# JamesYang007/adelie

Measured on AMD Instinct MI355X. Metric: lambda-paths/sec (100-lambda grpnet); HBM GB/s vs peak, higher is better.
Workload: dtype f64

## Files before the change

### adelie_amd/csrc/kernels.hpp

```cpp
#pragma once
#include <hip/hip_runtime.h>
#include <cstdint>

namespace ahip {

template <class T>
struct DenseView {
    const T* X;
    int64_t n, p, ld;
};
struct SnpView {
    const uint8_t* bits;
    int64_t n, p, ldb;
};

template <class T>
struct CscView {
    const int64_t* cptr;
    const int32_t* cidx;
    const T* cval;
    const int64_t* rptr;
    const int32_t* rcol;
    const T* rval;
    int64_t n, p, nnz;
    const int64_t* bptr;
    int nb;
    int64_t rb;
    const T* center;
    const T* inv_scale;
    const int64_t* tptr;
    const uint16_t* trow;
    const T* tval;
    int nt;
    int64_t th;
};

template <class T> void launch_vmul(const T* a, const T* b, T* out, int64_t n, hipStream_t s);
template <class T> void launch_fill(T* out, T value, int64_t n, hipStream_t s);

template <class T>
void launch_sweep(const DenseView<T>& X, const T* v, T* out, int64_t c0, int64_t ncols, const int32_t* cols,
                  const T* sub_scale, const T* sub_vec, bool square, T* work, hipStream_t s);
template <class T>
void launch_sweep_snp(const SnpView& X, const T* impute, const T* v, T* out, int64_t c0, int64_t ncols,
                      const int32_t* cols, const T* sub_scale, const T* sub_vec, bool square, T* work, hipStream_t s);
int64_t sweep_work_elems(int64_t n, int64_t ncols);
int64_t sweep_work_elems_csc(int nb, int64_t ncols);
template <class T>
void launch_sweep_csc(const CscView<T>& X, const T* v, T* out, int64_t c0, int64_t ncols, const int32_t* cols,
                      const T* sub_scale, const T* sub_vec, bool square, T* work, hipStream_t s);
constexpr int kVecSumScratch = 8 + 256;
template <class T> void launch_vec_sum(const T* v, int64_t n, T* out, hipStream_t s);
template <class T>
void launch_std_sweep_epilogue(const T* center, const T* inv_scale, const T* raw, const T* raw_plain, const T* vsum, bool square,
                               T* out, int64_t c0, int64_t ncols, const int32_t* cols, const T* sub_scale, const T* sub_vec,
                               hipStream_t s);
template <class T>
void launch_std_gram_fix(const T* center, const T* inv_scale, T* C, int64_t ldc, int32_t M, int32_t pos0, int32_t N,
                         const int32_t* vcol, const T* m, const T* wsum, const T* xm, bool centered, hipStream_t s);
template <class T>
void launch_std_scale_coef(const T* center, const T* inv_scale, const int32_t* cols, const T* coef, const int32_t* count_dev,
                           int32_t count, T* coef2, T* kappa, hipStream_t s);
template <class T> void launch_vec_shift(T* out, int64_t n, const T* kappa, T sign, const int32_t* count_dev, hipStream_t s);
template <class T>
void launch_std_fix_gblk(T* gblk, const int32_t* cols, int nb, const T* center, const T* inv_scale, const T* rsum_dev,
                         const T* xm_view_or_null, hipStream_t s);
struct SyrkBatch;
template <class T>
void launch_std_block_fix(T* D0, const SyrkBatch& sb, const int32_t* cols_base, int ldb, const T* center, const T* inv_scale,
                          const T* xm_view, const T* wsum_dev, bool centered, hipStream_t s);
template <class T>
void launch_csc_tile_scatter(const int64_t* colptr, const int32_t* cidx, const T* cval, int64_t p, int nt, int64_t th,
                             const int64_t* tptr, uint16_t* trow, T* tval, hipStream_t s);
constexpr int64_t kCscTileBytes = 128 * 1024;
void csc_block_layout(int64_t n, size_t value_size, int* nb, int64_t* rb);
void launch_csc_block_ptr(const int64_t* cptr, const int32_t* cidx, int64_t p, int nb, int64_t rb, int64_t* bptr, hipStream_t s);
int64_t gram_work_elems_csc(int64_t n, int64_t M, int64_t N, int nb);
template <class T>
void launch_gram_csc(const CscView<T>& X, const T* w, const int32_t* mcols, int32_t M, int32_t m_pos0, const int32_t* ncols,
                     int32_t N, int32_t n_pos0, const T* xm_by_col, bool center, T* C, int64_t ldc, T* work, hipStream_t s);
template <class T>
void launch_axpy_cols_csc(const CscView<T>& X, const int32_t* cols, const T* coef, const int32_t* count_dev, int32_t count,
                          T sign, T* out, T* delta_zeroed, hipStream_t s);
int64_t sp_tmul_work_elems_csc(int64_t p);
template <class T>
void launch_sp_tmul_csc(const CscView<T>& X, int64_t L, const int64_t* indptr, const int64_t* indices, const T* values, T* out,
                        T* work, hipStream_t s);

template <class T>
void launch_axpy_cols(const DenseView<T>& X, const int32_t* cols, const T* coef, const int32_t* count_dev,
                      int32_t count, T sign, T* out, hipStream_t s);
template <class T>
void launch_axpy_cols_snp(const SnpView& X, const T* impute, const int32_t* cols, const T* coef,
                          const int32_t* count_dev, int32_t count, T sign, T* out, hipStream_t s);
template <class T>
void launch_sp_tmul(const DenseView<T>& X, int64_t L, const int64_t* indptr, const int64_t* indices, const T* values,
                    T* out, hipStream_t s);
template <class T>
void launch_sp_tmul_snp(const SnpView& X, const T* impute, int64_t L, const int64_t* indptr, const int64_t* indices,
                        const T* values, T* out, hipStream_t s);

template <class T>
void launch_gram(const DenseView<T>& X, const T* w, const int32_t* mcols, int32_t M, int32_t m_pos0,
                 const int32_t* ncols, int32_t N, int32_t n_pos0, const T* xm_by_col, bool center, T* C, int64_t ldc,
                 T* work, hipStream_t s);
template <class T>
void launch_gram_snp(const SnpView& X, const T* impute, const T* w, const int32_t* mcols, int32_t M, int32_t m_pos0,
                     const int32_t* ncols, int32_t N, int32_t n_pos0, const T* xm_by_col, bool center, T* C,
                     int64_t ldc, T* work, hipStream_t s);
int64_t gram_work_elems(int64_t n, int64_t M, int64_t N);
struct SyrkBatch {
    static constexpr int MAX = 16;
    int32_t off[MAX];
    int32_t nb[MAX];
    int64_t dst[MAX];
    int32_t count;
};
int64_t syrk_batch_work_elems(int64_t n, int count);
template <class T>
void launch_panel_step_csc(const CscView<T>& X, const T* w, T* r, const int32_t* dcol, const T* dlt, const int32_t* nz_dev,
                           const int32_t* cols, int nb, const T* rsum_dev, const T* xm_by_col, T* gblk, hipStream_t s);
template <class T>
void launch_block_gram_csc(const CscView<T>& X, const T* w, const int32_t* cols_base, const SyrkBatch& sb, const T* xm_by_col,
                           bool center, T* D0, int ldb, hipStream_t s);
struct GramBatch {
// ... 180 lines not shown
    const T* C;
    int64_t ldc;
    const T* vars;
    const T* xmean;
    T* beta;
    T* g;
    int8_t* is_active;
    int32_t* active_set;
    T l1, l2, newton_tol, dbeta_tol;
    int32_t newton_max_iters, max_active_size, mark;
    const T* V;
    const int64_t* voff;
    const T* spen;
    const int32_t* sbegin;
    const int32_t* ssize;
    const int32_t* blk_g0;
    const int32_t* list;
    int32_t nblk;
    T* Dbuf;
    T* dlt;
    int32_t* didx;
    CdBlkState<T>* st;
    const T* gblk;
    const T* Dptr;
    const int32_t* vcol;
    int32_t* dcol;
    CdBlkState<T>* host_st;
    int32_t* host_seq;
    int32_t report_j, report_seq;
    int64_t* dbg;
    const T* Cprev;
    const T* pdlt;
    const int32_t* ppos;
    const int32_t* pnz;
    int32_t* dpos;
    int32_t* nz_out;
    T* rsum_out;
    int32_t rot;
    const int32_t* desc;
    const T* pdd;
    T* dd;
    const T* part;
    int32_t part_n;
    const T* part_rsum;
    int32_t* tail_counter;
    T* tail_g;
    const T* tail_rsum;
    const T* tail_xm;
    const T* clo;
    const T* chi;
    T* cmu;
    const T* Cnext;
    T* corr_out;
    const T* corr_in;
};
constexpr int GDESC_VMAP = 0;
constexpr int GDESC_VGRP = 128;
constexpr int GDESC_VSS = 256;
constexpr int GDESC_GOFF = 384;
constexpr int GDESC_GQ = 520;
constexpr int GDESC_GSS = 648;
constexpr int GDESC_NG = 776, GDESC_NVAL = 777;
constexpr int GDESC_VOFF = 784;
constexpr int GDESC_VPOS = 912;
constexpr int GDESC_VQ = 1040;
constexpr int GDESC_STRIDE = 1168;
template <class T> void launch_grp_layout(const CdGrpBlkParams<T>& p, int nblk, int32_t* desc, hipStream_t s);
struct GrpRotArgs {
    int32_t ng;
    int32_t goff[129];
    int64_t voff[128];
};
template <class T> void launch_grp_block_rotate(T* Dptr, const T* Dsrc, const T* V, const GrpRotArgs& a, T* scratch, hipStream_t s);
template <class T> void launch_cd_group_block_pass(const CdGrpBlkParams<T>& p, hipStream_t s);
template <class T> void launch_cd_group_block_range(const CdGrpBlkParams<T>& p, int j0, int j1, hipStream_t s);
template <class T> void launch_cd_group_block_update(const CdGrpBlkParams<T>& p, int j, hipStream_t s);
template <class T> void launch_cd_group_panel_solve(const CdGrpBlkParams<T>& p, int j, hipStream_t s);
int cd_block_size();
template <class T> void launch_cd_block_pass(const CdBlkParams<T>& p, hipStream_t s);
template <class T>
int launch_panel_step(const DenseView<T>& X, const T* w, T* r, const int32_t* dcol, const T* dlt, const int32_t* nz_dev,
                      const int32_t* cols, int nb, T* part, hipStream_t s);
template <class T>
struct StepTail {
    int32_t* counter;
    int32_t base;
    T* g;
    const T* rsum;
    const T* xm;
};
template <class T>
int launch_panel_step_snp(const SnpView& X, const T* impute, const T* w, T* r, const int32_t* dcol, const T* dlt,
                          const int32_t* nz_dev, const int32_t* cols, int nb, T* part, hipStream_t s,
                          const StepTail<T>* tail = nullptr, bool* tailed = nullptr);
int64_t panel_part_elems(int64_t n);
template <class T>
void launch_la_open_from_grad(const T* grad, const int32_t* cols, int nb, T* g, const T* rsum_src, T* rsum_out, hipStream_t s);
template <class T>
void launch_panel_reduce(const T* part, int nslices, int nb, const int32_t* cols, const T* rsum_dev, const T* xm_by_col,
                         T* gblk, hipStream_t s);
template <class T>
void launch_panel_reduce_ld(const T* part, int64_t part_ld, int nslices, int nb, const int32_t* cols, const T* rsum_dev,
                            const T* xm_by_col, T* gblk, hipStream_t s);
template <class T>
int launch_panel_fused(const CdBlkParams<T>& sp, int j, const DenseView<T>& X, const T* w, T* r, const int32_t* dcol,
                       const T* dlt, const int32_t* nz_dev, const int32_t* cols, int nb, T* part, bool tr, hipStream_t s);
template <class T>
int launch_panel_fused_snp(const CdBlkParams<T>& sp, int j, const SnpView& X, const T* impute, const T* w, T* r,
                           const int32_t* dcol, const T* dlt, const int32_t* nz_dev, const int32_t* cols, int nb, T* part,
                           bool tr, hipStream_t s);
template <class T>
int launch_panel_fused_grp(const CdGrpBlkParams<T>& sp, int j, const DenseView<T>& X, const T* w, T* r, const int32_t* dcol,
                           const T* dlt, const int32_t* nz_dev, const int32_t* cols, int nb, T* part, bool tr, hipStream_t s);
template <class T>
int launch_panel_fused_grp_snp(const CdGrpBlkParams<T>& sp, int j, const SnpView& X, const T* impute, const T* w, T* r,
                               const int32_t* dcol, const T* dlt, const int32_t* nz_dev, const int32_t* cols, int nb,
                               T* part, bool tr, hipStream_t s);
template <class T> void launch_cd_panel_solve(const CdBlkParams<T>& p, int j, hipStream_t s);
template <class T> void launch_center_vars(T* vars, const T* xm, int cnt, bool center, hipStream_t s);
void launch_gather_i32(const int32_t* src, const int32_t* idx, int cnt, int32_t* out, hipStream_t s);
template <class T>
void launch_cd_compact(const T* beta, const T* beta0, const int32_t* vcol, int nv, int32_t* dcols, T* dvals,
                       int32_t* n_delta, hipStream_t s);

template <class T>
struct MultiView {
    const T* X;
    int64_t nb, pb, ld;
    const T* ones;
    int32_t K, icpt;
    const uint8_t* bits = nullptr;
    int64_t ldb = 0;
    const T* impute = nullptr;
};
template <class T> void launch_multi_sweep(const MultiView<T>& X, const T* v, T* out, T* work, hipStream_t s);
template <class T> int64_t multi_sweep_work_elems(const MultiView<T>& X);
template <class T>
void launch_multi_sweep_snp(const SnpView& X, const T* impute, int K, const T* v, T* out, T* work, hipStream_t s);
template <class T>
int launch_multi_panel_step(const MultiView<T>& X, const T* w, T* r, const int32_t* dcol, const T* dlt,
                            const int32_t* nz_dev, const int32_t* cols, int nb_cols, T* part, hipStream_t s);
int64_t multi_panel_part_elems(int64_t nb);
template <class T>
void launch_multi_axpy_cols(const MultiView<T>& X, const int32_t* cols, const T* coef, const int32_t* cnt_dev, T sign,
                            T* out, hipStream_t s);
template <class T>
void launch_syrk_multi(const MultiView<T>& X, const T* w, const int32_t* ucols, int32_t M, T* C, int64_t ldc, T* work,
                       hipStream_t s);
template <class T>
void launch_multi_expand(const T* C, int64_t ldc, const int32_t* slot, const int32_t* resp, int nv, int lsel, T* D,
                         int64_t ldd, hipStream_t s);
void launch_multi_block_lists(const int32_t* cols, int nv, int K, int32_t* ulist, int32_t* slot, int32_t* resp,
                              hipStream_t s);
template <class T>
int launch_multi_panel_fused(const CdGrpBlkParams<T>& sp, int j, const MultiView<T>& X, const T* w, T* r,
                             const int32_t* dcol, const T* dlt, const int32_t* nz_dev, const int32_t* cols, int nb_cols,
                             T* part, hipStream_t s);
template <class T>
void launch_gram_multi(const MultiView<T>& X, const T* w, const int32_t* mcols, int32_t M, const int32_t* ncols, int32_t N,
                       T* C, int64_t ldc, T* work, hipStream_t s);
template <class T>
void launch_multi_expand_cross(const T* G, int64_t ldg, const int32_t* slot_r, const int32_t* resp_r, int nr,
                               const int32_t* slot_c, const int32_t* resp_c, int nc, T* C, int64_t ldc, hipStream_t s);
template <class T>
void launch_batch_pick(const T* src, int64_t nfeat, int K, int slot, const T* sub_scale, const T* sub_vec, T* out,
                       hipStream_t s);
template <class T> void launch_multi_to_major(const T* src, int64_t nb, int K, T* dst, hipStream_t s);
template <class T> void launch_multi_from_major(const T* src, int64_t nb, int K, T* dst, hipStream_t s);

template <class T>
struct IrlsScalars {
    T hess_sum, y_mean, y_var, resid_sum, conv, loss;
};

template <class T>
void launch_cov_gather(const T* S, int64_t lda, int tr, const int32_t* vcol, int32_t nv, int32_t pos0, int32_t N, T* C,
                       int64_t ldc, hipStream_t s);
template <class T>
void launch_cov_bmul(const T* S, int64_t lda, int tr, const int64_t* subset, int64_t ns, const int64_t* indices,
                     const T* values, int64_t ni, T* out, hipStream_t s);
// ... 84 lines not shown
```

### adelie_amd/csrc/kernels_cd_panel.hip

```cpp
#include "kernels.hpp"
#include "accessors.hpp"
#include "wavered.hpp"
#include "blk_solve_body.hpp"
#include "grp_solve_body.hpp"

namespace ahip {

namespace {

constexpr int PB = 128;
constexpr int PT = 256;

template <class T, int VEC>
struct RawDense { Pack<T, VEC> v; };
struct RawSnp { unsigned byte; };

template <class T, int VEC>
__device__ __forceinline__ RawDense<T, VEC> praw(const DenseAcc<T>& X, int64_t j, int64_t i, int64_t n, bool full) {
    RawDense<T, VEC> r;
    const T* col = X.colptr(j);
    if constexpr (VEC == 1) {
        const T x = col[(full || i < n) ? i : 0];
        r.v.v[0] = (full || i < n) ? x : T(0);
    } else {
        using V = typename VecOf<T>::type;
        static_assert(VEC == VecOf<T>::N, "dense vector width");
        const int64_t ii = (full || i < n) ? i : 0;
        const V x = __builtin_nontemporal_load(reinterpret_cast<const V*>(col + ii));
#pragma unroll
        for (int e = 0; e < VEC; ++e) r.v.v[e] = (full || i + e < n) ? x[e] : T(0);
    }
    return r;
}
template <class T, int VEC>
__device__ __forceinline__ RawSnp praw(const SnpAcc<T>& X, int64_t j, int64_t i, int64_t n, bool full) {
    static_assert(VEC == 4 || VEC == 16, "one byte (4 calls) or one 32-bit word (16 calls) per lane");
    RawSnp r;
    if constexpr (VEC == 4) {
        const unsigned b = unsigned(X.colptr(j)[((full || i < n) ? i : 0) >> 2]);
        r.byte = (full || i < n) ? b : 0u;
    } else {
        const unsigned b = reinterpret_cast<const unsigned*>(X.colptr(j))[((full || i < n) ? i : 0) >> 4];
        r.byte = (full || i < n) ? b : 0u;
    }
    return r;
}
template <class T, int VEC>
__device__ __forceinline__ Pack<T, VEC> pdecode(const DenseAcc<T>&, const RawDense<T, VEC>& r, int64_t, int64_t, int64_t) {
    return r.v;
}
template <class T, int VEC>
__device__ __forceinline__ Pack<T, VEC> pdecode(const SnpAcc<T>& X, const RawSnp& r, int64_t j, int64_t i, int64_t n) {
    Pack<T, VEC> o;
    const T imp = X.impute[j];
#pragma unroll
    for (int e = 0; e < VEC; ++e) {
        const unsigned c = (r.byte >> (2 * e)) & 3u;
        o.v[e] = (i + e < n) ? (c == 3u ? imp : T(c)) : T(0);
    }
    return o;
}
template <class T, class Acc, int VEC> struct RawOf;
template <class T, int VEC> struct RawOf<T, DenseAcc<T>, VEC> { using type = RawDense<T, VEC>; };
template <class T, int VEC> struct RawOf<T, SnpAcc<T>, VEC> { using type = RawSnp; };

template <class T, class Acc, int VEC, bool FULL, bool WGRED = false>
__device__ __forceinline__ void panel_step_body(const Acc& X, int64_t n, const T* __restrict__ w, T* __restrict__ r,
                                                const int32_t* __restrict__ dcol, const T* __restrict__ dlt, int nz,
                                                const int32_t* __restrict__ cols, int nb, T* __restrict__ part,
                                                int64_t part_ld, T (*red)[64 * VEC], T* wrs, int tid, int64_t slice) {
    constexpr int U = 16;
    using Raw = typename RawOf<T, Acc, VEC>::type;
    const int lane = tid & 63;
    const int wv = __builtin_amdgcn_readfirstlane(tid >> 6);
    const int64_t i = slice * (64 * VEC) + int64_t(lane) * VEC;
    const bool full = FULL ? true : (i + VEC <= n);

    constexpr int UB = 8;
    Raw xb[UB];
    int jb[UB];
    if (nb > 0) {
#pragma unroll
        for (int u = 0; u < UB; ++u) jb[u] = cols[min(wv + 4 * u, nb - 1)];
#pragma unroll
        for (int u = 0; u < UB; ++u) xb[u] = praw<T, VEC>(X, jb[u], i, n, full);
    }

    if (nz > 0) {
        T acc[VEC];
#pragma unroll
        for (int e = 0; e < VEC; ++e) acc[e] = T(0);
        for (int m0 = wv; m0 < nz; m0 += 4 * U) {
            Raw xa[U];
            int ja[U];
            T cf[U];
#pragma unroll
            for (int u = 0; u < U; ++u) {
                const int m = m0 + 4 * u;
                ja[u] = dcol[min(m, nz - 1)];
                cf[u] = m < nz ? dlt[min(m, nz - 1)] : T(0);
            }
#pragma unroll
            for (int u = 0; u < U; ++u) xa[u] = praw<T, VEC>(X, ja[u], i, n, full);
#pragma unroll
            for (int u = 0; u < U; ++u) {
                const Pack<T, VEC> xx = pdecode<T, VEC>(X, xa[u], ja[u], i, n);
#pragma unroll
                for (int e = 0; e < VEC; ++e) acc[e] = fma(cf[u], xx.v[e], acc[e]);
            }
        }
#pragma unroll
        for (int e = 0; e < VEC; ++e) red[wv][lane * VEC + e] = acc[e];
        __syncthreads();
        if (wv == 0) {
#pragma unroll
            for (int e = 0; e < VEC; ++e) {
                const int q = lane * VEC + e;
                T wr = T(0);
                if (FULL || i + e < n) {
                    const T rr = r[i + e] - ((red[0][q] + red[1][q]) + (red[2][q] + red[3][q]));
                    r[i + e] = rr;
                    wr = w[i + e] * rr;
                }
                wrs[q] = wr;
            }
        }
    } else if (wv == 0) {
#pragma unroll
        for (int e = 0; e < VEC; ++e) wrs[lane * VEC + e] = (FULL || i + e < n) ? w[i + e] * r[i + e] : T(0);
    }
    if (nb <= 0) return;
    __syncthreads();

    T wr[VEC];
#pragma unroll
    for (int e = 0; e < VEC; ++e) wr[e] = wrs[lane * VEC + e];
    for (int c0 = wv; c0 < nb; c0 += 4 * UB) {
        if (c0 != wv) {
#pragma unroll
            for (int u = 0; u < UB; ++u) jb[u] = cols[min(c0 + 4 * u, nb - 1)];
#pragma unroll
            for (int u = 0; u < UB; ++u) xb[u] = praw<T, VEC>(X, jb[u], i, n, full);
        }
        T pu[UB];
#pragma unroll
        for (int u = 0; u < UB; ++u) {
            const Pack<T, VEC> xx = pdecode<T, VEC>(X, xb[u], jb[u], i, n);
            T sacc = T(0);
#pragma unroll
            for (int e = 0; e < VEC; ++e) sacc = fma(xx.v[e], wr[e], sacc);
            pu[u] = sacc;
        }
        static_assert(UB == 8, "reduce8");
        const T tot = reduce8(pu, lane);
        if (lane < UB && c0 + 4 * lane < nb) {
            if constexpr (WGRED) red[0][c0 + 4 * lane] = tot;
            else part[part_ld > 0 ? int64_t(c0 + 4 * lane) * part_ld + slice : slice * PB + (c0 + 4 * lane)] = tot;
        }
    }
}

template <class T, class Acc, int VEC>
__global__ __launch_bounds__(PT, (VEC >= 16 ? 2 : 4)) void panel_step_kernel(Acc X, int64_t n, const T* __restrict__ w, T* __restrict__ r,
                                                        const int32_t* __restrict__ dcol, const T* __restrict__ dlt,
                                                        const int32_t* __restrict__ nz_dev,
                                                        const int32_t* __restrict__ cols, int nb, T* __restrict__ part,
                                                        int64_t part_ld) {
    constexpr int RS = 64 * VEC;
    __shared__ T red[4][RS];
    __shared__ T wrs[RS];
    const int nz = nz_dev[0];
    if ((int64_t(blockIdx.x) + 1) * RS <= n)
        panel_step_body<T, Acc, VEC, true>(X, n, w, r, dcol, dlt, nz, cols, nb, part, part_ld, red, wrs, threadIdx.x, blockIdx.x);
    else
        panel_step_body<T, Acc, VEC, false>(X, n, w, r, dcol, dlt, nz, cols, nb, part, part_ld, red, wrs, threadIdx.x, blockIdx.x);
}

constexpr int S16_RS = 1024;
constexpr int S16_NSUB = 2;

template <class T>
__device__ __forceinline__ T reduce16(const T (&v)[16], int lane) {
    const bool b0 = lane & 1, b1 = lane & 2, b2 = lane & 4, b3 = lane & 8;
    T a[8], c[4], d[2];
#pragma unroll
    for (int m = 0; m < 8; ++m) {
        const T keep = b0 ? v[2 * m + 1] : v[2 * m], send = b0 ? v[2 * m] : v[2 * m + 1];
        a[m] = keep + pdpp<0xB1>(send);
    }
#pragma unroll
    for (int m = 0; m < 4; ++m) {
        const T keep = b1 ? a[2 * m + 1] : a[2 * m], send = b1 ? a[2 * m] : a[2 * m + 1];
        c[m] = keep + pdpp<0x4E>(send);
    }
#pragma unroll
    for (int m = 0; m < 2; ++m) {
        const T keep = b2 ? c[2 * m + 1] : c[2 * m], send = b2 ? c[2 * m] : c[2 * m + 1];
        d[m] = keep + __shfl_xor(send, 4, 64);
    }
    const T keep = b3 ? d[1] : d[0], send = b3 ? d[0] : d[1];
    T t = keep + pdpp<0x128>(send);
    t += __shfl_xor(t, 16, 64);
    t += __shfl_xor(t, 32, 64);
    return t;
}

template <class T, bool FULL>
__device__ __forceinline__ void snp16_decode(unsigned word, T imp, int64_t i, int64_t n, T (&o)[16]) {
#pragma unroll
    for (int e = 0; e < 16; ++e) {
        const unsigned c = (word >> (2 * e)) & 3u;
        const T x = c == 3u ? imp : T(c);
        o[e] = (FULL || i + e < n) ? x : T(0);
    }
}

template <class T, bool FULL>
__device__ __forceinline__ void panel_step_snp16_body(const SnpAcc<T>& X, int64_t n, const T* __restrict__ w, T* __restrict__ r,
                                                      const int32_t* __restrict__ dcol, const T* __restrict__ dlt, int nz,
                                                      const int32_t* __restrict__ cols, int nb, T* __restrict__ part,
                                                      int64_t part_ld, T (*red)[S16_RS], T* wrs, T* psum, const T* ptab, int t,
                                                      int64_t slice) {
    constexpr int U = 16;
    const int lane = t & 63;
    const int wv = __builtin_amdgcn_readfirstlane(t >> 6);
    const int64_t i = slice * S16_RS + int64_t(lane) * 16;
    const bool in = FULL || i < n;
    const int64_t wofs = in ? (i >> 4) : 0;
    auto word = [&](int j) -> unsigned {
        const unsigned x = reinterpret_cast<const unsigned*>(X.colptr(j))[wofs];
        return in ? x : 0u;
    };
    unsigned xa[U], xb[U];
    int ja[U], jb[U];
    if (nz > 0) {
#pragma unroll
        for (int u = 0; u < U; ++u) ja[u] = dcol[min(wv + 4 * u, nz - 1)];
#pragma unroll
        for (int u = 0; u < U; ++u) xa[u] = word(ja[u]);
    }
    unsigned vmask = 0xFFFFFFFFu;
    if (!FULL) {
        const int64_t left = n - i;
        vmask = left >= 16 ? 0xFFFFFFFFu : (left <= 0 ? 0u : ((1u << (2 * int(left))) - 1u));
    }
    if (nb > 0) {
#pragma unroll
        for (int u = 0; u < U; ++u) jb[u] = cols[min(wv + 4 * u, nb - 1)];
#pragma unroll
        for (int u = 0; u < U; ++u) xb[u] = word(jb[u]);
    }
    const int64_t q0 = i + 4 * wv;
    T rq[4], wq[4];
#pragma unroll
    for (int k = 0; k < 4; ++k) {
        const bool ok = FULL || q0 + k < n;
        rq[k] = ok ? r[q0 + k] : T(0);
        wq[k] = ok ? w[q0 + k] : T(0);
// ... 196 lines not shown
            panel_step_body<T, Acc, VEC, true>(X, n, w, r, dcol, dlt, nz, cols, nb, part, part_ld, red, wrs, tid, slice4);
        else
            panel_step_body<T, Acc, VEC, false>(X, n, w, r, dcol, dlt, nz, cols, nb, part, part_ld, red, wrs, tid, slice4);
    }
}

inline int fused_fsa(int64_t ns) {
    if ((ns + 3) / 4 > 250) return 4;
    if (ns <= 250) return 1;
    if ((ns + 1) / 2 <= 250) return 2;
    return 4;
}

template <class T, class Acc, int VEC>
__global__ __launch_bounds__(256 * FS) void panel_fused_kernel(CdBlkParams<T> sp, int j, Acc X, int64_t n,
                                                              const T* __restrict__ w, T* __restrict__ r,
                                                              const int32_t* __restrict__ dcol, const T* __restrict__ dlt,
                                                              const int32_t* __restrict__ nz_dev,
                                                              const int32_t* __restrict__ cols, int nb,
                                                              T* __restrict__ part, int64_t part_ld, int fsa) {
    extern __shared__ __attribute__((aligned(16))) char smem_raw[];
    constexpr int RS = 64 * VEC;
    if (blockIdx.x == 0) {
        if (j < 0) {
            if (threadIdx.x == 0 && sp.part_rsum) {
                const T v = sp.part_rsum[0];
                sp.rsum_out[0] = v;
                sp.rsum_out[1] = v;
            }
            return;
        }
        blk_solve_la_body<T>(sp, j, smem_raw, threadIdx.x);
        return;
    }
    fused_step_part<T, Acc, VEC>(smem_raw, X, n, w, r, dcol, dlt, nz_dev, cols, nb, part, part_ld, fsa);
}

template <class T>
__global__ __launch_bounds__(PT) void panel_reduce_kernel(const T* __restrict__ part, int64_t part_ld, int nslices,
                                                          const int32_t* __restrict__ cols,
                                                          const T* __restrict__ rsum, const T* __restrict__ xm_by_col,
                                                          T* __restrict__ gblk) {
    __shared__ T red[4];
    const int c = blockIdx.x, tid = threadIdx.x, lane = tid & 63, wv = tid >> 6;
    const T* pc = part + int64_t(c) * part_ld;
    T s = T(0);
    for (int k = tid; k < nslices; k += PT) s += pc[k];
    s = wave_sum64(s);
    if (lane == 0) red[wv] = s;
    __syncthreads();
    if (tid == 0) {
        T g = (red[0] + red[1]) + (red[2] + red[3]);
        if (xm_by_col) g -= rsum[0] * xm_by_col[cols[c]];
        gblk[c] = g;
    }
}

template <class T>
__global__ void center_vars_kernel(T* __restrict__ vars, const T* __restrict__ xm, int cnt, int center) {
    const int a = blockIdx.x * blockDim.x + threadIdx.x;
    if (a >= cnt) return;
    T v = vars[a];
    if (center) v -= xm[a] * xm[a];
    vars[a] = v > T(0) ? v : T(0);
}

__global__ void gather_i32_kernel(const int32_t* __restrict__ src, const int32_t* __restrict__ idx, int cnt,
                                  int32_t* __restrict__ out) {
    const int a = blockIdx.x * blockDim.x + threadIdx.x;
    if (a < cnt) out[a] = src[idx[a]];
}

template <class T, class Acc, int VEC>
int step_launch(const Acc& acc, int64_t n, const T* w, T* r, const int32_t* dcol, const T* dlt, const int32_t* nz_dev,
                const int32_t* cols, int nb, T* part, hipStream_t s) {
    constexpr int RS = 64 * VEC;
    const int64_t ns = (n + RS - 1) / RS;
    hipLaunchKernelGGL((panel_step_kernel<T, Acc, VEC>), dim3((unsigned)ns), dim3(PT), 0, s, acc, n, w, r, dcol, dlt,
                       nz_dev, cols, nb, part, ns);
    return int(ns);
}

template <class T, class Acc, int VEC>
__global__ __launch_bounds__(256 * FS) void panel_fused_grp_kernel(CdGrpBlkParams<T> sp, int j, Acc X, int64_t n,
                                                                  const T* __restrict__ w, T* __restrict__ r,
                                                                  const int32_t* __restrict__ dcol,
                                                                  const T* __restrict__ dlt,
                                                                  const int32_t* __restrict__ nz_dev,
                                                                  const int32_t* __restrict__ cols, int nb,
                                                                  T* __restrict__ part, int64_t part_ld, int fsa) {
    extern __shared__ __attribute__((aligned(16))) char smem_raw[];
    constexpr int RS = 64 * VEC;
    if (blockIdx.x == 0) {
        if (j < 0) {
            if (threadIdx.x == 0 && sp.part_rsum) {
                const T v = sp.part_rsum[0];
                sp.rsum_out[0] = v;
                sp.rsum_out[1] = v;
            }
            return;
        }
        grp_solve_body<T, true, true>(sp, j, smem_raw, 256 * FS);
        return;
    }
    fused_step_part<T, Acc, VEC>(smem_raw, X, n, w, r, dcol, dlt, nz_dev, cols, nb, part, part_ld, fsa, sp.tail_counter != nullptr);
    if constexpr (RS >= PB) {
        if (sp.tail_counter == nullptr || nb <= 0) return;
        __shared__ int s_rank;
        __builtin_amdgcn_fence(__ATOMIC_RELEASE, "workgroup");
        __syncthreads();
        if (threadIdx.x == 0) s_rank = __hip_atomic_fetch_add(sp.tail_counter, 1, __ATOMIC_RELAXED, __HIP_MEMORY_SCOPE_AGENT);
        __syncthreads();
        const int nwg = int(gridDim.x) - 1, NT = nwg < 8 ? 1 : 8;
        const int rank = s_rank;
        if (rank < nwg - NT) return;
        const int tidx = rank - (nwg - NT);
        if (threadIdx.x == 0) {
            while (__hip_atomic_load(sp.tail_counter, __ATOMIC_RELAXED, __HIP_MEMORY_SCOPE_AGENT) < nwg) __builtin_amdgcn_s_sleep(1);
        }
        __syncthreads();
        __builtin_amdgcn_fence(__ATOMIC_ACQUIRE, "workgroup");
        T* red = reinterpret_cast<T*>(smem_raw);
        const int cpw = PB / NT;
        const int cl = int(threadIdx.x) % cpw, q = int(threadIdx.x) / cpw;
        const int c = tidx * cpw + cl;
        if (q < 8) {
            T sacc = T(0);
            for (int k0 = q; k0 < nwg; k0 += 8 * 32) {
                T v[32];
#pragma unroll
                for (int u = 0; u < 32; ++u) {
                    const int k = k0 + 8 * u;
                    v[u] = k < nwg ? __hip_atomic_load(part + int64_t(k) * PB + c, __ATOMIC_RELAXED, __HIP_MEMORY_SCOPE_AGENT) : T(0);
                }
#pragma unroll
                for (int u = 0; u < 32; ++u) sacc += v[u];
            }
            red[q * PB + c] = sacc;
        }
        __syncthreads();
        if (int(threadIdx.x) < cpw && c < nb) {
            T g = ((red[c] + red[PB + c]) + (red[2 * PB + c] + red[3 * PB + c])) +
                  ((red[4 * PB + c] + red[5 * PB + c]) + (red[6 * PB + c] + red[7 * PB + c]));
            if (sp.tail_xm) g -= sp.tail_rsum[0] * sp.tail_xm[cols[c]];
            sp.tail_g[c] = g;
        }
        if (threadIdx.x == 0) {
            const int d = __hip_atomic_fetch_add(sp.tail_counter + 1, 1, __ATOMIC_RELAXED, __HIP_MEMORY_SCOPE_AGENT);
            if (d == NT - 1) {
                __hip_atomic_store(sp.tail_counter + 1, 0, __ATOMIC_RELAXED, __HIP_MEMORY_SCOPE_AGENT);
                __hip_atomic_store(sp.tail_counter, 0, __ATOMIC_RELAXED, __HIP_MEMORY_SCOPE_AGENT);
            }
        }
    }
}

template <class T, class Acc, int VEC>
int fused_grp_launch(const CdGrpBlkParams<T>& sp, int j, const Acc& acc, int64_t n, const T* w, T* r, const int32_t* dcol,
                     const T* dlt, const int32_t* nz_dev, const int32_t* cols, int nb, T* part, bool tr, hipStream_t s) {
    constexpr int RS = 64 * VEC;
    const int64_t ns = (n + RS - 1) / RS;
    const int fsa = (64 * VEC >= PB) ? fused_fsa(ns) : FS;
    const int64_t nwg = (ns + fsa - 1) / fsa;
    const int64_t part_ld = (64 * VEC >= PB) ? nwg : nwg * FS;
    static bool attr_done = false;
    if (!attr_done) {
        (void)hipFuncSetAttribute(reinterpret_cast<const void*>(panel_fused_grp_kernel<T, Acc, VEC>),
                                  hipFuncAttributeMaxDynamicSharedMemorySize, int(grp_solve_lds_total<T>()));
        attr_done = true;
    }
    hipLaunchKernelGGL((panel_fused_grp_kernel<T, Acc, VEC>), dim3((unsigned)(nwg + 1)), dim3(256 * FS),
                       grp_solve_lds_total<T>(), s, sp, j, acc, n, w, r, dcol, dlt, nz_dev, cols, nb, part,
                       tr ? int64_t(0) : part_ld, fsa);
    return int(part_ld);
}

template <class T, class Acc, int VEC>
int fused_launch(const CdBlkParams<T>& sp, int j, const Acc& acc, int64_t n, const T* w, T* r, const int32_t* dcol,
                 const T* dlt, const int32_t* nz_dev, const int32_t* cols, int nb, T* part, bool tr, hipStream_t s) {
    constexpr int RS = 64 * VEC;
    const int64_t ns = (n + RS - 1) / RS;
    const int fsa = (64 * VEC >= PB) ? fused_fsa(ns) : FS;
    const int64_t nwg = (ns + fsa - 1) / fsa;
    const int64_t part_ld = (64 * VEC >= PB) ? nwg : nwg * FS;
    static bool attr_done = false;
    if (!attr_done) {
        (void)hipFuncSetAttribute(reinterpret_cast<const void*>(panel_fused_kernel<T, Acc, VEC>),
                                  hipFuncAttributeMaxDynamicSharedMemorySize, int(fused_lds<T>()));
        attr_done = true;
    }
    hipLaunchKernelGGL((panel_fused_kernel<T, Acc, VEC>), dim3((unsigned)(nwg + 1)), dim3(256 * FS),
                       fused_lds<T>(), s, sp, j, acc, n, w, r, dcol, dlt, nz_dev, cols, nb, part,
                       tr ? int64_t(0) : part_ld, fsa);
    return int(part_ld);
}

}

template <class T>
int launch_panel_fused(const CdBlkParams<T>& sp, int j, const DenseView<T>& X, const T* w, T* r, const int32_t* dcol,
                       const T* dlt, const int32_t* nz_dev, const int32_t* cols, int nb, T* part, bool tr, hipStream_t s) {
    DenseAcc<T> acc{X.X, X.ld};
    constexpr int V = VecOf<T>::N;
    const bool vecok = (X.ld % V == 0) && ((reinterpret_cast<uintptr_t>(X.X) % 16) == 0);
    if (vecok) return fused_launch<T, DenseAcc<T>, V>(sp, j, acc, X.n, w, r, dcol, dlt, nz_dev, cols, nb, part, tr, s);
    return fused_launch<T, DenseAcc<T>, 1>(sp, j, acc, X.n, w, r, dcol, dlt, nz_dev, cols, nb, part, tr, s);
}
template <class T>
int launch_panel_fused_snp(const CdBlkParams<T>& sp, int j, const SnpView& X, const T* impute, const T* w, T* r,
                           const int32_t* dcol, const T* dlt, const int32_t* nz_dev, const int32_t* cols, int nb, T* part,
                           bool tr, hipStream_t s) {
    SnpAcc<T> acc{X.bits, X.ldb, impute};
    return fused_launch<T, SnpAcc<T>, 4>(sp, j, acc, X.n, w, r, dcol, dlt, nz_dev, cols, nb, part, tr, s);
}

template <class T>
int launch_panel_fused_grp(const CdGrpBlkParams<T>& sp, int j, const DenseView<T>& X, const T* w, T* r, const int32_t* dcol,
                           const T* dlt, const int32_t* nz_dev, const int32_t* cols, int nb, T* part, bool tr, hipStream_t s) {
    DenseAcc<T> acc{X.X, X.ld};
    constexpr int V = VecOf<T>::N;
    const bool vecok = (X.ld % V == 0) && ((reinterpret_cast<uintptr_t>(X.X) % 16) == 0);
    if (vecok) return fused_grp_launch<T, DenseAcc<T>, V>(sp, j, acc, X.n, w, r, dcol, dlt, nz_dev, cols, nb, part, tr, s);
    return fused_grp_launch<T, DenseAcc<T>, 1>(sp, j, acc, X.n, w, r, dcol, dlt, nz_dev, cols, nb, part, tr, s);
}
template <class T>
int launch_panel_fused_grp_snp(const CdGrpBlkParams<T>& sp, int j, const SnpView& X, const T* impute, const T* w, T* r,
                               const int32_t* dcol, const T* dlt, const int32_t* nz_dev, const int32_t* cols, int nb,
                               T* part, bool tr, hipStream_t s) {
    SnpAcc<T> acc{X.bits, X.ldb, impute};
    return fused_grp_launch<T, SnpAcc<T>, 4>(sp, j, acc, X.n, w, r, dcol, dlt, nz_dev, cols, nb, part, tr, s);
}

namespace {
template <class T>
__global__ void la_open_kernel(const T* __restrict__ grad, const int32_t* __restrict__ cols, int nb, T* __restrict__ g,
                               const T* __restrict__ rsum_src, T* __restrict__ rsum_out) {
    const int c = threadIdx.x;
    if (c < nb) g[c] = grad[cols[c]];
    if (c == 0 && rsum_src) {
        const T v = rsum_src[0];
        rsum_out[0] = v;
        rsum_out[1] = v;
    }
}
}
template <class T>
void launch_la_open_from_grad(const T* grad, const int32_t* cols, int nb, T* g, const T* rsum_src, T* rsum_out, hipStream_t s) {
    hipLaunchKernelGGL((la_open_kernel<T>), dim3(1), dim3(PB), 0, s, grad, cols, nb, g, rsum_src, rsum_out);
}
template void launch_la_open_from_grad<double>(const double*, const int32_t*, int, double*, const double*, double*, hipStream_t);
template void launch_la_open_from_grad<float>(const float*, const int32_t*, int, float*, const float*, float*, hipStream_t);

int64_t panel_part_elems(int64_t n) { return int64_t(PB) * ((n + 63) / 64) + 16; }

template <class T>
int launch_panel_step(const DenseView<T>& X, const T* w, T* r, const int32_t* dcol, const T* dlt, const int32_t* nz_dev,
                      const int32_t* cols, int nb, T* part, hipStream_t s) {
    DenseAcc<T> acc{X.X, X.ld};
    constexpr int V = VecOf<T>::N;
    const bool vecok = (X.ld % V == 0) && ((reinterpret_cast<uintptr_t>(X.X) % 16) == 0);
    if (vecok) return step_launch<T, DenseAcc<T>, V>(acc, X.n, w, r, dcol, dlt, nz_dev, cols, nb, part, s);
    return step_launch<T, DenseAcc<T>, 1>(acc, X.n, w, r, dcol, dlt, nz_dev, cols, nb, part, s);
}

template <class T>
int launch_panel_step_snp(const SnpView& X, const T* impute, const T* w, T* r, const int32_t* dcol, const T* dlt,
                          const int32_t* nz_dev, const int32_t* cols, int nb, T* part, hipStream_t s, const StepTail<T>* tail,
                          bool* tailed) {
    SnpAcc<T> acc{X.bits, X.ldb, impute};
    if (tailed) *tailed = false;
    if (X.n >= 16384 && X.ldb % 4 == 0 && (reinterpret_cast<uintptr_t>(X.bits) % 4) == 0) {
        if (nb > PB) return step_launch<T, SnpAcc<T>, 16>(acc, X.n, w, r, dcol, dlt, nz_dev, cols, nb, part, s);
        constexpr int64_t RW = int64_t(S16_RS) * S16_NSUB;
        const int64_t nwg = (X.n + RW - 1) / RW;
        StepTail<T> tl{};
        if (tail && nb > 0) {
            tl = *tail;
            if (tailed) *tailed = true;
        }
        hipLaunchKernelGGL((panel_step_snp16_kernel<T>), dim3((unsigned)nwg), dim3(256 * S16_NSUB), 0, s, acc, X.n, w, r, dcol, dlt,
                           nz_dev, cols, nb, part, nwg, tl);
        return int(nwg);
    }
    return step_launch<T, SnpAcc<T>, 4>(acc, X.n, w, r, dcol, dlt, nz_dev, cols, nb, part, s);
}
template <class T>
void launch_panel_reduce(const T* part, int nslices, int nb, const int32_t* cols, const T* rsum_dev, const T* xm_by_col,
                         T* gblk, hipStream_t s) {
    if (nb <= 0) return;
    hipLaunchKernelGGL((panel_reduce_kernel<T>), dim3((unsigned)nb), dim3(PT), 0, s, part, int64_t(nslices), nslices, cols,
                       rsum_dev, xm_by_col, gblk);
}
template <class T>
void launch_panel_reduce_ld(const T* part, int64_t part_ld, int nslices, int nb, const int32_t* cols, const T* rsum_dev,
                            const T* xm_by_col, T* gblk, hipStream_t s) {
    if (nb <= 0) return;
    hipLaunchKernelGGL((panel_reduce_kernel<T>), dim3((unsigned)nb), dim3(PT), 0, s, part, part_ld, nslices, cols, rsum_dev,
                       xm_by_col, gblk);
}
template <class T>
void launch_center_vars(T* vars, const T* xm, int cnt, bool center, hipStream_t s) {
    if (cnt <= 0) return;
    hipLaunchKernelGGL((center_vars_kernel<T>), dim3((unsigned)((cnt + 255) / 256)), dim3(256), 0, s, vars, xm, cnt,
                       center ? 1 : 0);
}
void launch_gather_i32(const int32_t* src, const int32_t* idx, int cnt, int32_t* out, hipStream_t s) {
    if (cnt <= 0) return;
    hipLaunchKernelGGL(gather_i32_kernel, dim3((unsigned)((cnt + 255) / 256)), dim3(256), 0, s, src, idx, cnt, out);
}

#define INST(T)                                                                                                        \
    template int launch_panel_step<T>(const DenseView<T>&, const T*, T*, const int32_t*, const T*, const int32_t*,     \
                                      const int32_t*, int, T*, hipStream_t);                                           \
    template int launch_panel_step_snp<T>(const SnpView&, const T*, const T*, T*, const int32_t*, const T*,            \
                                          const int32_t*, const int32_t*, int, T*, hipStream_t, const StepTail<T>*,    \
                                          bool*);                                                                      \
    template void launch_panel_reduce<T>(const T*, int, int, const int32_t*, const T*, const T*, T*, hipStream_t);     \
    template void launch_panel_reduce_ld<T>(const T*, int64_t, int, int, const int32_t*, const T*, const T*, T*,       \
                                            hipStream_t);                                                              \
    template int launch_panel_fused<T>(const CdBlkParams<T>&, int, const DenseView<T>&, const T*, T*, const int32_t*,  \
                                       const T*, const int32_t*, const int32_t*, int, T*, bool, hipStream_t);          \
    template int launch_panel_fused_grp<T>(const CdGrpBlkParams<T>&, int, const DenseView<T>&, const T*, T*,           \
                                           const int32_t*, const T*, const int32_t*, const int32_t*, int, T*, bool,    \
                                           hipStream_t);                                                               \
    template int launch_panel_fused_grp_snp<T>(const CdGrpBlkParams<T>&, int, const SnpView&, const T*, const T*, T*,  \
                                               const int32_t*, const T*, const int32_t*, const int32_t*, int, T*, bool,\
                                               hipStream_t);                                                           \
    template int launch_panel_fused_snp<T>(const CdBlkParams<T>&, int, const SnpView&, const T*, const T*, T*,         \
                                           const int32_t*, const T*, const int32_t*, const int32_t*, int, T*, bool,    \
                                           hipStream_t);                                                               \
    template void launch_center_vars<T>(T*, const T*, int, bool, hipStream_t);
INST(double)
INST(float)
#undef INST

}
```

### adelie_amd/csrc/kernels_sweep.hip

```cpp
#include "kernels.hpp"
#include "accessors.hpp"
#include <cstdlib>

namespace ahip {

namespace {

constexpr int kThreads = 256;

template <class T>
__device__ __forceinline__ T wave_sum(T x) {
#pragma unroll
    for (int off = 32; off > 0; off >>= 1) x += __shfl_down(x, off, 64);
    return x;
}

template <class T, int VEC>
__device__ __forceinline__ Pack<T, VEC> load_vec(const T* p) {
    Pack<T, VEC> r;
    if constexpr (VEC == 1) r.v[0] = p[0];
    else {
        using V = typename VecOf<T>::type;
        V x = *reinterpret_cast<const V*>(p);
#pragma unroll
        for (int e = 0; e < VEC; ++e) r.v[e] = x[e];
    }
    return r;
}

template <class T, class Acc, int CB, int VEC, bool SQ>
__global__ __launch_bounds__(kThreads) void sweep_kernel(Acc X, const T* __restrict__ v, T* __restrict__ out,
                                                         int64_t n, int64_t c0, int64_t ncols,
                                                         const int32_t* __restrict__ cols, int64_t rows_per_split,
                                                         int nsplit, const T* __restrict__ sub_scale,
                                                         const T* __restrict__ sub_vec) {
    const int tid = threadIdx.x;
    const int64_t cb = blockIdx.x;
    const int split = blockIdx.y;
    const int64_t r0 = int64_t(split) * rows_per_split;
    const int64_t r1 = min(n, r0 + rows_per_split);

    int64_t cj[CB];
    decltype(X.colptr(0)) cp[CB];
#pragma unroll
    for (int k = 0; k < CB; ++k) {
        int64_t c = cb * CB + k;
        if (c >= ncols) c = ncols - 1;
        cj[k] = cols ? int64_t(cols[c]) : c0 + c;
        cp[k] = X.colptr(cj[k]);
    }
    T acc[CB];
#pragma unroll
    for (int k = 0; k < CB; ++k) acc[k] = T(0);

    const int64_t body_end = r0 + ((r1 - r0) / VEC) * VEC;
#pragma unroll 2
    for (int64_t i = r0 + int64_t(tid) * VEC; i < body_end; i += int64_t(kThreads) * VEC) {
        const Pack<T, VEC> vv = load_vec<T, VEC>(v + i);
        Pack<T, VEC> xx[CB];
#pragma unroll
        for (int k = 0; k < CB; ++k) xx[k] = X.template load<VEC>(cp[k], i, cj[k]);
#pragma unroll
        for (int k = 0; k < CB; ++k)
#pragma unroll
            for (int e = 0; e < VEC; ++e) {
                const T x = SQ ? xx[k].v[e] * xx[k].v[e] : xx[k].v[e];
                acc[k] = fma(x, vv.v[e], acc[k]);
            }
    }
    for (int64_t i = body_end + tid; i < r1; i += kThreads) {
        const T vi = v[i];
#pragma unroll
        for (int k = 0; k < CB; ++k) {
            const T x0 = X.template load<1>(cp[k], i, cj[k]).v[0];
            const T x = SQ ? x0 * x0 : x0;
            acc[k] = fma(x, vi, acc[k]);
        }
    }

    __shared__ T red[kThreads / 64][CB];
    const int lane = tid & 63, wv = tid >> 6;
#pragma unroll
    for (int k = 0; k < CB; ++k) {
        const T s = wave_sum(acc[k]);
        if (lane == 0) red[wv][k] = s;
    }
    __syncthreads();
    if (tid < CB) {
        const int64_t c = cb * CB + tid;
        if (c < ncols) {
            T s = T(0);
#pragma unroll
            for (int w = 0; w < kThreads / 64; ++w) s += red[w][tid];
            if (nsplit == 1) {
                if (sub_vec) s -= sub_scale[0] * sub_vec[cols ? int64_t(cols[c]) : c0 + c];
                out[c] = s;
            } else {
                out[int64_t(split) * ncols + c] = s;
            }
        }
    }
}

template <class T>
__global__ void sweep_reduce_kernel(const T* __restrict__ part, T* __restrict__ out, int64_t ncols, int nsplit,
                                    int64_t c0, const int32_t* __restrict__ cols, const T* __restrict__ sub_scale,
                                    const T* __restrict__ sub_vec) {
    const int64_t c = int64_t(blockIdx.x) * blockDim.x + threadIdx.x;
    if (c >= ncols) return;
    T s = T(0);
    for (int r = 0; r < nsplit; ++r) s += part[int64_t(r) * ncols + c];
    if (sub_vec) {
        const int64_t j = cols ? int64_t(cols[c]) : c0 + c;
        s -= sub_scale[0] * sub_vec[j];
    }
    out[c] = s;
}

constexpr int kSweepCB = 4;
inline int sweep_cb() { return kSweepCB; }

inline void sweep_shape(int64_t n, int64_t ncols, int vec, int64_t& blocks_c, int& nsplit, int64_t& rows_per_split) {
    const int cbv = sweep_cb();
    blocks_c = (ncols + cbv - 1) / cbv;
    const int64_t unit = int64_t(kThreads) * vec;
    const int64_t max_split = (n + unit * 4 - 1) / (unit * 4);
    int64_t want = (1024 + blocks_c - 1) / blocks_c;
    int64_t ns = want < 1 ? 1 : want;
    if (ns > max_split) ns = max_split;
    if (ns < 1) ns = 1;
    if (ns > 65535) ns = 65535;
    rows_per_split = (n + ns - 1) / ns;
    rows_per_split = ((rows_per_split + unit - 1) / unit) * unit;
    ns = (n + rows_per_split - 1) / rows_per_split;
    if (ns < 1) ns = 1;
    nsplit = int(ns);
}

template <class T, class Acc, int VEC>
void sweep_dispatch(Acc acc, const T* v, T* out, int64_t n, int64_t c0, int64_t ncols, const int32_t* cols,
                    const T* sub_scale, const T* sub_vec, bool square, T* work, hipStream_t s) {
    if (ncols <= 0) return;
    int64_t blocks_c, rows_per_split;
    int nsplit;
    sweep_shape(n, ncols, VEC, blocks_c, nsplit, rows_per_split);
    dim3 grid((unsigned)blocks_c, (unsigned)nsplit);
    T* dst = nsplit == 1 ? out : work;
    if (square && sweep_cb() == 8)
        hipLaunchKernelGGL((sweep_kernel<T, Acc, 8, VEC, true>), grid, dim3(kThreads), 0, s, acc, v, dst, n, c0,
                           ncols, cols, rows_per_split, nsplit, sub_scale, sub_vec);
    else if (square)
        hipLaunchKernelGGL((sweep_kernel<T, Acc, kSweepCB, VEC, true>), grid, dim3(kThreads), 0, s, acc, v, dst, n, c0,
                           ncols, cols, rows_per_split, nsplit, sub_scale, sub_vec);
    else if (sweep_cb() == 8)
        hipLaunchKernelGGL((sweep_kernel<T, Acc, 8, VEC, false>), grid, dim3(kThreads), 0, s, acc, v, dst, n, c0,
                           ncols, cols, rows_per_split, nsplit, sub_scale, sub_vec);
    else
        hipLaunchKernelGGL((sweep_kernel<T, Acc, kSweepCB, VEC, false>), grid, dim3(kThreads), 0, s, acc, v, dst, n, c0,
                           ncols, cols, rows_per_split, nsplit, sub_scale, sub_vec);
    if (nsplit > 1) {
        const int bt = 256;
        hipLaunchKernelGGL((sweep_reduce_kernel<T>), dim3((unsigned)((ncols + bt - 1) / bt)), dim3(bt), 0, s, work, out,
                           ncols, nsplit, c0, cols, sub_scale, sub_vec);
    }
}

template <class T, class Acc, int VEC>
__global__ __launch_bounds__(kThreads) void axpy_cols_kernel(Acc X, int64_t n, const int32_t* __restrict__ cols,
                                                             const T* __restrict__ coef,
                                                             const int32_t* __restrict__ count_dev, int32_t count,
                                                             T sign, T* __restrict__ out) {
    const int K = count_dev ? count_dev[0] : count;
    if (K <= 0) return;
    const int64_t i = (int64_t(blockIdx.x) * kThreads + threadIdx.x) * VEC;
    if (i >= n) return;
    if (i + VEC <= n) {
        T acc[VEC];
#pragma unroll
        for (int e = 0; e < VEC; ++e) acc[e] = T(0);
        int k = 0;
        for (; k + 4 <= K; k += 4) {
            Pack<T, VEC> xx[4];
            T cf[4];
#pragma unroll
            for (int u = 0; u < 4; ++u) {
                const int64_t j = cols[k + u];
                cf[u] = coef[k + u];
                xx[u] = X.template load<VEC>(X.colptr(j), i, j);
            }
#pragma unroll
            for (int u = 0; u < 4; ++u)
#pragma unroll
                for (int e = 0; e < VEC; ++e) acc[e] = fma(cf[u], xx[u].v[e], acc[e]);
        }
        for (; k < K; ++k) {
            const int64_t j = cols[k];
            const T cf = coef[k];
            const Pack<T, VEC> xx = X.template load<VEC>(X.colptr(j), i, j);
#pragma unroll
            for (int e = 0; e < VEC; ++e) acc[e] = fma(cf, xx.v[e], acc[e]);
        }
#pragma unroll
        for (int e = 0; e < VEC; ++e) out[i + e] += sign * acc[e];
    } else {
        for (int64_t r = i; r < n; ++r) {
            T acc = T(0);
            for (int k = 0; k < K; ++k) {
                const int64_t j = cols[k];
                acc = fma(coef[k], X.template load<1>(X.colptr(j), r, j).v[0], acc);
            }
            out[r] += sign * acc;
        }
    }
}

template <class T, class Acc, int VEC>
__global__ __launch_bounds__(kThreads) void sp_tmul_kernel(Acc X, int64_t n, const int64_t* __restrict__ indptr,
                                                           const int64_t* __restrict__ indices,
                                                           const T* __restrict__ values, T* __restrict__ out) {
    const int64_t l = blockIdx.y;
    const int64_t e0 = indptr[l], e1 = indptr[l + 1];
    const int64_t i = (int64_t(blockIdx.x) * kThreads + threadIdx.x) * VEC;
    if (i >= n) return;
    T* o = out + l * n;
    if (i + VEC <= n) {
        T acc[VEC];
#pragma unroll
        for (int e = 0; e < VEC; ++e) acc[e] = T(0);
        int64_t k = e0;
        for (; k + 4 <= e1; k += 4) {
            Pack<T, VEC> xx[4];
            T cf[4];
#pragma unroll
            for (int u = 0; u < 4; ++u) {
                const int64_t j = indices[k + u];
                cf[u] = values[k + u];
                xx[u] = X.template load<VEC>(X.colptr(j), i, j);
            }
#pragma unroll
            for (int u = 0; u < 4; ++u)
#pragma unroll
                for (int e = 0; e < VEC; ++e) acc[e] = fma(cf[u], xx[u].v[e], acc[e]);
        }
        for (; k < e1; ++k) {
            const int64_t j = indices[k];
            const T cf = values[k];
            const Pack<T, VEC> xx = X.template load<VEC>(X.colptr(j), i, j);
// ... 160 lines not shown
}

template <class T>
__global__ __launch_bounds__(256) void snp_impute_kernel(const uint8_t* __restrict__ bits, int64_t n, int64_t ldb,
                                                         T* __restrict__ impute) {
    __shared__ unsigned long long red[3][4];
    const int64_t j = blockIdx.x;
    const int tid = threadIdx.x, lane = tid & 63, wv = tid >> 6;
    const int64_t nb = (n + 3) / 4;
    unsigned long long c1 = 0, c2 = 0, c3 = 0;
    for (int64_t b = tid; b < nb; b += 256) {
        const unsigned byte = bits[j * ldb + b];
#pragma unroll
        for (int k = 0; k < 4; ++k) {
            const unsigned c = (byte >> (2 * k)) & 3u;
            c1 += c == 1u; c2 += c == 2u; c3 += c == 3u;
        }
    }
#pragma unroll
    for (int off = 32; off > 0; off >>= 1) {
        c1 += __shfl_xor(c1, off, 64); c2 += __shfl_xor(c2, off, 64); c3 += __shfl_xor(c3, off, 64);
    }
    if (lane == 0) { red[0][wv] = c1; red[1][wv] = c2; red[2][wv] = c3; }
    __syncthreads();
    if (tid == 0) {
        const unsigned long long s1 = red[0][0] + red[0][1] + red[0][2] + red[0][3];
        const unsigned long long s2 = red[1][0] + red[1][1] + red[1][2] + red[1][3];
        const unsigned long long s3 = red[2][0] + red[2][1] + red[2][2] + red[2][3];
        const unsigned long long valid = (unsigned long long)n - s3;
        impute[j] = T(double(s1 + 2 * s2) / double(valid > 0 ? valid : 1));
    }
}

inline unsigned grid1d(int64_t n, int bt, int64_t cap = 4096) {
    int64_t g = (n + bt - 1) / bt;
    if (g > cap) g = cap;
    if (g < 1) g = 1;
    return unsigned(g);
}

}

constexpr int kLutTile = 256;
inline void lut_shape(int64_t n, int64_t ncols, int64_t& blocks_c, int64_t& ns, int64_t& rps) {
    blocks_c = (ncols + kThreads - 1) / kThreads;
    ns = std::max<int64_t>(1, (8192 + blocks_c - 1) / blocks_c);
    ns = std::min<int64_t>(std::min(ns, std::max<int64_t>(1, n / (int64_t(kLutTile) * 8))), 65535);
    rps = (n + ns - 1) / ns;
    rps = ((rps + 2 * kLutTile - 1) / (2 * kLutTile)) * (2 * kLutTile);
    ns = (n + rps - 1) / rps;
}
int64_t sweep_work_elems(int64_t n, int64_t ncols) {
    if (ncols <= 0) return 0;
    int64_t blocks_c, rps;
    int ns;
    sweep_shape(n, ncols, 1, blocks_c, ns, rps);
    int64_t a = int64_t(ns) * ncols;
    sweep_shape(n, ncols, 4, blocks_c, ns, rps);
    int64_t b = int64_t(ns) * ncols;
    int64_t lns;
    lut_shape(n, ncols, blocks_c, lns, rps);
    return std::max(std::max(a, b), lns * ncols) + 16;
}

template <class T>
void launch_vmul(const T* a, const T* b, T* out, int64_t n, hipStream_t s) {
    if (n <= 0) return;
    hipLaunchKernelGGL((vmul_kernel<T>), dim3(grid1d(n, 256)), dim3(256), 0, s, a, b, out, n);
}
template <class T>
void launch_fill(T* out, T value, int64_t n, hipStream_t s) {
    if (n <= 0) return;
    hipLaunchKernelGGL((fill_kernel<T>), dim3(grid1d(n, 256)), dim3(256), 0, s, out, value, n);
}

template <class T>
static inline bool dense_vec_ok(const DenseView<T>& X) {
    constexpr int V = VecOf<T>::N;
    return (X.ld % V == 0) && ((reinterpret_cast<uintptr_t>(X.X) % 16) == 0);
}

template <class T>
void launch_sweep(const DenseView<T>& X, const T* v, T* out, int64_t c0, int64_t ncols, const int32_t* cols,
                  const T* sub_scale, const T* sub_vec, bool square, T* work, hipStream_t s) {
    DenseAcc<T> acc{X.X, X.ld};
    if (dense_vec_ok(X) && (reinterpret_cast<uintptr_t>(v) % 16) == 0)
        sweep_dispatch<T, DenseAcc<T>, VecOf<T>::N>(acc, v, out, X.n, c0, ncols, cols, sub_scale, sub_vec, square, work, s);
    else
        sweep_dispatch<T, DenseAcc<T>, 1>(acc, v, out, X.n, c0, ncols, cols, sub_scale, sub_vec, square, work, s);
}
constexpr int LUT_TR = 256;
static_assert(LUT_TR == 256, "lut_shape's tile");
template <class T, bool SQ>
__global__ __launch_bounds__(kThreads) void sweep_snp_lut_kernel(const uint8_t* __restrict__ bits, int64_t ldb,
                                                                 const T* __restrict__ impute, const T* __restrict__ v,
                                                                 T* __restrict__ out, int64_t n, int64_t c0, int64_t ncols,
                                                                 const int32_t* __restrict__ cols, int64_t rows_per_split,
                                                                 int nsplit, const T* __restrict__ sub_scale,
                                                                 const T* __restrict__ sub_vec) {
    static_assert(kThreads == 256, "256 columns per workgroup, 8 lanes per line");
    constexpr int NP = LUT_TR / 2;
    typedef unsigned u4_t __attribute__((ext_vector_type(4)));
    constexpr int NQ = LUT_TR / 4;
    __shared__ T t012[NP][16];
    __shared__ T t3q[NQ][16];
    __shared__ u4_t stage[kThreads * 8];
    __shared__ int64_t cofs[kThreads];
    const int tid = threadIdx.x;
    const int split = blockIdx.y;
    const int64_t r0 = int64_t(split) * rows_per_split;
    const int64_t r1 = min(n, r0 + rows_per_split);
    int64_t c = int64_t(blockIdx.x) * kThreads + tid;
    const bool live = c < ncols;
    if (!live) c = ncols - 1;
    const int64_t cj = cols ? int64_t(cols[c]) : c0 + c;
    cofs[tid] = cj * ldb;
    __syncthreads();
    const int fp = tid & 7, fc = tid >> 3;
    const uint8_t* fptr[8];
#pragma unroll
    for (int u = 0; u < 8; ++u) fptr[u] = bits + cofs[fc + 32 * u] + fp * 16;
    const int tp = tid >> 1, te0 = (tid & 1) * 8;
    const int tq = tid >> 2, tqe0 = (tid & 3) * 4;
    T a = T(0), b = T(0);
    u4_t w[8];
#pragma unroll
    for (int u = 0; u < 8; ++u) w[u] = __builtin_nontemporal_load(reinterpret_cast<const u4_t*>(fptr[u] + r0 / 4));
    for (int64_t base = r0; base < r1; base += 2 * LUT_TR) {
        __syncthreads();
#pragma unroll
        for (int u = 0; u < 8; ++u) {
            const int col = fc + 32 * u;
            stage[col * 8 + ((fp + col) & 7)] = w[u];
        }
        const int64_t nbase = base + 2 * LUT_TR;
        if (nbase < r1) {
#pragma unroll
            for (int u = 0; u < 8; ++u) w[u] = __builtin_nontemporal_load(reinterpret_cast<const u4_t*>(fptr[u] + nbase / 4));
        }
        T vv[4], vq[8];
#pragma unroll
        for (int h = 0; h < 2; ++h) {
            const int64_t i0 = base + h * LUT_TR + 2 * tp;
            vv[2 * h] = i0 < r1 ? v[i0] : T(0);
            vv[2 * h + 1] = i0 + 1 < r1 ? v[i0 + 1] : T(0);
            const int64_t j0 = base + h * LUT_TR + 4 * tq;
#pragma unroll
            for (int k = 0; k < 4; ++k) vq[4 * h + k] = j0 + k < r1 ? v[j0 + k] : T(0);
        }
#pragma unroll
        for (int h = 0; h < 2; ++h) {
            const T v0 = vv[2 * h], v1 = vv[2 * h + 1];
            if (h == 1) __syncthreads();
#pragma unroll
            for (int e = 0; e < 8; ++e) {
                const int idx = te0 + e, k0 = idx & 3, k1 = idx >> 2;
                t012[tp][idx] = (k0 < 3 ? T(SQ ? k0 * k0 : k0) : T(0)) * v0 + (k1 < 3 ? T(SQ ? k1 * k1 : k1) : T(0)) * v1;
            }
#pragma unroll
            for (int e = 0; e < 4; ++e) {
                const int idx = tqe0 + e;
                t3q[tq][idx] = (((idx & 1) ? vq[4 * h] : T(0)) + ((idx & 2) ? vq[4 * h + 1] : T(0))) +
                               (((idx & 4) ? vq[4 * h + 2] : T(0)) + ((idx & 8) ? vq[4 * h + 3] : T(0)));
            }
            __syncthreads();
            u4_t wd[4];
#pragma unroll
            for (int u = 0; u < 4; ++u) wd[u] = stage[tid * 8 + ((4 * h + u + tid) & 7)];
#pragma unroll
            for (int u = 0; u < 4; ++u) {
#pragma unroll
                for (int hh = 0; hh < 4; ++hh) {
                    const unsigned wq = wd[u][hh];
                    unsigned ms = wq & (wq >> 1) & 0x55555555u;
                    ms = (ms | (ms >> 1)) & 0x33333333u;
                    ms = (ms | (ms >> 2)) & 0x0F0F0F0Fu;
#pragma unroll
                    for (int k = 0; k < 8; ++k) {
                        const int pr = (u * 4 + hh) * 8 + k;
                        a += t012[pr][(wq >> (4 * k)) & 15u];
                    }
#pragma unroll
                    for (int k = 0; k < 4; ++k) {
                        const int qr = (u * 4 + hh) * 4 + k;
                        b += t3q[qr][(ms >> (8 * k)) & 15u];
                    }
                }
            }
        }
    }
    if (!live) return;
    const T imp = impute[cj];
    T sres = fma(SQ ? imp * imp : imp, b, a);
    if (nsplit == 1) {
        if (sub_vec) sres -= sub_scale[0] * sub_vec[cj];
        out[c] = sres;
    } else {
        out[int64_t(split) * ncols + c] = sres;
    }
}

template <class T>
void launch_sweep_snp(const SnpView& X, const T* impute, const T* v, T* out, int64_t c0, int64_t ncols,
                      const int32_t* cols, const T* sub_scale, const T* sub_vec, bool square, T* work, hipStream_t s) {
    if (ncols >= 512 && X.n >= 4096 && X.ldb % 128 == 0 && (reinterpret_cast<uintptr_t>(X.bits) % 128) == 0) {
        int64_t blocks_c, ns, rps;
        lut_shape(X.n, ncols, blocks_c, ns, rps);
        T* dst = ns == 1 ? out : work;
        if (square)
            hipLaunchKernelGGL((sweep_snp_lut_kernel<T, true>), dim3((unsigned)blocks_c, (unsigned)ns), dim3(kThreads), 0, s,
                               X.bits, X.ldb, impute, v, dst, X.n, c0, ncols, cols, rps, int(ns), sub_scale, sub_vec);
        else
            hipLaunchKernelGGL((sweep_snp_lut_kernel<T, false>), dim3((unsigned)blocks_c, (unsigned)ns), dim3(kThreads), 0, s,
                               X.bits, X.ldb, impute, v, dst, X.n, c0, ncols, cols, rps, int(ns), sub_scale, sub_vec);
        if (ns > 1) {
            const int bt = 256;
            hipLaunchKernelGGL((sweep_reduce_kernel<T>), dim3((unsigned)((ncols + bt - 1) / bt)), dim3(bt), 0, s, work, out,
                               ncols, int(ns), c0, cols, sub_scale, sub_vec);
        }
        return;
    }
    SnpAcc<T> acc{X.bits, X.ldb, impute};
    sweep_dispatch<T, SnpAcc<T>, VecOf<T>::N>(acc, v, out, X.n, c0, ncols, cols, sub_scale, sub_vec, square, work, s);
}

template <class T>
void launch_axpy_cols(const DenseView<T>& X, const int32_t* cols, const T* coef, const int32_t* count_dev,
                      int32_t count, T sign, T* out, hipStream_t s) {
    if (X.n <= 0 || (!count_dev && count <= 0)) return;
    DenseAcc<T> acc{X.X, X.ld};
    constexpr int V = VecOf<T>::N;
    if (dense_vec_ok(X)) {
        const unsigned g = unsigned((X.n + int64_t(kThreads) * V - 1) / (int64_t(kThreads) * V));
        hipLaunchKernelGGL((axpy_cols_kernel<T, DenseAcc<T>, V>), dim3(g), dim3(kThreads), 0, s, acc, X.n, cols, coef,
                           count_dev, count, sign, out);
    } else {
        const unsigned g = unsigned((X.n + kThreads - 1) / kThreads);
        hipLaunchKernelGGL((axpy_cols_kernel<T, DenseAcc<T>, 1>), dim3(g), dim3(kThreads), 0, s, acc, X.n, cols, coef,
                           count_dev, count, sign, out);
    }
}
template <class T>
void launch_axpy_cols_snp(const SnpView& X, const T* impute, const int32_t* cols, const T* coef,
                          const int32_t* count_dev, int32_t count, T sign, T* out, hipStream_t s) {
    if (X.n <= 0 || (!count_dev && count <= 0)) return;
    SnpAcc<T> acc{X.bits, X.ldb, impute};
    constexpr int V = VecOf<T>::N;
    const unsigned g = unsigned((X.n + int64_t(kThreads) * V - 1) / (int64_t(kThreads) * V));
    hipLaunchKernelGGL((axpy_cols_kernel<T, SnpAcc<T>, V>), dim3(g), dim3(kThreads), 0, s, acc, X.n, cols, coef,
                       count_dev, count, sign, out);
}

template <class T>
void launch_sp_tmul(const DenseView<T>& X, int64_t L, const int64_t* indptr, const int64_t* indices, const T* values,
                    T* out, hipStream_t s) {
    if (L <= 0 || X.n <= 0) return;
    DenseAcc<T> acc{X.X, X.ld};
    constexpr int V = VecOf<T>::N;
    const bool vec = dense_vec_ok(X) && (X.n % V == 0);
    for (int64_t l0 = 0; l0 < L; l0 += 65535) {
        const unsigned ly = unsigned(L - l0 < 65535 ? L - l0 : 65535);
        if (vec) {
            const unsigned g = unsigned((X.n + int64_t(kThreads) * V - 1) / (int64_t(kThreads) * V));
            hipLaunchKernelGGL((sp_tmul_kernel<T, DenseAcc<T>, V>), dim3(g, ly), dim3(kThreads), 0, s, acc, X.n,
                               indptr + l0, indices, values, out + l0 * X.n);
        } else {
            const unsigned g = unsigned((X.n + kThreads - 1) / kThreads);
            hipLaunchKernelGGL((sp_tmul_kernel<T, DenseAcc<T>, 1>), dim3(g, ly), dim3(kThreads), 0, s, acc, X.n,
                               indptr + l0, indices, values, out + l0 * X.n);
        }
    }
}
template <class T>
void launch_sp_tmul_snp(const SnpView& X, const T* impute, int64_t L, const int64_t* indptr, const int64_t* indices,
                        const T* values, T* out, hipStream_t s) {
    if (L <= 0 || X.n <= 0) return;
    SnpAcc<T> acc{X.bits, X.ldb, impute};
    constexpr int V = VecOf<T>::N;
    const bool vec = (X.n % V == 0);
    for (int64_t l0 = 0; l0 < L; l0 += 65535) {
        const unsigned ly = unsigned(L - l0 < 65535 ? L - l0 : 65535);
        if (vec) {
            const unsigned g = unsigned((X.n + int64_t(kThreads) * V - 1) / (int64_t(kThreads) * V));
            hipLaunchKernelGGL((sp_tmul_kernel<T, SnpAcc<T>, V>), dim3(g, ly), dim3(kThreads), 0, s, acc, X.n,
                               indptr + l0, indices, values, out + l0 * X.n);
        } else {
            const unsigned g = unsigned((X.n + kThreads - 1) / kThreads);
            hipLaunchKernelGGL((sp_tmul_kernel<T, SnpAcc<T>, 1>), dim3(g, ly), dim3(kThreads), 0, s, acc, X.n,
                               indptr + l0, indices, values, out + l0 * X.n);
        }
    }
}

template <class T>
void launch_abs_grad(const T* grad, const int64_t* groups, const int64_t* group_sizes, int64_t G, const int32_t* slot,
                     const T* screen_beta, const T* penalty, T oma_lmda, T* abs_grad, hipStream_t s) {
    if (G <= 0) return;
    hipLaunchKernelGGL((abs_grad_kernel<T>), dim3(unsigned((G + 255) / 256)), dim3(256), 0, s, grad, groups,
                       group_sizes, G, slot, screen_beta, penalty, oma_lmda, abs_grad);
}

// ... 91 lines not shown
    }
    dst[c * ldb_dst + bo] = uint8_t(out);
}
void launch_snp_subset(const SnpView& X, int64_t nout, int64_t pout, const int64_t* rows, const int64_t* cols, uint8_t* dst,
                       int64_t ldb_dst, hipStream_t s) {
    for (int64_t c0 = 0; c0 < pout; c0 += 65535) {
        const int64_t pc = std::min<int64_t>(65535, pout - c0);
        hipLaunchKernelGGL(snp_subset_kernel, dim3((unsigned)((ldb_dst + 255) / 256), (unsigned)pc), dim3(256), 0, s,
                           X.bits + (cols ? 0 : c0 * X.ldb), X.ldb, nout, pc, rows, cols ? cols + c0 : nullptr, dst + c0 * ldb_dst,
                           ldb_dst);
    }
}
template <class T>
__global__ void gather_cols_kernel(const T* __restrict__ src, const int64_t* __restrict__ cols, int64_t pout, T* __restrict__ out) {
    const int64_t c = int64_t(blockIdx.x) * blockDim.x + threadIdx.x;
    if (c < pout) out[c] = src[cols ? cols[c] : c];
}
template <class T>
void launch_gather_cols(const T* src, const int64_t* cols, int64_t pout, T* out, hipStream_t s) {
    hipLaunchKernelGGL((gather_cols_kernel<T>), dim3((unsigned)((pout + 255) / 256)), dim3(256), 0, s, src, cols, pout, out);
}

template <class T>
__global__ void csc_scatter_kernel(const int64_t* __restrict__ indptr, const int32_t* __restrict__ indices,
                                   const T* __restrict__ values, int64_t n, T* __restrict__ dst, int64_t ld) {
    const int64_t c = blockIdx.x;
    const int64_t b = indptr[c], e = indptr[c + 1];
    T* col = dst + c * ld;
    for (int64_t k = b + threadIdx.x; k < e; k += blockDim.x) {
        const int64_t i = indices[k];
        if (i >= 0 && i < n) atomicAdd(col + i, values[k]);
    }
}
template <class T>
void launch_csc_scatter(const int64_t* indptr, const int32_t* indices, const T* values, int64_t n, int64_t p, T* dst,
                        int64_t ld, hipStream_t s) {
    for (int64_t c0 = 0; c0 < p; c0 += 1 << 30) {
        const int64_t pc = std::min<int64_t>(int64_t(1) << 30, p - c0);
        hipLaunchKernelGGL((csc_scatter_kernel<T>), dim3((unsigned)pc), dim3(256), 0, s, indptr + c0, indices, values, n,
                           dst + c0 * ld, ld);
    }
}

template <class T>
void launch_transpose(const T* src, int64_t n, int64_t p, T* dst, int64_t ld, hipStream_t s) {
    if (n <= 0 || p <= 0) return;
    const int64_t gy_total = (n + 31) / 32;
    for (int64_t y0 = 0; y0 < gy_total; y0 += 65535) {
        const unsigned gy = unsigned(gy_total - y0 < 65535 ? gy_total - y0 : 65535);
        hipLaunchKernelGGL((transpose_kernel<T>), dim3(unsigned((p + 31) / 32), gy), dim3(32, 8), 0, s,
                           src + y0 * 32 * p, n - y0 * 32, p, dst + y0 * 32, ld);
    }
}
void launch_pack_snp(const int8_t* calldata, int64_t n, int64_t p, uint8_t* bits, int64_t ldb, hipStream_t s) {
    if (n <= 0 || p <= 0) return;
    for (int64_t j0 = 0; j0 < p; j0 += 65535) {
        const unsigned cy = unsigned(p - j0 < 65535 ? p - j0 : 65535);
        hipLaunchKernelGGL(pack_snp_kernel, dim3(grid1d(ldb, 256, 256), cy), dim3(256), 0, s, calldata + j0 * n, n, p,
                           bits + j0 * ldb, ldb);
    }
}

void launch_bed_transcode(const uint8_t* bed, int64_t n, int64_t p, int64_t stride_in, uint8_t* bits, int64_t ldb,
                          hipStream_t s) {
    if (n <= 0 || p <= 0) return;
    for (int64_t j0 = 0; j0 < p; j0 += 65535) {
        const unsigned cy = unsigned(p - j0 < 65535 ? p - j0 : 65535);
        hipLaunchKernelGGL(bed_transcode_kernel, dim3(grid1d(ldb, 256, 256), cy), dim3(256), 0, s, bed + j0 * stride_in, n,
                           stride_in, bits + j0 * ldb, ldb);
    }
}
template <class T>
void launch_snp_impute(const uint8_t* bits, int64_t n, int64_t p, int64_t ldb, T* impute, hipStream_t s) {
    if (p <= 0) return;
    hipLaunchKernelGGL((snp_impute_kernel<T>), dim3((unsigned)p), dim3(256), 0, s, bits, n, ldb, impute);
}
template void launch_snp_impute<double>(const uint8_t*, int64_t, int64_t, int64_t, double*, hipStream_t);
template void launch_snp_impute<float>(const uint8_t*, int64_t, int64_t, int64_t, float*, hipStream_t);

#define INST(T)                                                                                                        \
    template void launch_vmul<T>(const T*, const T*, T*, int64_t, hipStream_t);                                        \
    template void launch_fill<T>(T*, T, int64_t, hipStream_t);                                                         \
    template void launch_sweep<T>(const DenseView<T>&, const T*, T*, int64_t, int64_t, const int32_t*, const T*,       \
                                  const T*, bool, T*, hipStream_t);                                                    \
    template void launch_sweep_snp<T>(const SnpView&, const T*, const T*, T*, int64_t, int64_t, const int32_t*,        \
                                      const T*, const T*, bool, T*, hipStream_t);                                      \
    template void launch_axpy_cols<T>(const DenseView<T>&, const int32_t*, const T*, const int32_t*, int32_t, T, T*,   \
                                      hipStream_t);                                                                    \
    template void launch_axpy_cols_snp<T>(const SnpView&, const T*, const int32_t*, const T*, const int32_t*, int32_t, \
                                          T, T*, hipStream_t);                                                         \
    template void launch_sp_tmul<T>(const DenseView<T>&, int64_t, const int64_t*, const int64_t*, const T*, T*,        \
                                    hipStream_t);                                                                      \
    template void launch_sp_tmul_snp<T>(const SnpView&, const T*, int64_t, const int64_t*, const int64_t*, const T*,   \
                                        T*, hipStream_t);                                                              \
    template void launch_abs_grad<T>(const T*, const int64_t*, const int64_t*, int64_t, const int32_t*, const T*,      \
                                     const T*, T, T*, hipStream_t);                                                    \
    template void launch_abs_grad_cons<T>(const T*, const int64_t*, const int64_t*, int64_t, const int32_t*, const T*, \
                                          const T*, T, const T*, const T*, const T*, T*, T*, hipStream_t);             \
    template void launch_copy2d<T>(const T*, int64_t, T*, int64_t, int64_t, int64_t, hipStream_t);                     \
    template void launch_diag_vars<T>(const T*, int64_t, int32_t, int32_t, T*, hipStream_t);                           \
    template void launch_block_diag_vars<T>(const T*, const SyrkBatch&, int, int32_t, const int32_t*, T*, hipStream_t); \
    template void launch_csc_scatter<T>(const int64_t*, const int32_t*, const T*, int64_t, int64_t, T*, int64_t, hipStream_t);\
    template void launch_transpose<T>(const T*, int64_t, int64_t, T*, int64_t, hipStream_t);                            \
    template void launch_derive_dense<T>(const DenseView<T>&, int64_t, int64_t, const int64_t*, const int64_t*, const T*, \
                                         const T*, T*, int64_t, hipStream_t);                                          \
    template void launch_derive_dense_snp<T>(const SnpView&, const T*, int64_t, int64_t, const int64_t*, const int64_t*, \
                                             const T*, const T*, T*, int64_t, hipStream_t);                              \
    template void launch_gather_cols<T>(const T*, const int64_t*, int64_t, T*, hipStream_t);
INST(double)
INST(float)
#undef INST

}
```

### adelie_amd/csrc/solver_fit.hpp

```cpp
    FitOut<T> pin_solve(T lm, T pin_tol, T rsq_in, T& rsum_io, T y_mean_pin, T* r_dev) {
        poll_mid();
        const idx ns = idx(screen_set.size());
        FitOut<T> o;
        bool resume = false;
        if (spec_active) {
            resume = lm == spec_lm && r_dev == d_r.p && !is_glm() && nv >= spec_nv && panel_mode() &&
                     active_set_size == spec_asz;
            if (!resume) spec_rollback();
        }
        if (!resume) {
            AHIP_CHECK(hipMemcpyAsync(d_beta0.p, d_beta.p, size_t(nv) * sizeof(T), hipMemcpyDeviceToDevice, st));
        } else if (nv > spec_nv) {
            AHIP_CHECK(hipMemcpyAsync(d_beta0.p + spec_nv, d_beta.p + spec_nv, size_t(nv - spec_nv) * sizeof(T),
                                      hipMemcpyDeviceToDevice, st));
        }
        CdScalars<T> sc{};
        sc.rsq = rsq_in;
        sc.resid_sum = rsum_io;
        sc.active_size = int32_t(active_set_size);
        d_sc.upload(&sc, 1, st);
        CdParams<T> cp{};
        cp.nv = int32_t(nv);
        cp.ns = int32_t(ns);
        cp.sbegin = d_sbegin.p;
        cp.ssize = d_ssize.p;
        cp.spen = d_spen.p;
        cp.spen2 = has_pen2 ? d_spen2.p : nullptr;
        cp.C = d_C.p;
        cp.ldc = ldc;
        cp.vars = d_vars.p;
        cp.xmean = d_sxm.p;
        cp.V = d_V.p;
        cp.voff = d_voff.p;
        cp.beta = d_beta.p;
        cp.g = d_g.p;
        cp.is_active = d_isact.p;
        cp.active_set = d_actset.p;
        cp.lmda = lm;
        cp.alpha = alpha;
        cp.tol = pin_tol;
        cp.newton_tol = newton_tol;
        cp.dbeta_tol = T(g_dbeta_tol);
        cp.newton_max_iters = int32_t(std::min<size_t>(newton_max_iters, size_t(1) << 30));
        cp.max_active_size = int32_t(std::min<size_t>(max_active_size, size_t(1) << 30));
        cp.intercept = intercept;
        cp.all_scalar = all_scalar ? 1 : 0;
        cp.max_iters = int64_t(max_iters);
        cp.sc = d_sc.p;
        cp.beta0 = d_beta0.p;
        cp.vcol = d_vcol.p;
        cp.dcols = d_dcols.p;
        cp.dvals = d_dvals.p;
        cp.max_group_size = int32_t(max_gs);
        Stopwatch sw;
        sw.start();
        bool small_fit = false;
        open_from_grad = grad_fresh && open_from_grad_opt && !is_glm() && !cov_mode && r_dev == d_r.p && !resume && !std_generic();
        grad_fresh = false;
        if (!(nv > 0 && panel_mode() && !all_scalar)) join_uv();
        if (nv > 0 && panel_mode()) {
            spec_mode = resume ? 2 : 0;
            spec_active = false;
            struct ModeGuard { int& m; ~ModeGuard() { m = 0; } } mode_guard{spec_mode};
            if (all_scalar) run_panel_passes(cp, sc, r_dev);
            else run_group_panel_passes(cp, sc, r_dev);
            if (!is_glm() && sc.status == CD_OK && r_dev == d_r.p && prelaunch_sweep && inv_wanted) {
                launch_vmul<T>(d_w.p, d_r.p, d_v.p, n, st);
                t_sweep.begin(st);
                sweep(d_v.p, d_grad.p, nullptr, p, &d_blk.p->resid_sum, intercept ? d_xm.p : nullptr);
                t_sweep.end(st);
                device_abs_grad(lm, int(sc.active_size));
                grad_fresh = true;
                inv_prelaunched = true;
                inv_prelaunched_lm = lm;
            }
        } else if (nv > 0 && all_scalar && nv >= cd_block_min_nv) {
            run_block_passes(cp, sc, (is_glm() && gram_stale) ? r_dev : nullptr);
        } else if (nv > 0 && !all_scalar && max_gs <= cd_block_size() && nv >= cd_block_min_nv) {
            run_group_block_passes(cp, sc);
        } else {
            if (nv > 0) {
                t_cd.begin(st);
                launch_cd<T>(cp, st);
                t_cd.end(st);
            }
            d_sc.download(&sc, 1, st);
            sync();
            small_fit = true;
        }
        const double t_cd = sw.elapsed();
        open_from_grad = false;
        if (nv == 0) {
            if (!(T(0) < pin_tol)) throw max_cds_error(0);
            sc.status = CD_OK;
            sc.iters = 2;
        }
        cnt.n_cd_visits_screen += sc.n_visits_screen;
        cnt.n_cd_visits_active += sc.n_visits_active;
        cnt.n_updates += sc.n_updates;
        cnt.n_update_cols += all_scalar ? sc.n_updates : int64_t(double(sc.n_updates) * double(nv) / double(std::max<idx>(ns, 1)) + 0.5);
        cnt.n_cd_passes_screen += sc.n_passes_screen;
        cnt.n_cd_passes_active += sc.n_passes_active;
        for (int i = 0; i < 8; ++i) cd_dbg[i] += sc.dbg[i];
        if (sc.status != CD_OK) {
            AHIP_CHECK(hipMemcpyAsync(d_beta.p, d_beta0.p, size_t(nv) * sizeof(T), hipMemcpyDeviceToDevice, st));
            d_isact.upload(screen_is_active.data(), screen_is_active.size(), st);
            actcols_key = -1;
            ptab_act.count = -1;
            sync();
            if (sc.status == CD_MAX_CDS) throw max_cds_error(0);
            if (sc.status == CD_MAX_ACTIVE) throw make_solver_error("Maximum number of active groups reached.");
            if (sc.status == CD_CONS_PN) throw make_solver_error("ConstraintBase: proximal newton max iterations reached!");
            if (sc.status == CD_CONS_QP_BOX) throw make_solver_error("StatePinballFull: max iterations reached!");
            if (sc.status == CD_CONS_QP_NNQP) throw make_solver_error("StateNNQPFull: max iterations reached!");
            if (sc.status == CD_CONS_UNEXPECTED)
                throw make_core_error("Possibly an unexpected error! Previous iterate should have been properly initialized. ");
            throw make_solver_error("Newton-ABS max iterations reached! Try increasing newton_max_iters.");
        }
        if (sc.n_delta > 0 && !cov_mode) {
            t_axpy.begin(st);
            axpy_cols(d_dcols.p, d_dvals.p, &d_sc.p->n_delta, 0, T(-1), r_dev);
            t_axpy.end(st);
            cnt.n_resid_col_reads += sc.n_delta;
        }
        if (small_fit && !is_glm() && !cov_mode && prelaunch_sweep && inv_wanted && sc.status == CD_OK && r_dev == d_r.p &&
            !multi()) {
            launch_vmul<T>(d_w.p, d_r.p, d_v.p, n, st);
            t_sweep.begin(st);
            sweep(d_v.p, d_grad.p, nullptr, p, &d_sc.p->resid_sum, intercept ? d_xm.p : nullptr);
            t_sweep.end(st);
            device_abs_grad(lm, int(sc.active_size));
            grad_fresh = true;
            inv_prelaunched = true;
            inv_prelaunched_lm = lm;
        }
        grad_valid = false;
        const size_t old_active = active_set_size;
        active_set_size = size_t(sc.active_size);
        rsum_io = sc.resid_sum;
        o.rsq = sc.rsq;
        if (!defer_fit_output) d_beta.download(screen_beta.data(), size_t(nv), st);
        std::vector<int32_t> act(active_set_size > old_active ? active_set_size - old_active : 0);
        if (!act.empty()) d_actset.download(act.data(), act.size(), st, old_active);
        bool waited = false;
        if (spec_enabled && spec_next_lm > T(0) && inv_prelaunched && inv_prelaunched_lm == lm && !cons_on && nv > 0 &&
            panel_mode() && r_dev == d_r.p) {
            if (!spec_ev) AHIP_CHECK(hipEventCreateWithFlags(&spec_ev, hipEventDisableTiming));
            AHIP_CHECK(hipEventRecord(spec_ev, st));
            const size_t stage_mark = stage.mark();
            if (!all_scalar) {
                AHIP_CHECK(hipEventSynchronize(spec_ev));
                stage.flush();
                for (size_t i = 0; i < act.size(); ++i) {
                    active_set[old_active + i] = act[i];
                    screen_is_active[act[i]] = 1;
                }
                act.clear();
            }
            d_r_snap.reserve(size_t(n));
            AHIP_CHECK(hipMemcpyAsync(d_beta0.p, d_beta.p, size_t(nv) * sizeof(T), hipMemcpyDeviceToDevice, st));
            AHIP_CHECK(hipMemcpyAsync(d_r_snap.p, d_r.p, size_t(n) * sizeof(T), hipMemcpyDeviceToDevice, st));
            CdParams<T> cp2 = cp;
            cp2.lmda = spec_next_lm;
            CdScalars<T> sc2{};
            sc2.rsq = sc.rsq;
            sc2.resid_sum = sc.resid_sum;
            sc2.active_size = sc.active_size;
            spec_mode = 1;
            open_from_grad = grad_fresh && open_from_grad_opt;
            spec_used_grad = grad_fresh;
            grad_fresh = false;
            {
                struct ModeGuard { int& m; ~ModeGuard() { m = 0; } } mode_guard{spec_mode};
                if (all_scalar) run_panel_passes(cp2, sc2, r_dev);
                else run_group_panel_passes(cp2, sc2, r_dev);
            }
            if (spec_enqueued) {
                spec_active = true;
                spec_lm = spec_next_lm;
                spec_nv = nv;
                spec_asz = active_set_size;
                ++n_spec;
            }
            AHIP_CHECK(hipEventSynchronize(spec_ev));
            stage.flush();
            stage.release(stage_mark);
            waited = true;
        }
        if (!waited) sync();
        for (size_t i = 0; i < act.size(); ++i) {
            active_set[old_active + i] = act[i];
            screen_is_active[act[i]] = 1;
        }
        o.intercept = T(intercept) * (y_mean_pin + rsum_io);
        const double va = double(sc.n_visits_active), vs = double(sc.n_visits_screen);
        o.t_active = (va + vs) > 0 ? t_cd * va / (va + vs) : 0;
        o.t_screen = t_cd - o.t_active;
        if (!defer_fit_output) assemble_fit_output(o, true);
        return o;
    }

    bool defer_fit_output = false;
    void assemble_fit_output(FitOut<T>& o, bool have_beta) {
        if (!have_beta && nv > 0) {
            d_beta.download(screen_beta.data(), size_t(nv), st);
            sync();
        }
        {
            auto by_col = [&](idx i, idx j) { return groups[screen_set[active_set[i]]] < groups[screen_set[active_set[j]]]; };
            if (active_order.size() > active_set_size) active_order.clear();
            const size_t have = active_order.size();
            if (have < active_set_size) {
                std::vector<idx> fresh(active_set_size - have);
                std::iota(fresh.begin(), fresh.end(), idx(have));
                std::sort(fresh.begin(), fresh.end(), by_col);
                std::vector<idx> merged(active_set_size);
                std::merge(active_order.begin(), active_order.end(), fresh.begin(), fresh.end(), merged.begin(), by_col);
                active_order.swap(merged);
            }
        }
        const std::vector<idx>& order = active_order;
        o.beta_idx.reserve(size_t(nv));
        o.beta_val.reserve(size_t(nv));
        for (size_t i = 0; i < order.size(); ++i) {
            const idx ss = active_set[order[i]], g = screen_set[ss];
            for (idx t = 0; t < group_sizes[g]; ++t) {
                o.beta_idx.push_back(groups[g] + t);
                o.beta_val.push_back(screen_beta[screen_begins[ss] + t]);
            }
        }
    }

    void load_screen_gradient(const T* w_dev, const T* r_dev, const T* rsum_dev) {
        if (nv == 0) return;
        if (grad_valid) {
            launch_gather<T>(d_grad.p, d_vcol.p, nv, d_g.p, st);
        } else {
            launch_vmul<T>(w_dev, r_dev, d_v.p, n, st);
            sweep(d_v.p, d_g.p, d_vcol.p, nv, rsum_dev, intercept ? d_sxm_by_value() : nullptr);
        }
    }
    const T* d_sxm_by_value() const { return d_xm.p; }

    FitOut<T> cov_fit(T lm) {
        if (nv > 0) launch_gather<T>(d_grad.p, d_vcol.p, nv, d_g.p, st);
        T rsum = 0;
        FitOut<T> o = pin_solve(lm, tol, rsq, rsum, T(0), nullptr);
        rsq = o.rsq;
        return o;
    }

    FitOut<T> gaussian_fit(T lm) {
        CdScalars<T> sc{};
        sc.resid_sum = resid_sum;
        d_sc.upload(&sc, 1, st);
        cur_w = d_w.p;
// ... 303 lines not shown
```

### adelie_amd/csrc/solver_panel.hpp

```cpp
    void run_block_passes(const CdParams<T>& cp, CdScalars<T>& sc, T* r_stale = nullptr) {
        const int B = cd_block_size();
        if (r_stale) {
            d_beta_ref.reserve(size_t(cp.nv) + 8);
            AHIP_CHECK(hipMemcpyAsync(d_beta_ref.p, cp.beta, size_t(cp.nv) * sizeof(T), hipMemcpyDeviceToDevice, st));
        }
        int64_t n_pass = 0;
        d_blk.reserve(1);
        d_Dbuf.reserve(size_t(2) * B * B);
        d_dlt.reserve(B);
        d_didx.reserve(B);
        CdBlkState<T> bs{};
        bs.rsq = sc.rsq;
        bs.resid_sum = sc.resid_sum;
        bs.cm = 0;
        bs.n_updates = 0;
        bs.active_size = sc.active_size;
        bs.status = CD_OK;
        d_blk.upload(&bs, 1, st);
        CdBlkParams<T> bp{};
        bp.nv = cp.nv; bp.C = cp.C; bp.ldc = cp.ldc; bp.vars = cp.vars; bp.xmean = cp.xmean; bp.spen = cp.spen; bp.spen2 = cp.spen2;
        bp.beta = cp.beta; bp.g = cp.g; bp.is_active = cp.is_active; bp.active_set = cp.active_set;
        bp.l1 = cp.lmda * cp.alpha; bp.l2 = cp.lmda * (T(1) - cp.alpha);
        bp.max_active_size = cp.max_active_size;
        bp.Dbuf = d_Dbuf.p; bp.dlt = d_dlt.p; bp.didx = d_didx.p; bp.st = d_blk.p;
// ... 30 lines not shown
                const T cm = pass(cp.active_set, asz, false);
                if (status != CD_OK) break;
                if (cm < cp.tol) break;
                if (iters >= cp.max_iters) { status = CD_MAX_CDS; break; }
            }
            if (status != CD_OK) break;
            ++iters;
            ++sc.n_passes_screen;
            sc.n_visits_screen += cp.nv;
            const T cm = pass(nullptr, cp.nv, true);
            if (status != CD_OK) break;
            if (cm < cp.tol) break;
            if (iters >= cp.max_iters) { status = CD_MAX_CDS; break; }
        }
        sc.rsq = bs.rsq;
        sc.resid_sum = bs.resid_sum;
        sc.iters = iters;
        sc.n_updates = bs.n_updates;
        sc.active_size = asz;
        sc.status = status;
        launch_cd_compact<T>(cp.beta, r_stale ? d_beta_ref.p : cp.beta0, cp.vcol, cp.nv, cp.dcols, cp.dvals, &cp.sc->n_delta, st);
        AHIP_CHECK(hipMemcpyAsync(&sc.n_delta, &cp.sc->n_delta, sizeof(int32_t), hipMemcpyDeviceToHost, st));
        sync();
    }

    CdBlkState<T>* rep_st_dev = nullptr;
    int32_t* rep_seq_dev = nullptr;
    size_t panel_maxblk = 0;
    void panel_setup(size_t maxblk) {
        const int SL = cd_block_size();
        d_blk.reserve(1);
        d_dlt.reserve(SL);
        d_dcolblk.reserve(SL);
        d_gblk.reserve(SL);
        d_actcols.reserve(size_t(p) + SL);
        d_part.reserve(size_t(panel_part_elems(n)));
        if (panel_maxblk != maxblk) {
            d_Dpool.reserve(size_t(2) * maxblk * SL * SL);
            AHIP_CHECK(hipMemsetAsync(d_Dpool.p, 0, size_t(2) * maxblk * SL * SL * sizeof(T), st));
            dscr_nb.assign(maxblk, 0); dact_nb.assign(maxblk, 0);
            dscr_ver.assign(maxblk, 0); dact_ver.assign(maxblk, 0);
            if (strips_apply() && !all_scalar) {
                d_Draw.reserve(size_t(2) * maxblk * SL * SL);
                AHIP_CHECK(hipMemsetAsync(d_Draw.p, 0, size_t(2) * maxblk * SL * SL * sizeof(T), st));
            }
            panel_maxblk = maxblk;
        }
        if (side_grams && !st2) st2 = StreamPool::take();
        for (int k = 0; side_grams && k < std::min(n_side - 1, kMaxExtra); ++k)
            if (!st_x[k]) st_x[k] = StreamPool::take();
        if (use_report && !h_report) {
            void* hp = HostPool::take(sizeof(PassReport), hipHostMallocMapped);
            void* dp = nullptr;
            if (hp && hipHostGetDevicePointer(&dp, hp, 0) == hipSuccess) {
                h_report = static_cast<PassReport*>(hp);
                std::memset(h_report, 0, sizeof(PassReport));
                rep_st_dev = &static_cast<PassReport*>(dp)->st;
                rep_seq_dev = &static_cast<PassReport*>(dp)->seq;
            } else {
                (void)hipGetLastError();
                HostPool::give(hp, sizeof(PassReport), hipHostMallocMapped);
                use_report = false;
            }
        }
    }
    void wait_pass_state(CdBlkState<T>& bs) {
        if (h_report) {
            const auto t_spin = std::chrono::steady_clock::now();
            int spins = 0;
            while (__atomic_load_n(&h_report->seq, __ATOMIC_ACQUIRE) != report_seq) {
                if ((++spins & 0xFFFF) == 0 &&
                    std::chrono::duration<double>(std::chrono::steady_clock::now() - t_spin).count() > 20.0)
                    break;
            }
            if (__atomic_load_n(&h_report->seq, __ATOMIC_ACQUIRE) == report_seq) {
                bs = h_report->st;
                return;
            }
        }
        d_blk.download(&bs, 1, st);
        sync();
    }

    void run_panel_passes(const CdParams<T>& cp, CdScalars<T>& sc, T* r_dev) {
        const int B = panel_bsz > 0 ? panel_bsz : (is_glm() ? 64 : cd_block_size());
        const int SL = cd_block_size();
        const size_t maxblk = size_t((p + B - 1) / B + 1);
        panel_setup(maxblk);
        CdBlkState<T> bs{};
        bs.rsq = sc.rsq;
        bs.resid_sum = sc.resid_sum;
        bs.active_size = sc.active_size;
        bs.status = CD_OK;
        bs.nz = 0;
        const int mode = spec_mode;
        if (mode != 2) d_blk.upload(&bs, 1, st);
        bool first_open = open_from_grad && mode != 2 && !cons_on;
        open_from_grad = false;
        CdBlkParams<T> bp{};
        bp.nv = cp.nv; bp.vars = cp.vars; bp.xmean = cp.xmean; bp.spen = cp.spen; bp.spen2 = cp.spen2;
        bp.beta = cp.beta; bp.is_active = cp.is_active; bp.active_set = cp.active_set;
        bp.l1 = cp.lmda * cp.alpha; bp.l2 = cp.lmda * (T(1) - cp.alpha);
        bp.max_active_size = cp.max_active_size;
        bp.dlt = d_dlt.p; bp.st = d_blk.p;
        bp.gblk = d_gblk.p; bp.vcol = cp.vcol; bp.dcol = d_dcolblk.p;
        if (cons_on) { bp.clo = d_clo.p; bp.chi = d_chi.p; bp.cmu = d_cmu.p; }
        bp.bsz = B;
        bp.host_st = rep_st_dev; bp.host_seq = rep_seq_dev; bp.report_j = -1; bp.report_seq = 0;
        const T* xm_c = intercept ? cur_xm : nullptr;
        const bool trace = hooks.trace >= 1;
        int64_t iters = 0;
        int status = CD_OK;
        int asz = sc.active_size;
        for (hipEvent_t e : pre_ev)
            if (e) AHIP_CHECK(hipStreamWaitEvent(st, e, 0));
        pre_ev.clear();
        pre_used = 0;
        const bool prebuild_screen = is_glm() && prebuild_enabled;
        bool screen_prebuilt = false;
        const bool la = lookahead && !is_glm() && B == SL && !std_generic() && !sparse();
        if (la) {
            if (xscr_key.size() != maxblk) {
                d_Xpool.reserve(size_t(2) * maxblk * SL * SL);
                xscr_key.assign(maxblk, XKey{});
                xact_key.assign(maxblk, XKey{});
            }
            d_la_dlt.reserve(size_t(2) * SL); d_la_g.reserve(size_t(2) * SL); d_la_rsum.reserve(2); d_la_dd.reserve(size_t(2) * SL);
            d_la_dcol.reserve(size_t(2) * SL); d_la_dpos.reserve(size_t(2) * SL); d_la_nz.reserve(2);
            if (!d_zero_i32.p) {
                d_zero_i32.reserve(1);
                AHIP_CHECK(hipMemsetAsync(d_zero_i32.p, 0, sizeof(int32_t), st));
            }
            d_part.reserve(size_t(2 * panel_part_elems(n) + 2048));
            part2_half = size_t(panel_part_elems(n));
            d_part2.reserve(2 * part2_half);
            if (mode != 2) pending_slot = -1;
        }
        bool no_wait = false;
        auto pass_la = [&](bool screen_pass) -> T {
            const bool first_pass = first_open;
            first_open = false;
            const int count = screen_pass ? cp.nv : asz;
            if (count <= 0) return T(0);
            const int32_t* cols_all = d_vcol.p;
            if (!screen_pass) {
                if (actcols_key != count) launch_gather_i32(d_vcol.p, cp.active_set, count, d_actcols.p, st);
                actcols_key = count;
                cols_all = d_actcols.p;
            }
            auto& tab_nb = screen_pass ? dscr_nb : dact_nb;
            auto& tab_ver = screen_pass ? dscr_ver : dact_ver;
            T* pool = d_Dpool.p + (screen_pass ? size_t(0) : maxblk * SL * SL);
            T* xpool = d_Xpool.p + (screen_pass ? size_t(0) : maxblk * SL * SL);
            bp.list = screen_pass ? nullptr : cp.active_set;
            bp.count = count;
            bp.mark = screen_pass ? 1 : 0;
            const int nblk = (count + B - 1) / B;
            auto nb_of = [&](int j) { return std::min(B, count - j * B); };
            auto cols_of = [&](int j) { return cols_all + size_t(j) * B; };
            Stopwatch sw_enq;
            sw_enq.start();
            record_pass_e0();
            t_cd.begin(st);
            const bool fr_open = fuse_reduce && la_fused_open;
            int prev_ld = 0;
            const bool from_grad = fr_open && first_pass && pending_slot < 0;
            if (from_grad) {
                launch_la_open_from_grad<T>(d_grad.p, cols_all, nb_of(0), d_la_g.p, xm_c ? &d_blk.p->resid_sum : nullptr,
                                            d_la_rsum.p, st);
            } else if (fr_open) {
                const int ps = pending_slot;
                CdBlkParams<T> op = bp;
                op.report_j = -1;
                op.rsum_out = d_la_rsum.p;
                op.part_rsum = xm_c ? &d_blk.p->resid_sum : nullptr;
                const int32_t* dc = ps < 0 ? d_dcolblk.p : d_la_dcol.p + size_t(ps) * SL;
                const T* dl = ps < 0 ? d_dlt.p : d_la_dlt.p + size_t(ps) * SL;
                const int32_t* nzp = ps < 0 ? &d_blk.p->nz : d_la_nz.p + ps;
                T* part_out = d_part2.p + part2_half;
                if (time_panel) t_step.begin(st);
                if (dense())
                    prev_ld = launch_panel_fused<T>(op, -1, D->dense<T>(), cur_w, r_dev, dc, dl, nzp, cols_all, nb_of(0), part_out, true, st);
                else
                    prev_ld = launch_panel_fused_snp<T>(op, -1, D->snp(), static_cast<const T*>(D->impute), cur_w, r_dev, dc, dl, nzp,
                                                        cols_all, nb_of(0), part_out, true, st);
                if (time_panel) t_step.end(st);
                cnt.n_panel_cols += nb_of(0);
            } else {
                const int nb01 = nb_of(0) + (nblk > 1 ? nb_of(1) : 0);
                const int ps = pending_slot;
                if (time_panel) t_step.begin(st);
                const int nsl = panel_step(cur_w, r_dev, ps < 0 ? d_dcolblk.p : d_la_dcol.p + size_t(ps) * SL,
                                           ps < 0 ? d_dlt.p : d_la_dlt.p + size_t(ps) * SL,
                                           ps < 0 ? &d_blk.p->nz : d_la_nz.p + ps, cols_all, nb01);
                if (time_panel) t_step.end(st);
                launch_panel_reduce<T>(d_part.p, nsl, nb01, cols_all, &d_blk.p->resid_sum, xm_c, d_la_g.p, st);
                cnt.n_panel_cols += nb01;
            }
            build_stale_strips(nblk, tab_nb, tab_ver, screen_pass ? &xscr_key : &xact_key, pool, xpool, nb_of, cols_of);
            build_stale_blocks(nblk, tab_nb, tab_ver, pool, nb_of, cols_of);
            build_stale_cross(nblk, screen_pass ? xscr_key : xact_key, xpool, nb_of, cols_of);
            merge_strip_events(true);
            pass_e0_valid = false;
            for (int j = 0; j < nblk; ++j) {
                const int slot = j & 1, pslot = slot ^ 1;
                bp.gblk = d_la_g.p + size_t(slot) * B;
                bp.part = (fuse_reduce && prev_ld > 0) ? d_part2.p + size_t((j - 1) & 1) * part2_half : nullptr;
                bp.part_ld = 0;
                bp.part_n = prev_ld;
                bp.part_rsum = xm_c ? d_la_rsum.p + slot : nullptr;
                prev_ld = 0;
                bp.Dptr = pool + size_t(j) * SL * SL;
                bp.Cprev = j > 0 ? xpool + size_t(j) * SL * SL : nullptr;
                bp.pdlt = d_la_dlt.p + size_t(pslot) * SL;
                bp.ppos = d_la_dpos.p + size_t(pslot) * SL;
                bp.pnz = d_la_nz.p + pslot;
                bp.dlt = d_la_dlt.p + size_t(slot) * SL;
                bp.dcol = d_la_dcol.p + size_t(slot) * SL;
                bp.dpos = d_la_dpos.p + size_t(slot) * SL;
                bp.nz_out = d_la_nz.p + slot;
                bp.rsum_out = d_la_rsum.p + slot;
                bp.pdd = d_la_dd.p + size_t(pslot) * SL;
                bp.dd = d_la_dd.p + size_t(slot) * SL;
                if (h_report && j == nblk - 1) {
                    bp.report_j = j;
                    bp.report_seq = ++report_seq;
                } else {
                    bp.report_j = -1;
                }
                if (blk_ev[size_t(j)]) AHIP_CHECK(hipStreamWaitEvent(st, blk_ev[size_t(j)], 0));
                if (x_ev[size_t(j)]) AHIP_CHECK(hipStreamWaitEvent(st, x_ev[size_t(j)], 0));
                if (j == 0 && !fr_open) {
                    launch_cd_panel_solve<T>(bp, 0, st);
                    continue;
                }
                const int nbn = (j + 1 < nblk) ? nb_of(j + 1) : 0;
                const int32_t* cols_n = cols_all + size_t(j + 1) * B;
                const int32_t* nz_apply = (j == 0) ? d_zero_i32.p : d_la_nz.p + pslot;
                int ld;
                T* part_out = fuse_reduce ? d_part2.p + size_t(j & 1) * part2_half : d_part.p;
                if (time_panel) t_step.begin(st);
                if (dense())
                    ld = launch_panel_fused<T>(bp, j, D->dense<T>(), cur_w, r_dev, d_la_dcol.p + size_t(pslot) * SL,
                                               d_la_dlt.p + size_t(pslot) * SL, nz_apply, cols_n, nbn, part_out, fuse_reduce, st);
                else
                    ld = launch_panel_fused_snp<T>(bp, j, D->snp(), static_cast<const T*>(D->impute), cur_w, r_dev,
                                                   d_la_dcol.p + size_t(pslot) * SL, d_la_dlt.p + size_t(pslot) * SL,
                                                   nz_apply, cols_n, nbn, part_out, fuse_reduce, st);
                if (time_panel) t_step.end(st);
                if (nbn > 0) {
                    if (fuse_reduce) {
                        prev_ld = ld;
// ... 54 lines not shown
            t_cd.begin(st);
            const int nsl0 = step_of(0);
            build_stale_strips(nblk, tab_nb, tab_ver, nullptr, pool, static_cast<T*>(nullptr),
                               [&](int j) { return std::min(B, count - j * B); }, [&](int j) { return cols_all + size_t(j) * B; });
            const bool vfb = vars_from_blocks();
            if (vfb) {
                if (d_vars_act.cap < size_t(p) + 8) {
                    d_vars_act.reserve(size_t(p) + 8);
                    AHIP_CHECK(hipMemsetAsync(d_vars_act.p, 0, (size_t(p) + 8) * sizeof(T), st));
                }
                vb_vars = screen_pass ? d_vars.p : d_vars_act.p;
                vb_cols_all = cols_all;
                vb_list = screen_pass ? nullptr : cp.active_set;
            }
            build_stale_blocks(nblk, tab_nb, tab_ver, pool, [&](int j) { return std::min(B, count - j * B); },
                               [&](int j) { return cols_all + size_t(j) * B; }, false, screen_pass);
            vb_vars = nullptr;
            merge_strip_events(false);
            pass_e0_valid = false;
            if (!screen_pass && prebuild_screen && !screen_prebuilt && side_grams && st2) {
                screen_prebuilt = true;
                const int cnt_s = cp.nv, nblk_s = (cnt_s + B - 1) / B;
                if (vfb) { vb_vars = d_vars.p; vb_cols_all = d_vcol.p; vb_list = nullptr; }
                build_stale_blocks(nblk_s, dscr_nb, dscr_ver, d_Dpool.p, [&](int j) { return std::min(B, cnt_s - j * B); },
                                   [&](int j) { return d_vcol.p + size_t(j) * B; }, true);
                vb_vars = nullptr;
            }
            bp.gblk = d_gblk.p; bp.dlt = d_dlt.p; bp.dcol = d_dcolblk.p;
            bp.vars = vfb ? (screen_pass ? d_vars.p : d_vars_act.p) : cp.vars;
            bp.Cprev = nullptr; bp.dpos = nullptr; bp.nz_out = nullptr; bp.rsum_out = nullptr;
            bp.part = nullptr; bp.pdd = nullptr; bp.dd = nullptr;
            for (int j = 0; j < nblk; ++j) {
                const int nb = std::min(B, count - j * B);
                const int32_t* cols = cols_all + size_t(j) * B;
                T* Dptr = pool + size_t(j) * SL * SL;
                const int nsl = (j == 0) ? nsl0 : step_of(j);
                pending_slot = -1;
                cnt.n_panel_cols += nb;
                if (!step_tailed_of[j & 1]) panel_reduce(nsl, nb, cols, xm_c, d_gblk.p);
                bp.Dptr = Dptr;
                if (h_report && j == nblk - 1) {
                    bp.report_j = j;
                    bp.report_seq = ++report_seq;
                } else {
                    bp.report_j = -1;
                }
                if (blk_ev[size_t(j)]) AHIP_CHECK(hipStreamWaitEvent(st, blk_ev[size_t(j)], 0));
                launch_cd_panel_solve<T>(bp, j, st);
            }
            t_cd.end(st);
            AHIP_CHECK(hipGetLastError());
            cnt.n_panel_blocks += nblk;
            t_enq += sw_enq.elapsed();
            if (no_wait) { spec_blocks = nblk; return T(0); }
            sw_enq.start();
            wait_pass_state(bs);
            t_wait += sw_enq.elapsed();
            status = bs.status;
            asz = bs.active_size;
            if (trace) std::fprintf(stderr, "[panel] %s count=%d nblk=%d cm=%g tol=%g status=%d asz=%d nz=%d rsq=%g rsum=%g nupd=%lld\n",
                                    screen_pass ? "screen" : "active", count, nblk, double(bs.cm), double(cp.tol), status, asz,
                                    bs.nz, double(bs.rsq), double(bs.resid_sum), (long long)bs.n_updates);
            return bs.cm;
        };
        bool resume_first = mode == 2;
        auto pass = [&](bool screen_pass) -> T {
            if (resume_first) {
                resume_first = false;
                Stopwatch sw_w;
                sw_w.start();
                wait_pass_state(bs);
                t_wait += sw_w.elapsed();
                status = bs.status;
                if (bs.active_size != int32_t(spec_asz))
                    throw make_core_error("speculative pass changed the active set (internal error).");
                asz = bs.active_size;
                return bs.cm;
            }
            const int count = screen_pass ? cp.nv : asz;
            return (la && (count + B - 1) / B >= la_min_blocks) ? pass_la(screen_pass) : pass_plain(screen_pass);
        };
        if (mode == 1) {
            spec_enqueued = false;
            if (asz > 0 && !is_glm()) {
                const int64_t cols0 = cnt.n_panel_cols;
                no_wait = true;
                if (la && (asz + B - 1) / B >= la_min_blocks) pass_la(false);
                else pass_plain(false);
                spec_cols = cnt.n_panel_cols - cols0;
                spec_enqueued = true;
            }
            return;
        }
        while (status == CD_OK) {
            while (status == CD_OK) {
                ++iters;
                ++sc.n_passes_active;
                sc.n_visits_active += asz;
                const T cm = pass(false);
                if (status != CD_OK) break;
                if (cm < cp.tol) break;
                if (iters >= cp.max_iters) { status = CD_MAX_CDS; break; }
            }
            if (status != CD_OK) break;
            ++iters;
            ++sc.n_passes_screen;
            sc.n_visits_screen += cp.nv;
            const T cm = pass(true);
            if (status != CD_OK) break;
            if (cm < cp.tol) break;
            if (iters >= cp.max_iters) { status = CD_MAX_CDS; break; }
        }
        t_cd.begin(st);
        if (la && pending_slot >= 0) {
            panel_step(cur_w, r_dev, d_la_dcol.p + size_t(pending_slot) * SL, d_la_dlt.p + size_t(pending_slot) * SL,
                       d_la_nz.p + pending_slot, d_vcol.p, 0);
            pending_slot = -1;
        } else {
            panel_step(cur_w, r_dev, d_dcolblk.p, d_dlt.p, &d_blk.p->nz, d_vcol.p, 0);
        }
        t_cd.end(st);
        sc.rsq = bs.rsq;
        sc.resid_sum = bs.resid_sum;
        sc.iters = iters;
        sc.n_updates = bs.n_updates;
        sc.active_size = asz;
        sc.status = status;
        sc.n_delta = 0;
        if (status != CD_OK) {
            launch_cd_compact<T>(cp.beta, cp.beta0, cp.vcol, cp.nv, cp.dcols, cp.dvals, &cp.sc->n_delta, st);
            axpy_cols(cp.dcols, cp.dvals, &cp.sc->n_delta, 0, T(1), r_dev);
            sync();
        }
    }

    DevBuf<int32_t> d_blk_g0;
    int64_t actcols_key = -1;
    struct PassTables { int64_t count = -1; int nblk = 0; };
    PassTables ptab_scr, ptab_act;
    DevBuf<int32_t> d_blk_g0_act, d_gdesc_act;
    DevBuf<T> d_la_corr;
    bool pass_tables_cached = true;
    std::vector<int32_t> part_host;
    int build_partition(const idx* list, idx count) {
        const int B = cd_block_size();
        part_host.clear();
        part_host.push_back(0);
        idx acc = 0;
        for (idx pos = 0; pos < count; ++pos) {
            const idx ss = list ? list[pos] : pos;
            const idx q = group_sizes[screen_set[ss]];
            const bool alone = host_cons(screen_set[ss]);
            if (acc > 0 && (acc + q > B || alone)) {
                part_host.push_back(int32_t(pos));
                acc = 0;
            }
            acc += q;
            if (alone) acc = B;
        }
        if (count > 0) part_host.push_back(int32_t(count));
        return int(part_host.size()) - 1;
    }
    void run_group_block_passes(const CdParams<T>& cp, CdScalars<T>& sc) {
        const int B = cd_block_size();
        d_blk.reserve(1);
        d_Dbuf.reserve(size_t(2) * B * B);
        d_dlt.reserve(B);
        d_didx.reserve(B);
        CdBlkState<T> bs{};
        bs.rsq = sc.rsq;
        bs.resid_sum = sc.resid_sum;
        bs.active_size = sc.active_size;
        bs.status = CD_OK;
        d_blk.upload(&bs, 1, st);
        CdGrpBlkParams<T> bp{};
        bp.nv = cp.nv; bp.C = cp.C; bp.ldc = cp.ldc; bp.vars = cp.vars; bp.xmean = cp.xmean; bp.beta = cp.beta; bp.g = cp.g;
        bp.is_active = cp.is_active; bp.active_set = cp.active_set;
        bp.l1 = cp.lmda * cp.alpha; bp.l2 = cp.lmda * (T(1) - cp.alpha);
        bp.newton_tol = cp.newton_tol; bp.dbeta_tol = cp.dbeta_tol; bp.newton_max_iters = cp.newton_max_iters;
        bp.max_active_size = cp.max_active_size;
        bp.V = cp.V; bp.voff = cp.voff; bp.spen = cp.spen; bp.sbegin = cp.sbegin; bp.ssize = cp.ssize;
        bp.Dbuf = d_Dbuf.p; bp.dlt = d_dlt.p; bp.didx = d_didx.p; bp.st = d_blk.p;
        if (cons_on) { bp.clo = d_clo.p; bp.chi = d_chi.p; bp.cmu = d_cmu.p; }
        int64_t iters = 0;
        int status = CD_OK;
        int asz = sc.active_size;
        std::vector<idx> act_host(active_set.begin(), active_set.begin() + asz);
        auto pass = [&](bool screen_pass) -> T {
            const idx count = screen_pass ? idx(cp.ns) : idx(asz);
            if (count <= 0) return T(0);
            const int nblk = build_partition(screen_pass ? nullptr : act_host.data(), count);
            d_blk_g0.reserve(part_host.size());
            d_blk_g0.upload(part_host.data(), part_host.size(), st);
            ptab_scr.count = -1;
            bp.blk_g0 = d_blk_g0.p;
            bp.list = screen_pass ? nullptr : cp.active_set;
            bp.nblk = nblk;
            bp.mark = screen_pass ? 1 : 0;
            t_cd.begin(st);
            if (!cons_host) {
                launch_cd_group_block_pass<T>(bp, st);
            } else {
// ... 172 lines not shown
        for (size_t ss = 0; ss < screen_set.size() && ss < screen_begins.size(); ++ss) begin_of[size_t(screen_set[ss])] = screen_begins[ss];
        for (idx g = 0; g < G; ++g) {
            if (!host_cons(g) || on_device(g)) continue;
            const idx q = group_sizes[g], k = groups[g];
            v.assign(size_t(q), 0);
            if (begin_of[size_t(g)] >= 0) {
                const idx b = begin_of[size_t(g)];
                const double regul = double((1 - alpha) * lm) * double(penalty[g]);
                for (idx t = 0; t < q; ++t) v[size_t(t)] = double(screen_beta[size_t(b + t)]);
                out.assign(size_t(q), 0);
                if (cons_cb->gradient(cons_cb->user, g, q, v.data(), out.data()))
                    throw make_solver_error("constraint.gradient() raised.");
                double acc = 0;
                for (idx t = 0; t < q; ++t) {
                    const double e = double(grad[size_t(k + t)]) - regul * v[size_t(t)] - out[size_t(t)];
                    acc += e * e;
                }
                abs_grad[size_t(g)] = T(std::sqrt(acc));
            } else {
                for (idx t = 0; t < q; ++t) v[size_t(t)] = double(grad[size_t(k + t)]);
                double nrm = 0;
                if (cons_cb->solve_zero(cons_cb->user, g, q, v.data(), &nrm))
                    throw make_solver_error("constraint.solve_zero() raised.");
                abs_grad[size_t(g)] = T(nrm);
            }
        }
    }

    void dev_cons_abs_grad_host(T lm) {
        if (!cons_dev) return;
        const double M = 1e100;
        std::vector<idx> begin_of(static_cast<size_t>(G), idx(-1));
        for (size_t ss = 0; ss < screen_set.size() && ss < screen_begins.size(); ++ss) begin_of[size_t(screen_set[ss])] = screen_begins[ss];
        std::vector<T> va(static_cast<size_t>(p), T(0)), vb(static_cast<size_t>(p), T(0));
        d_cons_va.download(va.data(), size_t(p), st);
        d_cons_vb.download(vb.data(), size_t(p), st);
        sync();
        for (int32_t g : devcons_list) {
            const idx q = group_sizes[g], k = groups[g];
            const bool box = cons_native[g] == ADELIE_HIP_NATIVE_BOX;
            double acc = 0;
            if (begin_of[size_t(g)] >= 0) {
                const idx b = begin_of[size_t(g)];
                const double regul = double((1 - alpha) * lm) * double(penalty[g]);
                for (idx t = 0; t < q; ++t) {
                    const double cg = box ? double(cons_vmu[size_t(k + t)]) : double(va[size_t(k + t)]) * double(cons_vmu[size_t(k + t)]);
                    const double e = double(grad[size_t(k + t)]) - regul * double(screen_beta[size_t(b + t)]) - cg;
                    acc += e * e;
                }
            } else {
                for (idx t = 0; t < q; ++t) {
                    const double v = double(grad[size_t(k + t)]);
                    double m, e;
                    if (box) {
                        const double lo = -std::max(double(va[size_t(k + t)]), -M), up = std::min(double(vb[size_t(k + t)]), M);
                        m = std::min(std::max(v, (lo <= 0) ? -M : 0.0), (up <= 0) ? M : 0.0);
                        e = v - m;
                    } else {
                        const double sg = double(va[size_t(k + t)]), bb = std::min(double(vb[size_t(k + t)]), M);
                        m = std::min(std::max(sg * v, 0.0), (bb <= 0) ? M : 0.0);
                        e = v - sg * m;
                    }
                    cons_vmu[size_t(k + t)] = T(m);
                    acc += e * e;
                }
            }
            abs_grad[size_t(g)] = T(std::sqrt(acc));
        }
        d_cons_mu.upload(cons_vmu.data(), size_t(p), st);
        sync();
    }

    void run_group_panel_passes(const CdParams<T>& cp, CdScalars<T>& sc, T* r_dev) {
        const int SL = cd_block_size();
        panel_setup(group_maxblk());
        const size_t maxblk = panel_maxblk;
        CdBlkState<T> bs{};
        bs.rsq = sc.rsq;
        bs.resid_sum = sc.resid_sum;
        bs.active_size = sc.active_size;
        bs.status = CD_OK;
        bs.nz = 0;
        const int mode = spec_mode;
        if (mode != 2) d_blk.upload(&bs, 1, st);
        bool first_open = open_from_grad && mode != 2 && !cons_on && !multi();
        open_from_grad = false;
        CdGrpBlkParams<T> bp{};
        bp.nv = cp.nv; bp.vars = cp.vars; bp.xmean = cp.xmean; bp.beta = cp.beta;
        bp.is_active = cp.is_active; bp.active_set = cp.active_set;
        bp.l1 = cp.lmda * cp.alpha; bp.l2 = cp.lmda * (T(1) - cp.alpha);
        bp.newton_tol = cp.newton_tol; bp.dbeta_tol = cp.dbeta_tol; bp.newton_max_iters = cp.newton_max_iters;
        bp.max_active_size = cp.max_active_size;
        bp.V = cp.V; bp.voff = cp.voff; bp.spen = cp.spen; bp.sbegin = cp.sbegin; bp.ssize = cp.ssize;
        bp.dlt = d_dlt.p; bp.st = d_blk.p;
        bp.gblk = d_gblk.p; bp.vcol = cp.vcol; bp.dcol = d_dcolblk.p;
        bp.host_st = rep_st_dev; bp.host_seq = rep_seq_dev; bp.report_j = -1; bp.report_seq = 0;
        bp.rot = group_rot ? 1 : 0;
        if (cons_on) { bp.clo = d_clo.p; bp.chi = d_chi.p; bp.cmu = d_cmu.p; }
        struct RotGuard {
            Solver* s;
            ~RotGuard() { s->rot_on = false; s->rot_list = nullptr; }
        } rot_guard{this};
#ifdef AHIP_GRP_PROFILE
        if (!d_grp_dbg.p) { d_grp_dbg.reserve(8); AHIP_CHECK(hipMemsetAsync(d_grp_dbg.p, 0, 8 * sizeof(int64_t), st)); }
        bp.dbg = d_grp_dbg.p;
#endif
        const T* xm_c = intercept ? cur_xm : nullptr;
        int64_t iters = 0;
        int status = CD_OK;
        int asz = sc.active_size;
        std::vector<idx> act_host(active_set.begin(), active_set.begin() + asz);
        std::vector<int32_t>& acols = h_actcols;
        const bool la = lookahead && !is_glm() && (!multi() || multi_w_uniform) && !std_generic() && !sparse();
        if (la) {
            if (xscr_key.size() != maxblk) {
                d_Xpool.reserve(size_t(2) * maxblk * SL * SL);
                xscr_key.assign(maxblk, XKey{});
                xact_key.assign(maxblk, XKey{});
            }
            d_la_dlt.reserve(size_t(2) * SL); d_la_g.reserve(size_t(2) * SL); d_la_rsum.reserve(2); d_la_dd.reserve(size_t(2) * SL);
            d_la_dcol.reserve(size_t(2) * SL); d_la_dpos.reserve(size_t(2) * SL); d_la_nz.reserve(2);
            d_la_dd.reserve(size_t(2) * SL);
            d_part.reserve(size_t(2 * panel_part_elems(n) + 2048));
            part2_half = size_t(panel_part_elems(n));
            d_part2.reserve(2 * part2_half);
            if (mode != 2) pending_slot = -1;
        }
        bool tail_ok = false;
        if (!multi()) {
            if (dense()) {
                constexpr int V = int(16 / sizeof(T));
                tail_ok = (64 * V >= 128) && (D->ld % V == 0) && ((reinterpret_cast<uintptr_t>(D->X) % 16) == 0);
            } else {
                tail_ok = true;
            }
        }
        if (tail_ok && !d_tail_counter.p) {
            d_tail_counter.reserve(2);
            AHIP_CHECK(hipMemsetAsync(d_tail_counter.p, 0, 2 * sizeof(int32_t), st));
        }
        if (!d_zero_i32.p) {
            d_zero_i32.reserve(1);
            AHIP_CHECK(hipMemsetAsync(d_zero_i32.p, 0, sizeof(int32_t), st));
        }
        if (tail_ok) d_part2.reserve(2 * size_t(panel_part_elems(n)));
        bool no_wait = false;
        d_gdesc.reserve(maxblk * size_t(GDESC_STRIDE));
        auto pass_la = [&](bool screen_pass) -> T {
            const bool first_pass = first_open;
            first_open = false;
            const idx count = screen_pass ? idx(cp.ns) : idx(asz);
            if (count <= 0) return T(0);
            const int nblk = build_partition_values(screen_pass ? nullptr : act_host.data(), count);
            PassTables& ptab = screen_pass ? ptab_scr : ptab_act;
            DevBuf<int32_t>& g0buf = screen_pass ? d_blk_g0 : d_blk_g0_act;
            DevBuf<int32_t>& descbuf = screen_pass ? d_gdesc : d_gdesc_act;
            const bool tables_hit = pass_tables_cached && ptab.count == int64_t(count) && ptab.nblk == nblk && g0buf.p && descbuf.p;
            if (!tables_hit) {
                g0buf.reserve(std::max<size_t>(part_host.size(), maxblk + 2));
                g0buf.upload(part_host.data(), part_host.size(), st);
            }
            const int32_t* cols_all = d_vcol.p;
            if (!screen_pass) {
                if (!tables_hit) {
                    acols.clear();
                    for (idx pos = 0; pos < count; ++pos) {
// ... 241 lines not shown
                        if (on_device(screen_set[ss0])) {
                            dev_group_visit(cp, ss0, screen_pass, j == 0, false, j == nblk - 1);
                            last_on_host = false;
                            continue;
                        }
                        host_bs = host_group_visit(cp, ss0, screen_pass, j == 0);
                        last_on_host = (j == nblk - 1);
                        continue;
                    }
                    last_on_host = false;
                }
                bp.Dptr = Dptr;
                if (h_report && j == nblk - 1) {
                    bp.report_j = j;
                    bp.report_seq = ++report_seq;
                } else {
                    bp.report_j = -1;
                }
                if (blk_ev[size_t(j)]) AHIP_CHECK(hipStreamWaitEvent(st, blk_ev[size_t(j)], 0));
                launch_cd_group_panel_solve<T>(bp, j, st);
            }
            t_cd.end(st);
            AHIP_CHECK(hipGetLastError());
            cnt.n_panel_blocks += nblk;
            if (no_wait) { spec_blocks = nblk; return T(0); }
            if (last_on_host) bs = host_bs;
            else wait_pass_state(bs);
            status = bs.status;
            if (bs.active_size > asz) {
                std::vector<int32_t> fresh(size_t(bs.active_size - asz));
                d_actset.download(fresh.data(), fresh.size(), st, asz);
                sync();
                for (int32_t v : fresh) act_host.push_back(v);
            }
            asz = bs.active_size;
            return bs.cm;
        };
        bool resume_first = mode == 2;
        auto pass = [&](bool screen_pass) -> T {
            if (resume_first) {
                resume_first = false;
                wait_pass_state(bs);
                status = bs.status;
                asz = bs.active_size;
                return bs.cm;
            }
            if (!la) return pass_plain(screen_pass);
            const idx count = screen_pass ? idx(cp.ns) : idx(asz);
            const int nblk = count > 0 ? build_partition(screen_pass ? nullptr : act_host.data(), count) : 0;
            return nblk >= la_min_blocks ? pass_la(screen_pass) : pass_plain(screen_pass);
        };
        if (mode == 1) {
            spec_enqueued = false;
            if (asz > 0 && !is_glm()) {
                const int64_t cols0 = cnt.n_panel_cols;
                no_wait = true;
                pass(false);
                spec_cols = cnt.n_panel_cols - cols0;
                spec_enqueued = true;
            }
            return;
        }
        while (status == CD_OK) {
            while (status == CD_OK) {
                ++iters;
                ++sc.n_passes_active;
                sc.n_visits_active += asz;
                const T cm = pass(false);
                if (status != CD_OK) break;
                if (cm < cp.tol) break;
                if (iters >= cp.max_iters) { status = CD_MAX_CDS; break; }
            }
            if (status != CD_OK) break;
            ++iters;
            ++sc.n_passes_screen;
            sc.n_visits_screen += cp.ns;
            const T cm = pass(true);
            if (status != CD_OK) break;
            if (cm < cp.tol) break;
            if (iters >= cp.max_iters) { status = CD_MAX_CDS; break; }
        }
        t_cd.begin(st);
        if (la && pending_slot >= 0) {
            panel_step(cur_w, r_dev, d_la_dcol.p + size_t(pending_slot) * SL, d_la_dlt.p + size_t(pending_slot) * SL,
                       d_la_nz.p + pending_slot, d_vcol.p, 0);
            pending_slot = -1;
        } else {
            panel_step(cur_w, r_dev, d_dcolblk.p, d_dlt.p, &d_blk.p->nz, d_vcol.p, 0);
        }
        t_cd.end(st);
        sc.rsq = bs.rsq;
        sc.resid_sum = bs.resid_sum;
        sc.iters = iters;
        sc.n_updates = bs.n_updates;
        sc.active_size = asz;
        sc.status = status;
        sc.n_delta = 0;
        if (status != CD_OK) {
            launch_cd_compact<T>(cp.beta, cp.beta0, cp.vcol, cp.nv, cp.dcols, cp.dvals, &cp.sc->n_delta, st);
            axpy_cols(cp.dcols, cp.dvals, &cp.sc->n_delta, 0, T(1), r_dev);
            sync();
        }
    }
```

### adelie_amd/csrc/solver_screen.hpp

```cpp
    void sweep(const T* v, T* out, const int32_t* cols, idx ncols, const T* sub_scale, const T* sub_vec,
               bool square = false) {
        if (multi()) {
            if (cols || ncols != p || sub_vec || square) throw make_core_error("unsupported sweep on a multi-response view.");
            const MultiView<T> mv = D->multi<T>();
            launch_multi_sweep<T>(mv, v, out, d_work_sweep.reserve(size_t(multi_sweep_work_elems<T>(mv))), st);
            return;
        }
        if (std_generic()) {
            const T* ce = static_cast<const T*>(D->std_center);
            const T* is = static_cast<const T*>(D->std_iscale);
            T* tmp = d_std_tmp.reserve(size_t(2 * ncols + kVecSumScratch));
            T *raw = tmp, *raw_plain = tmp + ncols, *vsum = tmp + 2 * ncols;
            T* work = d_work_sweep.reserve(size_t(sweep_work_elems(n, ncols)));
            auto base = [&](T* dst, bool sq) {
                if (dense()) launch_sweep<T>(D->dense<T>(), v, dst, 0, ncols, cols, nullptr, nullptr, sq, work, st);
                else launch_sweep_snp<T>(D->snp(), static_cast<const T*>(D->impute), v, dst, 0, ncols, cols, nullptr, nullptr, sq, work, st);
            };
            base(raw, square);
            if (square) base(raw_plain, false);
            launch_vec_sum<T>(v, n, vsum, st);
            launch_std_sweep_epilogue<T>(ce, is, raw, raw_plain, vsum, square, out, 0, ncols, cols, sub_scale, sub_vec, st);
            return;
        }
        if (batcher && dense() && !cols && ncols == p && !square &&
            batcher->template sweep<T>(D->dense<T>(), v, out, sub_scale, sub_vec, st)) {
            ++cnt.n_sweeps_shared;
            return;
        }
        if (dense() && D->factor() && !cols && ncols == p && !square && factor_sweep_on(hooks.factor_sweep)) {
            launch_sweep_factor<T>(D->factor_view<T>(), v, out, sub_scale, sub_vec,
                                   d_work_sweep.reserve(size_t(factor_sweep_work_elems(n, p, D->f_nchunk))), st);
            ++cnt.n_sweeps_factor;
            return;
        }
        if (sparse()) {
            launch_sweep_csc<T>(D->csc<T>(), v, out, 0, ncols, cols, sub_scale, sub_vec, square,
                                d_work_sweep.reserve(size_t(sweep_work_elems_csc(D->sp_parts(), ncols))), st);
            return;
        }
        T* work = d_work_sweep.reserve(size_t(sweep_work_elems(n, ncols)));
        if (dense()) launch_sweep<T>(D->dense<T>(), v, out, 0, ncols, cols, sub_scale, sub_vec, square, work, st);
        else launch_sweep_snp<T>(D->snp(), static_cast<const T*>(D->impute), v, out, 0, ncols, cols, sub_scale, sub_vec, square, work, st);
    }
    DevBuf<int32_t> d_tail_ctr;
    int32_t tail_base = 0;
    bool step_tailed = false;
    int panel_step(const T* w, T* r, const int32_t* dcol, const T* dlt, const int32_t* nz_dev, const int32_t* cols, int nb,
                   bool want_tail = false, const T* tail_xm = nullptr) {
        step_tailed = false;
        if (multi()) return launch_multi_panel_step<T>(D->multi<T>(), w, r, dcol, dlt, nz_dev, cols, nb, d_part.p, st);
        const T* kappa = nullptr;
        const bool stdv = D->std_center != nullptr;
        if (stdv) {
            T* c2 = d_std_coef.reserve(size_t(cd_block_size()) + 16);
            T* kp = c2 + cd_block_size();
            launch_std_scale_coef<T>(static_cast<const T*>(D->std_center), static_cast<const T*>(D->std_iscale), dcol, dlt, nz_dev, 0, c2,
                                     kp, st);
            dlt = c2;
            kappa = kp;
            launch_vec_shift<T>(r, n, kappa, T(-1), nz_dev, st);
        }
        if (sparse()) {
            launch_panel_step_csc<T>(D->csc<T>(), w, r, dcol, dlt, nz_dev, cols, nb, &d_blk.p->resid_sum,
                                     (intercept && !stdv) ? cur_xm : nullptr, d_gblk.p, st);
            if (stdv && nb > 0)
                launch_std_fix_gblk<T>(d_gblk.p, cols, nb, static_cast<const T*>(D->std_center), static_cast<const T*>(D->std_iscale),
                                       &d_blk.p->resid_sum, intercept ? cur_xm : nullptr, st);
            return 0;
        }
        if (dense()) return launch_panel_step<T>(D->dense<T>(), w, r, dcol, dlt, nz_dev, cols, nb, d_part.p, st);
        StepTail<T> tl{};
        const bool tail_ok = want_tail && !stdv && nb > 0;
        if (tail_ok) {
            if (!d_tail_ctr.p) {
                d_tail_ctr.reserve(4);
                AHIP_CHECK(hipMemsetAsync(d_tail_ctr.p, 0, 4 * sizeof(int32_t), st));
                tail_base = 0;
            }
            tl.counter = d_tail_ctr.p; tl.base = tail_base; tl.g = d_gblk.p; tl.rsum = &d_blk.p->resid_sum; tl.xm = tail_xm;
        }
        const int nsl = launch_panel_step_snp<T>(D->snp(), static_cast<const T*>(D->impute), w, r, dcol, dlt, nz_dev, cols, nb,
                                                 d_part.p, st, tail_ok ? &tl : nullptr, &step_tailed);
        if (step_tailed) {
            tail_base += nsl;
            if (tail_base > (int32_t(1) << 30)) {
                AHIP_CHECK(hipMemsetAsync(d_tail_ctr.p, 0, 4 * sizeof(int32_t), st));
                tail_base = 0;
            }
        }
        (void)kappa;
        return nsl;
    }
    void panel_reduce(int nsl, int nb, const int32_t* cols, const T* xm_c, T* gblk) {
        if (nsl <= 0) return;
        if (!std_generic()) {
            launch_panel_reduce<T>(d_part.p, nsl, nb, cols, &d_blk.p->resid_sum, xm_c, gblk, st);
            return;
        }
        launch_panel_reduce<T>(d_part.p, nsl, nb, cols, &d_blk.p->resid_sum, static_cast<const T*>(nullptr), gblk, st);
        launch_std_fix_gblk<T>(gblk, cols, nb, static_cast<const T*>(D->std_center), static_cast<const T*>(D->std_iscale),
                               &d_blk.p->resid_sum, xm_c, st);
    }
    DevBuf<T> d_std_ws[2 + kMaxExtra + 1];
    void std_block_fix(const T* w, const int32_t* cols_base, const SyrkBatch& sb, const T* xm_view, T* D0, int side, hipStream_t gs) {
        T* ws = d_std_ws[side].reserve(size_t(kVecSumScratch) + 8);
        launch_vec_sum<T>(w, n, ws, gs);
        launch_std_block_fix<T>(D0, sb, cols_base, cd_block_size(), static_cast<const T*>(D->std_center),
                                static_cast<const T*>(D->std_iscale), xm_view, ws, intercept, gs);
    }
    void gram_block_batch(const T* w, const int32_t* cols_base, const SyrkBatch& sb, const T* xm, T* D0, int side) {
        const int B = cd_block_size();
        hipStream_t gs = side == 0 ? st : (side >= 2 ? st_x[side - 2] : st2);
        if (sparse()) {
            t_gram.begin(gs);
            const bool stdv = D->std_center != nullptr;
            launch_block_gram_csc<T>(D->csc<T>(), w, cols_base, sb, xm, intercept && !stdv, D0, B, gs);
            if (stdv) std_block_fix(w, cols_base, sb, xm, D0, side, gs);
            t_gram.end(gs);
            for (int y = 0; y < sb.count; ++y) cnt.n_gram_col_reads += 2 * sb.nb[y];
            return;
        }
        T* work = (side == 0 ? d_work_gram : (side >= 2 ? d_work_x[side - 2] : d_work_gram2))
                      .reserve(size_t(std::max(syrk_batch_work_elems(n, sb.count), syrk_work_elems(n, 128))));
        t_gram.begin(gs);
        const bool stdv = std_generic();
        if (dense()) launch_syrk_batch<T>(D->dense<T>(), w, cols_base, sb, xm, intercept && !stdv, D0, B, work, gs);
        else launch_syrk_batch_snp<T>(D->snp(), static_cast<const T*>(D->impute), w, cols_base, sb, xm, intercept && !stdv, D0, B, work, gs);
        if (stdv) std_block_fix(w, cols_base, sb, xm, D0, side, gs);
        t_gram.end(gs);
        for (int y = 0; y < sb.count; ++y) {
            const int nb = sb.nb[y];
            cnt.gram_flops += 2.0 * double(n) * 256.0 * (nb <= 32 ? 3.0 : (nb <= 64 ? 10.0 : 36.0));
            cnt.n_gram_col_reads += 2 * nb;
        }
    }
    void gram_block(const T* w, const int32_t* cols, int nb, const T* xm, T* Dptr, int side = 0) {
        const int B = cd_block_size();
        hipStream_t gs = side == 0 ? st : (side >= 2 ? st_x[side - 2] : st2);
        t_gram.begin(gs);
        if (sparse()) {
            SyrkBatch sb{};
            sb.count = 1; sb.off[0] = 0; sb.nb[0] = nb; sb.dst[0] = 0;
            const bool stdv = D->std_center != nullptr;
            launch_block_gram_csc<T>(D->csc<T>(), w, cols, sb, xm, intercept && !stdv, Dptr, B, gs);
            if (stdv) std_block_fix(w, cols, sb, xm, Dptr, side, gs);
            t_gram.end(gs);
            cnt.n_gram_col_reads += 2 * nb;
            return;
        }
        if (multi()) {
            const MultiView<T> mv = D->multi<T>();
            const int32_t* hc = host_cols(cols);
            multi_seen.clear();
            for (int a = 0; a < nb; ++a) {
                const int32_t u = hc[a] / mv.K;
                if (std::find(multi_seen.begin(), multi_seen.end(), u) == multi_seen.end()) multi_seen.push_back(u);
            }
            const int nu = int(multi_seen.size());
            DevBuf<int32_t>& ml = side ? d_mlist2 : d_mlist;
            DevBuf<T>& mc = side ? d_mC2 : d_mC;
            ml.reserve(size_t(6 * B));
            mc.reserve(size_t(B) * B);
            launch_multi_block_lists(cols, nb, mv.K, ml.p, ml.p + B, ml.p + 2 * B, gs);
            T* work = (side ? d_work_gram2 : d_work_gram).reserve(size_t(syrk_work_elems(mv.nb, 128)));
            const int reps = multi_w_uniform ? 1 : mv.K;
            for (int l = 0; l < reps; ++l) {
                launch_syrk_multi<T>(mv, w + size_t(l) * size_t(mv.nb), ml.p, nu, mc.p, B, work, gs);
                launch_multi_expand<T>(mc.p, B, ml.p + B, ml.p + 2 * B, nb, multi_w_uniform ? -1 : l, Dptr, B, gs);
                cnt.gram_flops += 2.0 * double(mv.nb) * 256.0 * (nu <= 32 ? 3.0 : (nu <= 64 ? 10.0 : 36.0));
            }
            cnt.n_gram_col_reads += 2 * nu * reps;
            t_gram.end(gs);
            return;
        }
// ... 44 lines not shown
    void gram(const T* w, idx M, idx pos0, idx N, const T* xm, bool center) {
        T* work = d_work_gram.reserve(size_t(sparse() ? gram_work_elems_csc(n, M, N, D->sp_parts()) : gram_work_elems(n, M, N)));
        t_gram.begin(st);
        if (std_generic()) {
            const T* ce = static_cast<const T*>(D->std_center);
            const T* is = static_cast<const T*>(D->std_iscale);
            if (dense())
                launch_gram<T>(D->dense<T>(), w, d_vcol.p, int32_t(M), 0, d_vcol.p + pos0, int32_t(N), int32_t(pos0), xm, false, d_C.p,
                               ldc, work, st);
            else
                launch_gram_snp<T>(D->snp(), static_cast<const T*>(D->impute), w, d_vcol.p, int32_t(M), 0, d_vcol.p + pos0, int32_t(N),
                                   int32_t(pos0), xm, false, d_C.p, ldc, work, st);
            T* tmp = d_std_tmp.reserve(size_t(M + kVecSumScratch));
            T *mv = tmp, *wsum = tmp + M;
            T* swork = d_work_sweep.reserve(size_t(sweep_work_elems(n, M)));
            if (dense()) launch_sweep<T>(D->dense<T>(), w, mv, 0, M, d_vcol.p, nullptr, nullptr, false, swork, st);
            else launch_sweep_snp<T>(D->snp(), static_cast<const T*>(D->impute), w, mv, 0, M, d_vcol.p, nullptr, nullptr, false, swork, st);
            launch_vec_sum<T>(w, n, wsum, st);
            launch_std_gram_fix<T>(ce, is, d_C.p, ldc, int32_t(M), int32_t(pos0), int32_t(N), d_vcol.p, mv, wsum, xm, center, st);
        } else if (sparse())
            launch_gram_csc<T>(D->csc<T>(), w, d_vcol.p, int32_t(M), 0, d_vcol.p + pos0, int32_t(N), int32_t(pos0), xm, center, d_C.p,
                               ldc, work, st);
        else if (dense())
            launch_gram<T>(D->dense<T>(), w, d_vcol.p, int32_t(M), 0, d_vcol.p + pos0, int32_t(N), int32_t(pos0), xm, center,
                           d_C.p, ldc, work, st);
        else
            launch_gram_snp<T>(D->snp(), static_cast<const T*>(D->impute), w, d_vcol.p, int32_t(M), 0, d_vcol.p + pos0,
                               int32_t(N), int32_t(pos0), xm, center, d_C.p, ldc, work, st);
        t_gram.end(st);
        cnt.n_gram_col_reads += M + N;
        cnt.gram_flops += 2.0 * double(n) * double(M) * double(N);
        gram_shapes.emplace_back(M, N);
    }
    Staging stage;
    DeferredFrees deferred;
    double t_sync_total = 0;
    bool uv_side = true;
    hipEvent_t uv_ev = nullptr, uv_in_ev = nullptr;
    bool uv_pending = false;
    void join_uv() {
        if (!uv_pending) return;
        AHIP_CHECK(hipStreamWaitEvent(st, uv_ev, 0));
        uv_pending = false;
    }
    void sync() {
        join_uv();
        const auto t0 = std::chrono::steady_clock::now();
        AHIP_CHECK(hipStreamSynchronize(st));
        t_sync_total += std::chrono::duration<double>(std::chrono::steady_clock::now() - t0).count();
        stage.reset();
    }

    void update_abs_grad_host(T lm) {
        for (size_t ss = 0; ss < screen_set.size(); ++ss) {
            const idx i = screen_set[ss], b = screen_begins[ss], k = groups[i], sz = group_sizes[i];
            const T regul = ((1 - alpha) * lm) * penalty2[i];
            if (cons_on && cons_kind[i] && !host_cons(i)) {
                abs_grad[i] = std::abs(grad[k] - regul * screen_beta[b] - cons_mu[i]);
                continue;
            }
            T acc = 0;
            for (idx t = 0; t < sz; ++t) {
                const T e = grad[k + t] - regul * screen_beta[b + t];
                acc += e * e;
            }
            abs_grad[i] = std::sqrt(acc);
        }
        for (idx i = 0; i < G; ++i) {
            if (is_screen(i)) continue;
            const idx k = groups[i];
            if (cons_on && cons_kind[i] && !host_cons(i)) {
                const T M = T(1e100), v = grad[k];
                cons_mu[i] = std::min(std::max(v, cons_lo[i] >= 0 ? -M : T(0)), cons_hi[i] <= 0 ? M : T(0));
                abs_grad[i] = std::abs(v - cons_mu[i]);
                continue;
            }
            T acc = 0;
            for (idx t = 0; t < group_sizes[i]; ++t) acc += grad[k + t] * grad[k + t];
            abs_grad[i] = std::sqrt(acc);
        }
    }

    T lmda_of_sweep = 0;
    void device_abs_grad(T lm, int active_now) {
        lmda_of_sweep = lm;
        if (cons_on) {
            launch_abs_grad_cons<T>(d_grad.p, d_groups.p, d_gsizes.p, G, d_slot.p, d_beta.p, d_penalty.p, (1 - alpha) * lm, d_clo_g.p,
                                    d_chi_g.p, d_cmu.p, d_absgrad.p, d_mu_g.p, st);
            d_mu_g.download(cons_mu.data(), size_t(G), st);
            if (cons_dev)
                launch_cons_abs_grad<T>(d_devcons_list.p, int(devcons_list.size()), d_cons_native.p, d_groups.p, d_gsizes.p, d_slot.p,
                                        d_grad.p, d_beta.p, d_penalty.p, (1 - alpha) * lm, d_cons_va.p, d_cons_vb.p, d_cons_mu.p, d_absgrad.p, st);
        } else {
            launch_abs_grad<T>(d_grad.p, d_groups.p, d_gsizes.p, G, d_slot.p, d_beta.p, has_pen2 ? d_penalty2.p : d_penalty.p,
                               (1 - alpha) * lm, d_absgrad.p, st);
        }
        d_absgrad.download(abs_grad.data(), size_t(G), st);
    }

    int64_t n_host_screens = 0;

    void update_screen_derived_base() {
        const auto old = screen_begins.size();
        if (in_screen.size() != size_t(G)) in_screen.assign(G, 0);
        for (size_t i = old; i < screen_set.size(); ++i) in_screen[screen_set[i]] = 1;
        size_t vs = (old == 0) ? 0 : (screen_begins.back() + group_sizes[screen_set[old - 1]]);
        for (size_t i = old; i < screen_set.size(); ++i) {
            screen_begins.push_back(vs);
            vs += group_sizes[screen_set[i]];
        }
        screen_beta.resize(vs, 0);
        screen_is_active.resize(screen_set.size(), 0);
    }

    void device_append_screen() {
        const idx ns = idx(screen_set.size());
        if (ns_dev == ns) return;
        std::vector<int32_t> vcol, sbegin, ssize, slot_idx;
        std::vector<T> spen, beta_new;
        std::vector<int8_t> isact;
        const size_t fallbacks0 = stage.n_fallback;
        const idx nv_old = nv;
        idx nv_new = nv_old;
        for (idx ss = ns_dev; ss < ns; ++ss) {
            const idx g = screen_set[ss];
            sbegin.push_back(int32_t(screen_begins[ss]));
            ssize.push_back(int32_t(group_sizes[g]));
            spen.push_back(penalty[g]);
            isact.push_back(screen_is_active[ss]);
            for (idx t = 0; t < group_sizes[g]; ++t) {
                vcol.push_back(int32_t(groups[g] + t));
                beta_new.push_back(screen_beta[screen_begins[ss] + t]);
            }
            nv_new += group_sizes[g];
        }
        h_vcol.resize(size_t(nv_old));
        h_vcol.insert(h_vcol.end(), vcol.begin(), vcol.end());
        const int Ng = int(ns - ns_dev), Nv = int(nv_new - nv_old);
        const AppendImage<T> L(Ng, Nv, cons_on);
        app_img.assign(L.total, 0);
        auto put = [&](size_t off, const void* src, size_t bytes) { if (bytes) std::memcpy(app_img.data() + off, src, bytes); };
        put(L.pen, spen.data(), sizeof(T) * spen.size());
        if (has_pen2) {
            h_spen2.reserve(size_t(G));
            h_spen2.resize(size_t(ns_dev));
            for (idx ss = ns_dev; ss < ns; ++ss) h_spen2.push_back(penalty2[screen_set[ss]]);
            d_spen2.upload(h_spen2.data() + ns_dev, size_t(ns - ns_dev), st, size_t(ns_dev));
        }
        put(L.beta, beta_new.data(), sizeof(T) * beta_new.size());
        if (cons_on) {
            std::vector<T> clo_new, chi_new, cmu_new;
            for (idx ss = ns_dev; ss < ns; ++ss) {
                const idx g = screen_set[ss];
                for (idx t = 0; t < group_sizes[g]; ++t) {
                    clo_new.push_back(cons_lo[g]);
                    chi_new.push_back(cons_hi[g]);
                    cmu_new.push_back(cons_mu[g]);
                }
            }
            put(L.lo, clo_new.data(), sizeof(T) * clo_new.size());
            put(L.hi, chi_new.data(), sizeof(T) * chi_new.size());
            put(L.mu, cmu_new.data(), sizeof(T) * cmu_new.size());
        }
        std::vector<int32_t> isact32(isact.begin(), isact.end()), grp32;
        for (idx ss = ns_dev; ss < ns; ++ss) grp32.push_back(int32_t(screen_set[ss]));
        put(L.begin, sbegin.data(), 4 * sbegin.size());
        put(L.size, ssize.data(), 4 * ssize.size());
        put(L.isact, isact32.data(), 4 * isact32.size());
        put(L.group, grp32.data(), 4 * grp32.size());
// ... 60 lines not shown
        for (idx ss = idx(g_begin); ss < ns; ++ss) {
            const idx q = group_sizes[screen_set[ss]];
            if (q > 1) any_group = true;
            max_q = std::max(max_q, q);
        }
        if (any_group && device_eig && max_q <= idx(kEigMaxQ)) {
            eig_desc.clear();
            size_t v_new = 0;
            if (h_voff.size() < size_t(ns)) h_voff.resize(size_t(ns), 0);
            for (idx ss = idx(g_begin); ss < ns; ++ss) {
                const idx q = group_sizes[screen_set[ss]], b = screen_begins[ss];
                if (q == 1) continue;
                EigDesc e{};
                e.src = b + b * ldc;
                e.ld = int32_t(ldc);
                e.q = int32_t(q);
                e.vars_pos = b;
                e.v_off = int64_t(v_used + v_new);
                voff[ss - g_begin] = idx(v_used + v_new);
                h_voff[size_t(ss)] = voff[ss - g_begin];
                v_new += size_t(q) * q;
                eig_desc.push_back(e);
            }
            if (v_new) d_V.grow(v_used + v_new, v_used, st);
            v_used += v_new;
            d_eig_desc.reserve(eig_desc.size());
            d_eig_desc.upload(eig_desc.data(), eig_desc.size(), st);
            launch_grp_eig<T>(d_C.p, d_eig_desc.p, int(eig_desc.size()), int(max_q), d_vars.p, d_V.p, st);
            d_voff.upload(voff.data(), voff.size(), st, g_begin);
            host_mirrors_stale = true;
            if (Staging::current() != &stage || !stage.base) sync();
            return;
        }
        std::vector<T> vars_host(N);
        d_vars.download(vars_host.data(), N, st, pos0);
        sync();
        if (any_group) {
            for (idx ss = idx(g_begin); ss < ns; ++ss) {
                const idx q = group_sizes[screen_set[ss]], b = screen_begins[ss];
                if (q == 1) {
                    screen_transforms[ss] = std::vector<T>{T(1)};
                    continue;
                }
                std::vector<T> blk(size_t(q) * q);
                AHIP_CHECK(hipMemcpy2DAsync(blk.data(), q * sizeof(T), d_C.p + b + b * ldc, ldc * sizeof(T), q * sizeof(T), q,
                                            hipMemcpyDeviceToHost, st));
                sync();
                std::vector<double> A(blk.begin(), blk.end()), V, Dv;
                jacobi_eigh(int(q), A, V, Dv);
                std::vector<T> Vt(V.begin(), V.end());
                for (idx t = 0; t < q; ++t) vars_host[b + t - pos0] = T(Dv[t] >= 0 ? Dv[t] : 0.0);
                d_V.grow(v_used + size_t(q) * q, v_used, st);
                d_V.upload(Vt.data(), Vt.size(), st, v_used);
                voff[ss - g_begin] = idx(v_used);
                if (h_voff.size() < size_t(ns)) h_voff.resize(size_t(ns), 0);
                h_voff[size_t(ss)] = idx(v_used);
                v_used += size_t(q) * q;
                screen_transforms[ss] = std::move(Vt);
                sync();
            }
            d_vars.upload(vars_host.data(), N, st, pos0);
            d_voff.upload(voff.data(), voff.size(), st, g_begin);
            sync();
        } else {
            for (idx ss = idx(g_begin); ss < ns; ++ss) screen_transforms[ss] = std::vector<T>{T(1)};
        }
        for (idx t = 0; t < N; ++t) screen_vars[pos0 + t] = vars_host[t];
    }

    void update_vars_panel(const T* w_dev, const T* xm_dev, const std::vector<T>& xm_host, size_t g_begin) {
        const idx ns = idx(screen_set.size());
        const idx pos0 = (g_begin < size_t(ns)) ? screen_begins[g_begin] : nv;
        const idx N = nv - pos0;
        screen_X_means.resize(nv);
        screen_vars.resize(nv, 0);
        screen_transforms.resize(ns);
        if (N <= 0) return;
        cnt.n_new_screen_cols += N;
        if (!all_scalar) {
            update_vars_panel_groups(w_dev, xm_dev, xm_host, g_begin, pos0, N);
            return;
        }
        const bool vfb = vars_from_blocks();
        if (!vfb) sweep(w_dev, d_vars.p + pos0, d_vcol.p + pos0, N, nullptr, nullptr, true);
        for (idx ss = idx(g_begin); ss < ns; ++ss) {
            const idx g = screen_set[ss], b = screen_begins[ss];
            screen_X_means[b] = xm_host[groups[g]];
            if (screen_transforms[ss].size() != 1) screen_transforms[ss].assign(1, T(1));
        }
        launch_gather<T>(xm_dev, d_vcol.p + pos0, N, d_sxm.p + pos0, st);
        if (!vfb) launch_center_vars<T>(d_vars.p + pos0, d_sxm.p + pos0, int(N), intercept, st);
    }

    std::vector<int32_t> gp_vbeg;
    size_t n_host_cons = 0;
    size_t group_maxblk() const { return size_t(2 * p / cd_block_size() + 2) + 2 * n_host_cons; }
    int build_partition_values(const idx* list, idx count) {
        const int nblk = build_partition(list, count);
        gp_vbeg.assign(size_t(nblk) + 1, 0);
        int32_t acc = 0;
        for (int j = 0; j < nblk; ++j) {
            for (int32_t pos = part_host[j]; pos < part_host[j + 1]; ++pos)
                acc += int32_t(group_sizes[screen_set[list ? list[pos] : pos]]);
            gp_vbeg[size_t(j) + 1] = acc;
        }
        return nblk;
    }
    void update_vars_panel_groups(const T* w_dev, const T* xm_dev, const std::vector<T>& xm_host, size_t g_begin, idx pos0,
                                  idx N) {
        const idx ns = idx(screen_set.size());
        const int SL = cd_block_size();
        panel_setup(group_maxblk());
        const int nblk = build_partition_values(nullptr, ns);
        for (idx ss = idx(g_begin); ss < ns; ++ss) {
            const idx g = screen_set[ss], b = screen_begins[ss];
            for (idx t = 0; t < group_sizes[g]; ++t) screen_X_means[b + t] = xm_host[groups[g] + t];
        }
        launch_gather<T>(xm_dev, d_vcol.p + pos0, N, d_sxm.p + pos0, st);
        int j0 = 0;
        while (j0 + 1 < nblk && size_t(part_host[j0 + 1]) <= g_begin) ++j0;
        idx max_q = 1;
        for (idx ss = idx(g_begin); ss < ns; ++ss) max_q = std::max(max_q, group_sizes[screen_set[ss]]);
        const bool dev_eig = device_eig && max_q <= idx(kEigMaxQ);
        std::vector<T> hD(dev_eig ? size_t(0) : size_t(nblk - j0) * SL * SL);
        std::vector<int> rebuilt_blocks;
        if (!is_glm()) { cur_w = w_dev; cur_xm = xm_dev; }
        const bool use_strips = strips_apply();
        const bool raw_split = use_strips && group_rot;
        T* const rawbase = raw_split ? d_Draw.p : d_Dpool.p;
        const bool on_side = use_strips && dev_eig && uv_side && side_grams && st2 != nullptr;
        if (use_strips) {
            const bool with_x = lookahead && xscr_key.size() == panel_maxblk && d_Xpool.p != nullptr;
            build_stale_strips(nblk, dscr_nb, dscr_ver, with_x ? &xscr_key : nullptr, rawbase, with_x ? d_Xpool.p : static_cast<T*>(nullptr),
                               [&](int j) { return int(gp_vbeg[size_t(j) + 1] - gp_vbeg[j]); },
                               [&](int j) { return d_vcol.p + gp_vbeg[j]; }, nullptr, nullptr, !on_side);
            rebuilt_blocks = strip_built;
        }
        for (int j = j0; j < nblk; ++j) {
            const int nval = gp_vbeg[size_t(j) + 1] - gp_vbeg[j];
            T* Dptr = rawbase + size_t(j) * SL * SL;
            if (dscr_nb[j] != nval || dscr_ver[j] != w_version) {
                gram_block(w_dev, d_vcol.p + gp_vbeg[j], nval, xm_dev, Dptr);
                dscr_nb[j] = nval;
                dscr_ver[j] = w_version;
                ++cnt.n_panel_grams;
                rebuilt_blocks.push_back(j);
            }
            if (!dev_eig)
                AHIP_CHECK(hipMemcpyAsync(hD.data() + size_t(j - j0) * SL * SL, Dptr, size_t(SL) * SL * sizeof(T),
                                          hipMemcpyDeviceToHost, st));
        }
        std::vector<idx> voff(size_t(ns) - g_begin, 0);
        h_voff.resize(size_t(ns), 0);
        if (dev_eig) {
            eig_desc.clear();
            size_t v_new = 0;
            int j = j0;
            for (idx ss = idx(g_begin); ss < ns; ++ss) {
                while (j + 1 < nblk && part_host[j + 1] <= int32_t(ss)) ++j;
                const idx q = group_sizes[screen_set[ss]], b = screen_begins[ss];
                const idx o = b - gp_vbeg[j];
                EigDesc e{};
                e.src = int64_t(j) * SL * SL + o + o * SL;
                e.ld = SL;
                e.q = int32_t(q);
                e.vars_pos = b;
                e.v_off = 0;
                if (q > 1) {
                    voff[ss - g_begin] = idx(v_used + v_new);
                    h_voff[size_t(ss)] = voff[ss - g_begin];
                    e.v_off = int64_t(v_used + v_new);
                    v_new += size_t(q) * q;
                }
                eig_desc.push_back(e);
            }
// ... 280 lines not shown
```

Before: 3.970.

## Fuse abs-grad into sweep, vars into one launch, panel close, speculative open

Several kernel launches are merged. The sweep kernel now computes abs_grad in its epilogue for scalar groups. Screen variances, centering and the mean gather run in a single split-reduce kernel that uses an atomic counter. The closing panel step writes w*r and a residual snapshot directly, and the beta0 copy and column gather are folded into the speculative-open kernel. The aim is to cut launch overhead and extra passes over HBM. The cost is added code paths with device counters and internal state flags that must stay consistent.

```diff
diff --git a/adelie_amd/csrc/kernels.hpp b/adelie_amd/csrc/kernels.hpp
--- a/adelie_amd/csrc/kernels.hpp
+++ b/adelie_amd/csrc/kernels.hpp
@@ -39,8 +39,21 @@
 template <class T> void launch_fill(T* out, T value, int64_t n, hipStream_t s);
 
 template <class T>
+struct SweepAbsGrad {
+    const int32_t* slot;
+    const T* screen_beta;
+    const T* penalty;
+    T oma_lmda;
+    T* abs_grad;
+};
+template <class T>
 void launch_sweep(const DenseView<T>& X, const T* v, T* out, int64_t c0, int64_t ncols, const int32_t* cols,
-                  const T* sub_scale, const T* sub_vec, bool square, T* work, hipStream_t s);
+                  const T* sub_scale, const T* sub_vec, bool square, T* work, hipStream_t s,
+                  const SweepAbsGrad<T>* abs_grad = nullptr);
+template <class T>
+void launch_sweep_vars(const DenseView<T>& X, const T* v, int64_t ncols, const int32_t* cols, const T* xm_by_col, bool center,
+                       T* vars, T* xm_out, T* work, int32_t* counter, hipStream_t s);
+int64_t sweep_vars_counters(int64_t ncols);
 template <class T>
 void launch_sweep_snp(const SnpView& X, const T* impute, const T* v, T* out, int64_t c0, int64_t ncols,
                       const int32_t* cols, const T* sub_scale, const T* sub_vec, bool square, T* work, hipStream_t s);
@@ -387,6 +400,9 @@
 int launch_panel_step(const DenseView<T>& X, const T* w, T* r, const int32_t* dcol, const T* dlt, const int32_t* nz_dev,
                       const int32_t* cols, int nb, T* part, hipStream_t s);
 template <class T>
+int launch_panel_close(const DenseView<T>& X, const T* w, T* r, const int32_t* dcol, const T* dlt, const int32_t* nz_dev,
+                       T* v_out, T* snap_out, hipStream_t s);
+template <class T>
 struct StepTail {
     int32_t* counter;
     int32_t base;
@@ -401,6 +417,9 @@
 int64_t panel_part_elems(int64_t n);
 template <class T>
 void launch_la_open_from_grad(const T* grad, const int32_t* cols, int nb, T* g, const T* rsum_src, T* rsum_out, hipStream_t s);
+template <class T>
+void launch_spec_open(const T* beta, T* beta0, int nv, const int32_t* vcol, const int32_t* active_set, int ngather,
+                      int32_t* actcols, const T* grad, int nb, T* g, const T* rsum_src, T* rsum_out, hipStream_t s);
 template <class T>
 void launch_panel_reduce(const T* part, int nslices, int nb, const int32_t* cols, const T* rsum_dev, const T* xm_by_col,
                          T* gblk, hipStream_t s);
diff --git a/adelie_amd/csrc/kernels_cd_panel.hip b/adelie_amd/csrc/kernels_cd_panel.hip
--- a/adelie_amd/csrc/kernels_cd_panel.hip
+++ b/adelie_amd/csrc/kernels_cd_panel.hip
@@ -64,11 +64,12 @@
 template <class T, int VEC> struct RawOf<T, DenseAcc<T>, VEC> { using type = RawDense<T, VEC>; };
 template <class T, int VEC> struct RawOf<T, SnpAcc<T>, VEC> { using type = RawSnp; };
 
-template <class T, class Acc, int VEC, bool FULL, bool WGRED = false>
+template <class T, class Acc, int VEC, bool FULL, bool WGRED = false, bool EPI = false>
 __device__ __forceinline__ void panel_step_body(const Acc& X, int64_t n, const T* __restrict__ w, T* __restrict__ r,
                                                 const int32_t* __restrict__ dcol, const T* __restrict__ dlt, int nz,
                                                 const int32_t* __restrict__ cols, int nb, T* __restrict__ part,
-                                                int64_t part_ld, T (*red)[64 * VEC], T* wrs, int tid, int64_t slice) {
+                                                int64_t part_ld, T (*red)[64 * VEC], T* wrs, int tid, int64_t slice,
+                                                T* __restrict__ v_out = nullptr, T* __restrict__ snap_out = nullptr) {
     constexpr int U = 16;
     using Raw = typename RawOf<T, Acc, VEC>::type;
     const int lane = tid & 63;
@@ -121,13 +122,27 @@
                     const T rr = r[i + e] - ((red[0][q] + red[1][q]) + (red[2][q] + red[3][q]));
                     r[i + e] = rr;
                     wr = w[i + e] * rr;
+                    if constexpr (EPI) {
+                        v_out[i + e] = wr;
+                        if (snap_out) snap_out[i + e] = rr;
+                    }
                 }
                 wrs[q] = wr;
             }
         }
     } else if (wv == 0) {
-#pragma unroll
-        for (int e = 0; e < VEC; ++e) wrs[lane * VEC + e] = (FULL || i + e < n) ? w[i + e] * r[i + e] : T(0);
+        if constexpr (EPI) {
+#pragma unroll
+            for (int e = 0; e < VEC; ++e)
+                if (FULL || i + e < n) {
+                    const T rr = r[i + e];
+                    v_out[i + e] = w[i + e] * rr;
+                    if (snap_out) snap_out[i + e] = rr;
+                }
+        } else {
+#pragma unroll
+            for (int e = 0; e < VEC; ++e) wrs[lane * VEC + e] = (FULL || i + e < n) ? w[i + e] * r[i + e] : T(0);
+        }
     }
     if (nb <= 0) return;
     __syncthreads();
@@ -174,6 +189,23 @@
         panel_step_body<T, Acc, VEC, true>(X, n, w, r, dcol, dlt, nz, cols, nb, part, part_ld, red, wrs, threadIdx.x, blockIdx.x);
     else
         panel_step_body<T, Acc, VEC, false>(X, n, w, r, dcol, dlt, nz, cols, nb, part, part_ld, red, wrs, threadIdx.x, blockIdx.x);
+}
+
+template <class T, class Acc, int VEC>
+__global__ __launch_bounds__(PT, (VEC >= 16 ? 2 : 4)) void panel_close_kernel(Acc X, int64_t n, const T* __restrict__ w, T* __restrict__ r,
+                                                         const int32_t* __restrict__ dcol, const T* __restrict__ dlt,
+                                                         const int32_t* __restrict__ nz_dev, T* __restrict__ v_out,
+                                                         T* __restrict__ snap_out) {
+    constexpr int RS = 64 * VEC;
+    __shared__ T red[4][RS];
+    __shared__ T wrs[RS];
+    const int nz = nz_dev[0];
+    if ((int64_t(blockIdx.x) + 1) * RS <= n)
+        panel_step_body<T, Acc, VEC, true, false, true>(X, n, w, r, dcol, dlt, nz, nullptr, 0, nullptr, 0, red, wrs, threadIdx.x,
+                                                        blockIdx.x, v_out, snap_out);
+    else
+        panel_step_body<T, Acc, VEC, false, false, true>(X, n, w, r, dcol, dlt, nz, nullptr, 0, nullptr, 0, red, wrs, threadIdx.x,
+                                                         blockIdx.x, v_out, snap_out);
 }
 
 constexpr int S16_RS = 1024;
@@ -536,6 +568,16 @@
 }
 
 template <class T, class Acc, int VEC>
+int close_launch(const Acc& acc, int64_t n, const T* w, T* r, const int32_t* dcol, const T* dlt, const int32_t* nz_dev, T* v_out,
+                 T* snap_out, hipStream_t s) {
+    constexpr int RS = 64 * VEC;
+    const int64_t ns = (n + RS - 1) / RS;
+    hipLaunchKernelGGL((panel_close_kernel<T, Acc, VEC>), dim3((unsigned)ns), dim3(PT), 0, s, acc, n, w, r, dcol, dlt, nz_dev,
+                       v_out, snap_out);
+    return int(ns);
+}
+
+template <class T, class Acc, int VEC>
 __global__ __launch_bounds__(256 * FS) void panel_fused_grp_kernel(CdGrpBlkParams<T> sp, int j, Acc X, int64_t n,
                                                                   const T* __restrict__ w, T* __restrict__ r,
                                                                   const int32_t* __restrict__ dcol,
@@ -702,6 +744,34 @@
 void launch_la_open_from_grad(const T* grad, const int32_t* cols, int nb, T* g, const T* rsum_src, T* rsum_out, hipStream_t s) {
     hipLaunchKernelGGL((la_open_kernel<T>), dim3(1), dim3(PB), 0, s, grad, cols, nb, g, rsum_src, rsum_out);
 }
+namespace {
+template <class T>
+__global__ void spec_open_kernel(const T* __restrict__ beta, T* __restrict__ beta0, int nv, const int32_t* __restrict__ vcol,
+                                 const int32_t* __restrict__ active_set, int ngather, int32_t* __restrict__ actcols,
+                                 const T* __restrict__ grad, int nb, T* __restrict__ g, const T* __restrict__ rsum_src,
+                                 T* __restrict__ rsum_out) {
+    const int a = blockIdx.x * blockDim.x + threadIdx.x;
+    if (a < nv) beta0[a] = beta[a];
+    if (a < ngather) actcols[a] = vcol[active_set[a]];
+    if (a < nb) g[a] = grad[vcol[active_set[a]]];
+    if (a == 0 && rsum_src) {
+        const T v = rsum_src[0];
+        rsum_out[0] = v;
+        rsum_out[1] = v;
+    }
+}
+}
+template <class T>
+void launch_spec_open(const T* beta, T* beta0, int nv, const int32_t* vcol, const int32_t* active_set, int ngather,
+                      int32_t* actcols, const T* grad, int nb, T* g, const T* rsum_src, T* rsum_out, hipStream_t s) {
+    const int m = std::max(std::max(nv, ngather), std::max(nb, 1));
+    hipLaunchKernelGGL((spec_open_kernel<T>), dim3((unsigned)((m + 255) / 256)), dim3(256), 0, s, beta, beta0, nv, vcol, active_set,
+                       ngather, actcols, grad, nb, g, rsum_src, rsum_out);
+}
+template void launch_spec_open<double>(const double*, double*, int, const int32_t*, const int32_t*, int, int32_t*, const double*,
+                                       int, double*, const double*, double*, hipStream_t);
+template void launch_spec_open<float>(const float*, float*, int, const int32_t*, const int32_t*, int, int32_t*, const float*, int,
+                                      float*, const float*, float*, hipStream_t);
 template void launch_la_open_from_grad<double>(const double*, const int32_t*, int, double*, const double*, double*, hipStream_t);
 template void launch_la_open_from_grad<float>(const float*, const int32_t*, int, float*, const float*, float*, hipStream_t);
 
@@ -715,6 +785,16 @@
     const bool vecok = (X.ld % V == 0) && ((reinterpret_cast<uintptr_t>(X.X) % 16) == 0);
     if (vecok) return step_launch<T, DenseAcc<T>, V>(acc, X.n, w, r, dcol, dlt, nz_dev, cols, nb, part, s);
     return step_launch<T, DenseAcc<T>, 1>(acc, X.n, w, r, dcol, dlt, nz_dev, cols, nb, part, s);
+}
+
+template <class T>
+int launch_panel_close(const DenseView<T>& X, const T* w, T* r, const int32_t* dcol, const T* dlt, const int32_t* nz_dev,
+                       T* v_out, T* snap_out, hipStream_t s) {
+    DenseAcc<T> acc{X.X, X.ld};
+    constexpr int V = VecOf<T>::N;
+    const bool vecok = (X.ld % V == 0) && ((reinterpret_cast<uintptr_t>(X.X) % 16) == 0);
+    if (vecok) return close_launch<T, DenseAcc<T>, V>(acc, X.n, w, r, dcol, dlt, nz_dev, v_out, snap_out, s);
+    return close_launch<T, DenseAcc<T>, 1>(acc, X.n, w, r, dcol, dlt, nz_dev, v_out, snap_out, s);
 }
 
 template <class T>
@@ -766,6 +846,8 @@
 #define INST(T)                                                                                                        \
     template int launch_panel_step<T>(const DenseView<T>&, const T*, T*, const int32_t*, const T*, const int32_t*,     \
                                       const int32_t*, int, T*, hipStream_t);                                           \
+    template int launch_panel_close<T>(const DenseView<T>&, const T*, T*, const int32_t*, const T*, const int32_t*,    \
+                                       T*, T*, hipStream_t);                                                           \
     template int launch_panel_step_snp<T>(const SnpView&, const T*, const T*, T*, const int32_t*, const T*,            \
                                           const int32_t*, const int32_t*, int, T*, hipStream_t, const StepTail<T>*,    \
                                           bool*);                                                                      \
diff --git a/adelie_amd/csrc/kernels_sweep.hip b/adelie_amd/csrc/kernels_sweep.hip
--- a/adelie_amd/csrc/kernels_sweep.hip
+++ b/adelie_amd/csrc/kernels_sweep.hip
@@ -28,12 +28,26 @@
     return r;
 }
 
-template <class T, class Acc, int CB, int VEC, bool SQ>
+template <class T>
+__device__ __forceinline__ void abs_grad_of_column(const SweepAbsGrad<T>& ag, int64_t c, T s) {
+    const int32_t sl = ag.slot[c];
+    T acc = T(0);
+    if (sl >= 0) {
+        const T regul = ag.oma_lmda * ag.penalty[c];
+        const T e = s - regul * ag.screen_beta[sl];
+        acc += e * e;
+    } else {
+        acc += s * s;
+    }
+    ag.abs_grad[c] = sqrt(acc);
+}
+
+template <class T, class Acc, int CB, int VEC, bool SQ, bool AG = false>
 __global__ __launch_bounds__(kThreads) void sweep_kernel(Acc X, const T* __restrict__ v, T* __restrict__ out,
                                                          int64_t n, int64_t c0, int64_t ncols,
                                                          const int32_t* __restrict__ cols, int64_t rows_per_split,
                                                          int nsplit, const T* __restrict__ sub_scale,
-                                                         const T* __restrict__ sub_vec) {
+                                                         const T* __restrict__ sub_vec, SweepAbsGrad<T> ag = SweepAbsGrad<T>{}) {
     const int tid = threadIdx.x;
     const int64_t cb = blockIdx.x;
     const int split = blockIdx.y;
@@ -95,6 +109,7 @@
             if (nsplit == 1) {
                 if (sub_vec) s -= sub_scale[0] * sub_vec[cols ? int64_t(cols[c]) : c0 + c];
                 out[c] = s;
+                if constexpr (AG) abs_grad_of_column(ag, c, s);
             } else {
                 out[int64_t(split) * ncols + c] = s;
             }
@@ -105,7 +120,7 @@
 template <class T>
 __global__ void sweep_reduce_kernel(const T* __restrict__ part, T* __restrict__ out, int64_t ncols, int nsplit,
                                     int64_t c0, const int32_t* __restrict__ cols, const T* __restrict__ sub_scale,
-                                    const T* __restrict__ sub_vec) {
+                                    const T* __restrict__ sub_vec, SweepAbsGrad<T> ag) {
     const int64_t c = int64_t(blockIdx.x) * blockDim.x + threadIdx.x;
     if (c >= ncols) return;
     T s = T(0);
@@ -115,6 +130,96 @@
         s -= sub_scale[0] * sub_vec[j];
     }
     out[c] = s;
+    if (ag.abs_grad) abs_grad_of_column(ag, c, s);
+}
+
+template <class T, class Acc, int CB, int VEC>
+__global__ __launch_bounds__(kThreads) void sweep_vars_kernel(Acc X, const T* __restrict__ v, T* part, int64_t n, int64_t ncols,
+                                                              const int32_t* __restrict__ cols, int64_t rows_per_split,
+                                                              int nsplit, const T* __restrict__ xm_by_col, int center,
+                                                              T* __restrict__ vars, T* __restrict__ xm_out, int32_t* counter) {
+    const int tid = threadIdx.x;
+    const int64_t cb = blockIdx.x;
+    const int split = blockIdx.y;
+    const int64_t r0 = int64_t(split) * rows_per_split;
+    const int64_t r1 = min(n, r0 + rows_per_split);
+
+    int64_t cj[CB];
+    decltype(X.colptr(0)) cp[CB];
+#pragma unroll
+    for (int k = 0; k < CB; ++k) {
+        int64_t c = cb * CB + k;
+        if (c >= ncols) c = ncols - 1;
+        cj[k] = int64_t(cols[c]);
+        cp[k] = X.colptr(cj[k]);
+    }
+    T acc[CB];
+#pragma unroll
+    for (int k = 0; k < CB; ++k) acc[k] = T(0);
+
+    const int64_t body_end = r0 + ((r1 - r0) / VEC) * VEC;
+#pragma unroll 2
+    for (int64_t i = r0 + int64_t(tid) * VEC; i < body_end; i += int64_t(kThreads) * VEC) {
+        const Pack<T, VEC> vv = load_vec<T, VEC>(v + i);
+        Pack<T, VEC> xx[CB];
+#pragma unroll
+        for (int k = 0; k < CB; ++k) xx[k] = X.template load<VEC>(cp[k], i, cj[k]);
+#pragma unroll
+        for (int k = 0; k < CB; ++k)
+#pragma unroll
+            for (int e = 0; e < VEC; ++e) {
+                const T x = xx[k].v[e] * xx[k].v[e];
+                acc[k] = fma(x, vv.v[e], acc[k]);
+            }
+    }
+    for (int64_t i = body_end + tid; i < r1; i += kThreads) {
+        const T vi = v[i];
+#pragma unroll
+        for (int k = 0; k < CB; ++k) {
+            const T x0 = X.template load<1>(cp[k], i, cj[k]).v[0];
+            const T x = x0 * x0;
+            acc[k] = fma(x, vi, acc[k]);
+        }
+    }
+
+    __shared__ T red[kThreads / 64][CB];
+    __shared__ int s_rank;
+    const int lane = tid & 63, wv = tid >> 6;
+#pragma unroll
+    for (int k = 0; k < CB; ++k) {
+        const T s = wave_sum(acc[k]);
+        if (lane == 0) red[wv][k] = s;
+    }
+    __syncthreads();
+    const int64_t c = cb * CB + tid;
+    const bool mine = tid < CB && c < ncols;
+    T s = T(0);
+    if (mine) {
+#pragma unroll
+        for (int w = 0; w < kThreads / 64; ++w) s += red[w][tid];
+    }
+    if (nsplit > 1) {
+        if (mine) part[int64_t(split) * ncols + c] = s;
+        __threadfence();
+        __syncthreads();
+        if (tid == 0) s_rank = atomicAdd(counter + cb, 1);
+        __syncthreads();
+        if (s_rank != nsplit - 1) return;
+        __threadfence();
+        if (mine) {
+            s = T(0);
+            for (int r = 0; r < nsplit; ++r)
+                s += __hip_atomic_load(part + int64_t(r) * ncols + c, __ATOMIC_RELAXED, __HIP_MEMORY_SCOPE_AGENT);
+        }
+        if (tid == 0) counter[cb] = 0;
+    }
+    if (mine) {
+        const T xm = xm_by_col[cols[c]];
+        T var = s;
+        if (center) var -= xm * xm;
+        vars[c] = var > T(0) ? var : T(0);
+        xm_out[c] = xm;
+    }
 }
 
 constexpr int kSweepCB = 4;
@@ -139,14 +244,19 @@
 
 template <class T, class Acc, int VEC>
 void sweep_dispatch(Acc acc, const T* v, T* out, int64_t n, int64_t c0, int64_t ncols, const int32_t* cols,
-                    const T* sub_scale, const T* sub_vec, bool square, T* work, hipStream_t s) {
+                    const T* sub_scale, const T* sub_vec, bool square, T* work, hipStream_t s,
+                    const SweepAbsGrad<T>* agp = nullptr) {
     if (ncols <= 0) return;
     int64_t blocks_c, rows_per_split;
     int nsplit;
     sweep_shape(n, ncols, VEC, blocks_c, nsplit, rows_per_split);
     dim3 grid((unsigned)blocks_c, (unsigned)nsplit);
     T* dst = nsplit == 1 ? out : work;
-    if (square && sweep_cb() == 8)
+    const SweepAbsGrad<T> ag = agp ? *agp : SweepAbsGrad<T>{};
+    if (agp && nsplit == 1)
+        hipLaunchKernelGGL((sweep_kernel<T, Acc, kSweepCB, VEC, false, true>), grid, dim3(kThreads), 0, s, acc, v, dst, n, c0,
+                           ncols, cols, rows_per_split, nsplit, sub_scale, sub_vec, ag);
+    else if (square && sweep_cb() == 8)
         hipLaunchKernelGGL((sweep_kernel<T, Acc, 8, VEC, true>), grid, dim3(kThreads), 0, s, acc, v, dst, n, c0,
                            ncols, cols, rows_per_split, nsplit, sub_scale, sub_vec);
     else if (square)
@@ -161,8 +271,20 @@
     if (nsplit > 1) {
         const int bt = 256;
         hipLaunchKernelGGL((sweep_reduce_kernel<T>), dim3((unsigned)((ncols + bt - 1) / bt)), dim3(bt), 0, s, work, out,
-                           ncols, nsplit, c0, cols, sub_scale, sub_vec);
-    }
+                           ncols, nsplit, c0, cols, sub_scale, sub_vec, ag);
+    }
+}
+
+template <class T, class Acc, int VEC>
+void sweep_vars_dispatch(Acc acc, const T* v, int64_t n, int64_t ncols, const int32_t* cols, const T* xm_by_col, bool center,
+                         T* vars, T* xm_out, T* work, int32_t* counter, hipStream_t s) {
+    if (ncols <= 0) return;
+    int64_t blocks_c, rows_per_split;
+    int nsplit;
+    sweep_shape(n, ncols, VEC, blocks_c, nsplit, rows_per_split);
+    dim3 grid((unsigned)blocks_c, (unsigned)nsplit);
+    hipLaunchKernelGGL((sweep_vars_kernel<T, Acc, kSweepCB, VEC>), grid, dim3(kThreads), 0, s, acc, v, work, n, ncols, cols,
+                       rows_per_split, nsplit, xm_by_col, center ? 1 : 0, vars, xm_out, counter);
 }
 
 template <class T, class Acc, int VEC>
@@ -489,13 +611,24 @@
 
 template <class T>
 void launch_sweep(const DenseView<T>& X, const T* v, T* out, int64_t c0, int64_t ncols, const int32_t* cols,
-                  const T* sub_scale, const T* sub_vec, bool square, T* work, hipStream_t s) {
+                  const T* sub_scale, const T* sub_vec, bool square, T* work, hipStream_t s, const SweepAbsGrad<T>* abs_grad) {
+    DenseAcc<T> acc{X.X, X.ld};
+    if (abs_grad && (cols || c0 != 0 || square)) abs_grad = nullptr;
+    if (dense_vec_ok(X) && (reinterpret_cast<uintptr_t>(v) % 16) == 0)
+        sweep_dispatch<T, DenseAcc<T>, VecOf<T>::N>(acc, v, out, X.n, c0, ncols, cols, sub_scale, sub_vec, square, work, s, abs_grad);
+    else
+        sweep_dispatch<T, DenseAcc<T>, 1>(acc, v, out, X.n, c0, ncols, cols, sub_scale, sub_vec, square, work, s, abs_grad);
+}
+template <class T>
+void launch_sweep_vars(const DenseView<T>& X, const T* v, int64_t ncols, const int32_t* cols, const T* xm_by_col, bool center,
+                       T* vars, T* xm_out, T* work, int32_t* counter, hipStream_t s) {
     DenseAcc<T> acc{X.X, X.ld};
     if (dense_vec_ok(X) && (reinterpret_cast<uintptr_t>(v) % 16) == 0)
-        sweep_dispatch<T, DenseAcc<T>, VecOf<T>::N>(acc, v, out, X.n, c0, ncols, cols, sub_scale, sub_vec, square, work, s);
+        sweep_vars_dispatch<T, DenseAcc<T>, VecOf<T>::N>(acc, v, X.n, ncols, cols, xm_by_col, center, vars, xm_out, work, counter, s);
     else
-        sweep_dispatch<T, DenseAcc<T>, 1>(acc, v, out, X.n, c0, ncols, cols, sub_scale, sub_vec, square, work, s);
-}
+        sweep_vars_dispatch<T, DenseAcc<T>, 1>(acc, v, X.n, ncols, cols, xm_by_col, center, vars, xm_out, work, counter, s);
+}
+int64_t sweep_vars_counters(int64_t ncols) { return (ncols + kSweepCB - 1) / kSweepCB; }
 constexpr int LUT_TR = 256;
 static_assert(LUT_TR == 256, "lut_shape's tile");
 template <class T, bool SQ>
@@ -623,7 +756,7 @@
         if (ns > 1) {
             const int bt = 256;
             hipLaunchKernelGGL((sweep_reduce_kernel<T>), dim3((unsigned)((ncols + bt - 1) / bt)), dim3(bt), 0, s, work, out,
-                               ncols, int(ns), c0, cols, sub_scale, sub_vec);
+                               ncols, int(ns), c0, cols, sub_scale, sub_vec, SweepAbsGrad<T>{});
         }
         return;
     }
@@ -881,7 +1014,9 @@
     template void launch_vmul<T>(const T*, const T*, T*, int64_t, hipStream_t);                                        \
     template void launch_fill<T>(T*, T, int64_t, hipStream_t);                                                         \
     template void launch_sweep<T>(const DenseView<T>&, const T*, T*, int64_t, int64_t, const int32_t*, const T*,       \
-                                  const T*, bool, T*, hipStream_t);                                                    \
+                                  const T*, bool, T*, hipStream_t, const SweepAbsGrad<T>*);                            \
+    template void launch_sweep_vars<T>(const DenseView<T>&, const T*, int64_t, const int32_t*, const T*, bool, T*, T*, \
+                                       T*, int32_t*, hipStream_t);                                                     \
     template void launch_sweep_snp<T>(const SnpView&, const T*, const T*, T*, int64_t, int64_t, const int32_t*,        \
                                       const T*, const T*, bool, T*, hipStream_t);                                      \
     template void launch_axpy_cols<T>(const DenseView<T>&, const int32_t*, const T*, const int32_t*, int32_t, T, T*,   \
diff --git a/adelie_amd/csrc/solver_fit.hpp b/adelie_amd/csrc/solver_fit.hpp
--- a/adelie_amd/csrc/solver_fit.hpp
+++ b/adelie_amd/csrc/solver_fit.hpp
@@ -54,6 +54,7 @@
         cp.max_group_size = int32_t(max_gs);
         Stopwatch sw;
         sw.start();
+        bool snap_fused = false;
         bool small_fit = false;
         open_from_grad = grad_fresh && open_from_grad_opt && !is_glm() && !cov_mode && r_dev == d_r.p && !resume && !std_generic();
         grad_fresh = false;
@@ -62,14 +63,24 @@
             spec_mode = resume ? 2 : 0;
             spec_active = false;
             struct ModeGuard { int& m; ~ModeGuard() { m = 0; } } mode_guard{spec_mode};
+            const bool sweep_follows = !is_glm() && r_dev == d_r.p && prelaunch_sweep && inv_wanted;
+            const bool spec_follows = sweep_follows && spec_enabled && spec_next_lm > T(0) && !cons_on;
+            if (spec_follows) d_r_snap.reserve(size_t(n));
+            close_v = sweep_follows ? d_v.p : nullptr;
+            close_snap = spec_follows ? d_r_snap.p : nullptr;
+            close_fused = false;
+            struct CloseGuard { T*& v; T*& s; ~CloseGuard() { v = nullptr; s = nullptr; } } close_guard{close_v, close_snap};
             if (all_scalar) run_panel_passes(cp, sc, r_dev);
             else run_group_panel_passes(cp, sc, r_dev);
-            if (!is_glm() && sc.status == CD_OK && r_dev == d_r.p && prelaunch_sweep && inv_wanted) {
-                launch_vmul<T>(d_w.p, d_r.p, d_v.p, n, st);
+            snap_fused = close_fused && spec_follows;
+            if (sweep_follows && sc.status == CD_OK) {
+                if (!close_fused) launch_vmul<T>(d_w.p, d_r.p, d_v.p, n, st);
+                SweepAbsGrad<T> ag{};
+                const bool want_ag = sweep_abs_grad(lm, ag);
                 t_sweep.begin(st);
-                sweep(d_v.p, d_grad.p, nullptr, p, &d_blk.p->resid_sum, intercept ? d_xm.p : nullptr);
+                sweep(d_v.p, d_grad.p, nullptr, p, &d_blk.p->resid_sum, intercept ? d_xm.p : nullptr, false, want_ag ? &ag : nullptr);
                 t_sweep.end(st);
-                device_abs_grad(lm, int(sc.active_size));
+                device_abs_grad(lm, int(sc.active_size), sweep_ag_done);
                 grad_fresh = true;
                 inv_prelaunched = true;
                 inv_prelaunched_lm = lm;
@@ -158,8 +169,8 @@
                 act.clear();
             }
             d_r_snap.reserve(size_t(n));
-            AHIP_CHECK(hipMemcpyAsync(d_beta0.p, d_beta.p, size_t(nv) * sizeof(T), hipMemcpyDeviceToDevice, st));
-            AHIP_CHECK(hipMemcpyAsync(d_r_snap.p, d_r.p, size_t(n) * sizeof(T), hipMemcpyDeviceToDevice, st));
+            beta0_pending = true;
+            if (!snap_fused) AHIP_CHECK(hipMemcpyAsync(d_r_snap.p, d_r.p, size_t(n) * sizeof(T), hipMemcpyDeviceToDevice, st));
             CdParams<T> cp2 = cp;
             cp2.lmda = spec_next_lm;
             CdScalars<T> sc2{};
@@ -171,7 +182,7 @@
             spec_used_grad = grad_fresh;
             grad_fresh = false;
             {
-                struct ModeGuard { int& m; ~ModeGuard() { m = 0; } } mode_guard{spec_mode};
+                struct ModeGuard { int& m; bool& b; ~ModeGuard() { m = 0; b = false; } } mode_guard{spec_mode, beta0_pending};
                 if (all_scalar) run_panel_passes(cp2, sc2, r_dev);
                 else run_group_panel_passes(cp2, sc2, r_dev);
             }
diff --git a/adelie_amd/csrc/solver_panel.hpp b/adelie_amd/csrc/solver_panel.hpp
--- a/adelie_amd/csrc/solver_panel.hpp
+++ b/adelie_amd/csrc/solver_panel.hpp
@@ -136,6 +136,12 @@
         sync();
     }
 
+    bool beta0_pending = false;
+    void flush_beta0(const CdParams<T>& cp) {
+        if (!beta0_pending) return;
+        beta0_pending = false;
+        AHIP_CHECK(hipMemcpyAsync(d_beta0.p, d_beta.p, size_t(cp.nv) * sizeof(T), hipMemcpyDeviceToDevice, st));
+    }
     void run_panel_passes(const CdParams<T>& cp, CdScalars<T>& sc, T* r_dev) {
         const int B = panel_bsz > 0 ? panel_bsz : (is_glm() ? 64 : cd_block_size());
         const int SL = cd_block_size();
@@ -197,8 +203,12 @@
             const int count = screen_pass ? cp.nv : asz;
             if (count <= 0) return T(0);
             const int32_t* cols_all = d_vcol.p;
+            int spec_gather = 0;
             if (!screen_pass) {
-                if (actcols_key != count) launch_gather_i32(d_vcol.p, cp.active_set, count, d_actcols.p, st);
+                if (actcols_key != count) {
+                    if (beta0_pending) spec_gather = count;
+                    else launch_gather_i32(d_vcol.p, cp.active_set, count, d_actcols.p, st);
+                }
                 actcols_key = count;
                 cols_all = d_actcols.p;
             }
@@ -220,8 +230,14 @@
             int prev_ld = 0;
             const bool from_grad = fr_open && first_pass && pending_slot < 0;
             if (from_grad) {
-                launch_la_open_from_grad<T>(d_grad.p, cols_all, nb_of(0), d_la_g.p, xm_c ? &d_blk.p->resid_sum : nullptr,
-                                            d_la_rsum.p, st);
+                if (beta0_pending) {
+                    launch_spec_open<T>(d_beta.p, d_beta0.p, cp.nv, d_vcol.p, cp.active_set, spec_gather, d_actcols.p, d_grad.p, nb_of(0),
+                                        d_la_g.p, xm_c ? &d_blk.p->resid_sum : nullptr, d_la_rsum.p, st);
+                    beta0_pending = false;
+                } else {
+                    launch_la_open_from_grad<T>(d_grad.p, cols_all, nb_of(0), d_la_g.p, xm_c ? &d_blk.p->resid_sum : nullptr,
+                                                d_la_rsum.p, st);
+                }
             } else if (fr_open) {
                 const int ps = pending_slot;
                 CdBlkParams<T> op = bp;
@@ -442,11 +458,14 @@
         };
         if (mode == 1) {
             spec_enqueued = false;
+            const bool la_pass = la && (asz + B - 1) / B >= la_min_blocks;
+            if (!(asz > 0 && !is_glm() && la_pass && fuse_reduce && la_fused_open && first_open && pending_slot < 0)) flush_beta0(cp);
             if (asz > 0 && !is_glm()) {
                 const int64_t cols0 = cnt.n_panel_cols;
                 no_wait = true;
-                if (la && (asz + B - 1) / B >= la_min_blocks) pass_la(false);
+                if (la_pass) pass_la(false);
                 else pass_plain(false);
+                if (beta0_pending) throw make_core_error("speculative pass opened without its coefficient copy (internal error).");
                 spec_cols = cnt.n_panel_cols - cols0;
                 spec_enqueued = true;
             }
@@ -473,11 +492,11 @@
         }
         t_cd.begin(st);
         if (la && pending_slot >= 0) {
-            panel_step(cur_w, r_dev, d_la_dcol.p + size_t(pending_slot) * SL, d_la_dlt.p + size_t(pending_slot) * SL,
-                       d_la_nz.p + pending_slot, d_vcol.p, 0);
+            panel_close(r_dev, d_la_dcol.p + size_t(pending_slot) * SL, d_la_dlt.p + size_t(pending_slot) * SL,
+                        d_la_nz.p + pending_slot);
             pending_slot = -1;
         } else {
-            panel_step(cur_w, r_dev, d_dcolblk.p, d_dlt.p, &d_blk.p->nz, d_vcol.p, 0);
+            panel_close(r_dev, d_dcolblk.p, d_dlt.p, &d_blk.p->nz);
         }
         t_cd.end(st);
         sc.rsq = bs.rsq;
@@ -816,6 +835,7 @@
         bs.status = CD_OK;
         bs.nz = 0;
         const int mode = spec_mode;
+        flush_beta0(cp);
         if (mode != 2) d_blk.upload(&bs, 1, st);
         bool first_open = open_from_grad && mode != 2 && !cons_on && !multi();
         open_from_grad = false;
@@ -1223,11 +1243,11 @@
         }
         t_cd.begin(st);
         if (la && pending_slot >= 0) {
-            panel_step(cur_w, r_dev, d_la_dcol.p + size_t(pending_slot) * SL, d_la_dlt.p + size_t(pending_slot) * SL,
-                       d_la_nz.p + pending_slot, d_vcol.p, 0);
+            panel_close(r_dev, d_la_dcol.p + size_t(pending_slot) * SL, d_la_dlt.p + size_t(pending_slot) * SL,
+                        d_la_nz.p + pending_slot);
             pending_slot = -1;
         } else {
-            panel_step(cur_w, r_dev, d_dcolblk.p, d_dlt.p, &d_blk.p->nz, d_vcol.p, 0);
+            panel_close(r_dev, d_dcolblk.p, d_dlt.p, &d_blk.p->nz);
         }
         t_cd.end(st);
         sc.rsq = bs.rsq;
diff --git a/adelie_amd/csrc/solver_screen.hpp b/adelie_amd/csrc/solver_screen.hpp
--- a/adelie_amd/csrc/solver_screen.hpp
+++ b/adelie_amd/csrc/solver_screen.hpp
@@ -1,5 +1,7 @@
+    bool sweep_ag_done = false;
     void sweep(const T* v, T* out, const int32_t* cols, idx ncols, const T* sub_scale, const T* sub_vec,
-               bool square = false) {
+               bool square = false, const SweepAbsGrad<T>* ag = nullptr) {
+        sweep_ag_done = false;
         if (multi()) {
             if (cols || ncols != p || sub_vec || square) throw make_core_error("unsupported sweep on a multi-response view.");
             const MultiView<T> mv = D->multi<T>();
@@ -39,8 +41,13 @@
             return;
         }
         T* work = d_work_sweep.reserve(size_t(sweep_work_elems(n, ncols)));
-        if (dense()) launch_sweep<T>(D->dense<T>(), v, out, 0, ncols, cols, sub_scale, sub_vec, square, work, st);
-        else launch_sweep_snp<T>(D->snp(), static_cast<const T*>(D->impute), v, out, 0, ncols, cols, sub_scale, sub_vec, square, work, st);
+        if (dense()) {
+            if (cols || ncols != p || square) ag = nullptr;
+            launch_sweep<T>(D->dense<T>(), v, out, 0, ncols, cols, sub_scale, sub_vec, square, work, st, ag);
+            sweep_ag_done = ag != nullptr;
+        } else {
+            launch_sweep_snp<T>(D->snp(), static_cast<const T*>(D->impute), v, out, 0, ncols, cols, sub_scale, sub_vec, square, work, st);
+        }
     }
     DevBuf<int32_t> d_tail_ctr;
     int32_t tail_base = 0;
@@ -90,6 +97,16 @@
         }
         (void)kappa;
         return nsl;
+    }
+    T *close_v = nullptr, *close_snap = nullptr;
+    bool close_fused = false;
+    void panel_close(T* r, const int32_t* dcol, const T* dlt, const int32_t* nz_dev) {
+        if (close_v && r == d_r.p && cur_w == d_w.p && dense() && D->std_center == nullptr) {
+            launch_panel_close<T>(D->dense<T>(), cur_w, r, dcol, dlt, nz_dev, close_v, close_snap, st);
+            close_fused = true;
+            return;
+        }
+        panel_step(cur_w, r, dcol, dlt, nz_dev, d_vcol.p, 0);
     }
     void panel_reduce(int nsl, int nb, const int32_t* cols, const T* xm_c, T* gblk) {
         if (nsl <= 0) return;
@@ -300,9 +317,19 @@
     }
 
     T lmda_of_sweep = 0;
-    void device_abs_grad(T lm, int active_now) {
+    bool sweep_abs_grad(T lm, SweepAbsGrad<T>& ag) const {
+        if (cons_on || !all_scalar || G != p) return false;
+        ag.slot = d_slot.p;
+        ag.screen_beta = d_beta.p;
+        ag.penalty = has_pen2 ? d_penalty2.p : d_penalty.p;
+        ag.oma_lmda = (1 - alpha) * lm;
+        ag.abs_grad = d_absgrad.p;
+        return true;
+    }
+    void device_abs_grad(T lm, int active_now, bool in_sweep = false) {
         lmda_of_sweep = lm;
-        if (cons_on) {
+        if (in_sweep) {
+        } else if (cons_on) {
             launch_abs_grad_cons<T>(d_grad.p, d_groups.p, d_gsizes.p, G, d_slot.p, d_beta.p, d_penalty.p, (1 - alpha) * lm, d_clo_g.p,
                                     d_chi_g.p, d_cmu.p, d_absgrad.p, d_mu_g.p, st);
             d_mu_g.download(cons_mu.data(), size_t(G), st);
@@ -529,15 +556,28 @@
             return;
         }
         const bool vfb = vars_from_blocks();
-        if (!vfb) sweep(w_dev, d_vars.p + pos0, d_vcol.p + pos0, N, nullptr, nullptr, true);
+        const bool one_launch = !vfb && dense() && D->std_center == nullptr;
+        if (one_launch) {
+            const size_t nctr = size_t(sweep_vars_counters(p)) + 8;
+            if (d_vars_ctr.cap < nctr) {
+                d_vars_ctr.reserve(nctr);
+                AHIP_CHECK(hipMemsetAsync(d_vars_ctr.p, 0, nctr * sizeof(int32_t), st));
+            }
+            launch_sweep_vars<T>(D->dense<T>(), w_dev, N, d_vcol.p + pos0, xm_dev, intercept, d_vars.p + pos0, d_sxm.p + pos0,
+                                 d_work_sweep.reserve(size_t(sweep_work_elems(n, N))), d_vars_ctr.p, st);
+        } else if (!vfb) {
+            sweep(w_dev, d_vars.p + pos0, d_vcol.p + pos0, N, nullptr, nullptr, true);
+        }
         for (idx ss = idx(g_begin); ss < ns; ++ss) {
             const idx g = screen_set[ss], b = screen_begins[ss];
             screen_X_means[b] = xm_host[groups[g]];
             if (screen_transforms[ss].size() != 1) screen_transforms[ss].assign(1, T(1));
         }
+        if (one_launch) return;
         launch_gather<T>(xm_dev, d_vcol.p + pos0, N, d_sxm.p + pos0, st);
         if (!vfb) launch_center_vars<T>(d_vars.p + pos0, d_sxm.p + pos0, int(N), intercept, st);
     }
+    DevBuf<int32_t> d_vars_ctr;
 
     std::vector<int32_t> gp_vbeg;
     size_t n_host_cons = 0;
```

Result: slower. 3.912 (-1.5%).
